# bytewax/bytewax

Measured on AMD Instinct MI355X. Metric: events/sec (whole node), tumbling-window wordcount, higher is better.
Workload: dtype int64; 1 GPU; model=tumbling-window wordcount (keyed count, 60s windows), events_per_batch_per_gpu=64000000, vocab=1000000, parallelism=key-hash all-to-allv dp1, engine=dataflow (run_main: source -> keyed_window_agg -> sink), radix=True, radix_v2=False, latency_method=poll-gap under load, closed_window_rows=317000000

## Files before the change

### bytewax_amd/_native/stream_kernels.hip

```cpp

#include <hip/hip_runtime.h>
#include <torch/extension.h>
#include <pybind11/stl.h>
#include <ATen/hip/HIPContext.h>

#include <chrono>
#include <type_traits>
#include <cstdlib>
#include <cstdint>
#include <cstring>
#include <vector>

#define WAVE 64
#define EMPTY_SLOT 0xFFFFFFFFFFFFFFFFULL

#define HIP_CHECK(expr)                                               \
  do {                                                                \
    hipError_t _e = (expr);                                           \
    TORCH_CHECK(_e == hipSuccess, "HIP error: ", hipGetErrorString(_e)); \
  } while (0)

static inline int n_blocks(int64_t n, int block) {
  int64_t b = (n + block - 1) / block;
  if (b > 2048) b = 2048;
// ... 169 lines not shown
    int64_t late_cap) {
  static_assert(!(LATE && DEDUP), "late tracking excludes the dedup path");
  if (ts_base_dev != nullptr) ts_base += *ts_base_dev;
  int lane = threadIdx.x & (WAVE - 1);
  int64_t stride = gridDim.x * (int64_t)blockDim.x;
  int64_t local_max = 0;
  int64_t first = blockIdx.x * (int64_t)blockDim.x + threadIdx.x;
  for (int64_t i = first; i - lane < n; i += stride) {
    bool valid = i < n;
    int64_t t = valid ? ((int64_t)ts[i] + ts_base) : 0;
    if constexpr (LATE) {
      bool is_late = valid && t < late_cutoff;
      int64_t lv = 0;
      if (MODE == AGG_SUM && is_late) lv = vals[i];
      late_append<MODE == AGG_SUM>(
          is_late, is_late ? keys[i] : 0, t, lv, late_keys, late_ts,
          late_vals, late_n, late_cap, error_flag);
      if (is_late) {
        valid = false;
        t = 0;
      }
    }
    if (t > local_max) local_max = t;
    uint64_t packed = 0;
    unsigned long long inc = 0;
    if (valid) {
      int64_t win = (t - align_ms) / off_ms;
      packed = ((uint64_t)(uint32_t)(int32_t)win << 32) | (uint32_t)keys[i];
      inc = (MODE == AGG_COUNT) ? 1ULL : (unsigned long long)vals[i];
      if (off_ms < len_ms) {
        int64_t num = t - align_ms - len_ms;
        int64_t win_lo = num / off_ms;
        if (num % off_ms != 0 && num < 0) win_lo -= 1;
        win_lo += 1;
        for (int64_t wn = win_lo; wn < win; ++wn) {
          uint64_t p2 =
              ((uint64_t)(uint32_t)(int32_t)wn << 32) | (uint32_t)keys[i];
          if (!hash_add(tkeys, tvals, mask, region_bits, p2, inc)) {
            atomicOr(error_flag, 1);
          }
        }
      }
    }

    bool ok = true;
    if (DEDUP) {
      unsigned long long remaining = __ballot(valid);
      bool leader = false;
      unsigned long long agg = 0;
      while (remaining) {
        int l = __ffsll((unsigned long long)remaining) - 1;
        uint64_t lk = (uint64_t)__shfl((long long)packed, l);
        unsigned long long match =
            __ballot(valid && packed == lk);
        if (MODE == AGG_COUNT) {
          if (lane == l) {
            leader = true;
            agg = __popcll(match);
          }
        } else {
          unsigned long long contrib =
              (valid && packed == lk) ? inc : 0ULL;
          for (int off = WAVE / 2; off > 0; off >>= 1) {
            contrib += (unsigned long long)__shfl_xor(
                (long long)contrib, off);
          }
          if (lane == l) {
            leader = true;
            agg = contrib;
          }
        }
        remaining &= ~match;
      }
      if (leader) ok = hash_add(tkeys, tvals, mask, region_bits, packed, agg);
    } else if (valid) {
      ok = hash_add(tkeys, tvals, mask, region_bits, packed, inc);
    }
    if (!ok) atomicOr(error_flag, 1);
  }
  for (int off = WAVE / 2; off > 0; off >>= 1) {
    int64_t other = __shfl_down((long long)local_max, off);
    if (other > local_max) local_max = other;
  }
  if ((threadIdx.x & (WAVE - 1)) == 0 && local_max > 0) {
    atomicMax(max_ts, (unsigned long long)local_max);
  }
}



#define V2_COARSE 256
#define V2_STAGE 32

__global__ __launch_bounds__(512) void k_scatter_coarse(
    const int32_t* __restrict__ keys,
    const int64_t* __restrict__ ts,
    int64_t n,
    int64_t align_ms,
    int64_t len_ms,
    int64_t ts_base,
    uint64_t mask,
    int region_bits,
    int64_t cap_c,
    int64_t res_cap,
    int* __restrict__ gcur,
    int* __restrict__ gres,
    uint64_t* __restrict__ ev,
    uint64_t* __restrict__ ev_res,
    unsigned long long* __restrict__ max_ts,
    int* __restrict__ error_flag) {
  __shared__ uint64_t stage[V2_COARSE][V2_STAGE];
  __shared__ int lcnt[V2_COARSE];
  int nb = (int)(((mask + 1) >> region_bits));
  int shift = 0;
  while ((nb >> shift) > V2_COARSE) ++shift;
  for (int b = threadIdx.x; b < V2_COARSE; b += blockDim.x) lcnt[b] = 0;
  __syncthreads();

  const int TILE = 8;
  int64_t chunk = (int64_t)blockDim.x * TILE;
  int64_t start = (int64_t)blockIdx.x * chunk;
  int64_t gstride = (int64_t)gridDim.x * chunk;
  int64_t local_max = 0;
  for (int64_t tile0 = start; tile0 < n; tile0 += gstride) {
    for (int t = 0; t < TILE; ++t) {
      int64_t i = tile0 + (int64_t)t * blockDim.x + threadIdx.x;
      if (i < n) {
        int64_t tm = ts[i] + ts_base;
        if (tm > local_max) local_max = tm;
        int64_t win = (tm - align_ms) / len_ms;
        uint64_t packed =
            ((uint64_t)(uint32_t)(int32_t)win << 32) | (uint32_t)keys[i];
        int cb = (int)(region_of(mix64(packed), mask, region_bits) >> shift);
        int r = atomicAdd(&lcnt[cb], 1);
        if (r < V2_STAGE) {
          stage[cb][r] = packed;
        } else {
          int rp = atomicAdd(&gres[cb], 1);
          if (rp < res_cap) {
            ev_res[(int64_t)cb * res_cap + rp] = packed;
          } else {
            atomicOr(error_flag, 1);
          }
        }
      }
    }
    __syncthreads();
    for (int b = threadIdx.x; b < V2_COARSE; b += blockDim.x) {
      int c = lcnt[b];
      if (c > V2_STAGE) c = V2_STAGE;
      int groups = c / 8;
      for (int g = 0; g < groups; ++g) {
        int base8 = atomicAdd(&gcur[b], 8);
        if (base8 + 8 <= cap_c) {
          uint64_t* dst = ev + (int64_t)b * cap_c + base8;
          #pragma unroll
          for (int q = 0; q < 8; ++q) dst[q] = stage[b][g * 8 + q];
        } else {
          for (int q = 0; q < 8; ++q) {
            int rp = atomicAdd(&gres[b], 1);
            if (rp < res_cap) {
              ev_res[(int64_t)b * res_cap + rp] = stage[b][g * 8 + q];
            } else {
              atomicOr(error_flag, 1);
            }
          }
        }
      }
      int rem = c - groups * 8;
      for (int q = 0; q < rem; ++q) {
        stage[b][q] = stage[b][groups * 8 + q];
      }
      lcnt[b] = rem;
    }
    __syncthreads();
  }
  for (int b = threadIdx.x; b < V2_COARSE; b += blockDim.x) {
    int c = lcnt[b];
    if (c > V2_STAGE) c = V2_STAGE;
    for (int q = 0; q < c; ++q) {
      int rp = atomicAdd(&gres[b], 1);
      if (rp < res_cap) {
        ev_res[(int64_t)b * res_cap + rp] = stage[b][q];
      } else {
        atomicOr(error_flag, 1);
      }
    }
  }
  for (int off = WAVE / 2; off > 0; off >>= 1) {
    int64_t other = __shfl_down((long long)local_max, off);
    if (other > local_max) local_max = other;
  }
  if ((threadIdx.x & (WAVE - 1)) == 0 && local_max > 0) {
    atomicMax(max_ts, (unsigned long long)local_max);
  }
}

#define V2_CACHE 4096

__global__ __launch_bounds__(256) void k_agg_cached(
    const uint64_t* __restrict__ ev,
    const uint64_t* __restrict__ ev_res,
    const int* __restrict__ gcur,
    const int* __restrict__ gres,
    int64_t cap_c,
    int64_t res_cap,
    int slices,
    uint64_t* __restrict__ tkeys,
    unsigned long long* __restrict__ tvals,
    uint64_t mask,
    int region_bits,
    int* __restrict__ error_flag) {
  __shared__ uint64_t ckeys[V2_CACHE];
  __shared__ unsigned long long cvals[V2_CACHE];
  for (int s = threadIdx.x; s < V2_CACHE; s += blockDim.x) {
    ckeys[s] = EMPTY_SLOT;
    cvals[s] = 0;
  }
  __syncthreads();
  int cb = blockIdx.x % V2_COARSE;
  int slice = blockIdx.x / V2_COARSE;

  auto agg_one = [&](uint64_t packed) {
    uint64_t h64 = mix64(packed);
    int lh = (int)((h64 >> 20) & (V2_CACHE - 1));
    for (int p = 0; p < 2; ++p) {
      uint64_t cur = ckeys[lh];
      if (cur == packed) {
        atomicAdd(&cvals[lh], 1ULL);
        return;
      }
      if (cur == EMPTY_SLOT) {
        uint64_t prev = atomicCAS(
            (unsigned long long*)&ckeys[lh], EMPTY_SLOT, packed);
        if (prev == EMPTY_SLOT || prev == packed) {
          atomicAdd(&cvals[lh], 1ULL);
          return;
        }
      }
      lh = (lh + 1) & (V2_CACHE - 1);
    }
    if (!hash_add(tkeys, tvals, mask, region_bits, packed, 1ULL)) {
      atomicOr(error_flag, 1);
    }
  };

  int c = gcur[cb];
  if (c > cap_c) c = (int)cap_c;
  for (int j = slice * (int)blockDim.x + threadIdx.x; j < c;
       j += slices * (int)blockDim.x) {
    agg_one(ev[(int64_t)cb * cap_c + j]);
  }
  int cr = gres[cb];
  if (cr > res_cap) cr = (int)res_cap;
  for (int j = slice * (int)blockDim.x + threadIdx.x; j < cr;
       j += slices * (int)blockDim.x) {
    agg_one(ev_res[(int64_t)cb * res_cap + j]);
  }
  __syncthreads();
  for (int s = threadIdx.x; s < V2_CACHE; s += blockDim.x) {
    if (ckeys[s] != EMPTY_SLOT) {
      if (!hash_add(tkeys, tvals, mask, region_bits, ckeys[s], cvals[s])) {
        atomicOr(error_flag, 1);
      }
    }
  }
}

__device__ __forceinline__ int64_t win_lo_of(
    int64_t t, int64_t align_ms, int64_t len_ms, int64_t off_ms) {
  int64_t num = t - align_ms - len_ms;
  int64_t fl = num >= 0 ? num / off_ms : -((-num + off_ms - 1) / off_ms);
  return fl + 1;
}

__device__ __forceinline__ int64_t win_of(
    int64_t t, int64_t align_ms, int64_t len_ms, uint64_t m2,
    uint64_t maxfast) {
  int64_t x = t - align_ms;
  if (m2 != 0 && (uint64_t)x < maxfast) {
    return (int64_t)__umul64hi((uint64_t)x, m2);
  }
  return x / len_ms;
}

static inline void magic_div_u64(
    int64_t d, uint64_t* m2, uint64_t* maxfast) {
  *m2 = 0;
  *maxfast = 0;
  if (d <= 1) return;
  if ((d & (d - 1)) == 0) {
    int s = 0;
    while ((int64_t(1) << s) < d) ++s;
    *m2 = (uint64_t)1 << (64 - s);
    *maxfast = ~(uint64_t)0;
    return;
  }
  const unsigned p = 60;
  unsigned __int128 one = 1;
  uint64_t M = (uint64_t)(((one << p) + (uint64_t)d - 1) / (uint64_t)d);
  uint64_t e = (uint64_t)((unsigned __int128)M * (uint64_t)d - (one << p));
  *m2 = M << 4;
  *maxfast = e ? (uint64_t)((one << p) / e) : ~(uint64_t)0;
}

template <int MODE, typename TS = int64_t, bool LATE = false>
__global__ void k_radix_scatter_fixed(
    const int32_t* __restrict__ keys,
    const TS* __restrict__ ts,
    const int64_t* __restrict__ vals,
    int64_t n,
    int64_t align_ms,
    int64_t len_ms,
    int64_t off_ms,
    int64_t ts_base,
    uint64_t mask,
    int region_bits,
    int64_t cap,
    int* __restrict__ gcursors,
    uint64_t* __restrict__ ev_packed,
    int64_t* __restrict__ ev_vals,
    int* __restrict__ ov_cursor,
    uint64_t* __restrict__ ov_packed,
    int64_t* __restrict__ ov_vals,
    int64_t ov_cap,
    unsigned long long* __restrict__ max_ts,
    int* __restrict__ error_flag,
    uint64_t win_m2,
    uint64_t win_maxfast,
    int64_t late_cutoff,
    int32_t* __restrict__ late_keys,
    int64_t* __restrict__ late_ts,
    int64_t* __restrict__ late_vals,
    int* __restrict__ late_n,
    int64_t late_cap) {
  static_assert(!(LATE && MODE == AGG_TS), "no late tracking for AGG_TS");
  extern __shared__ int lmem[];
  __shared__ int s_late[LATE ? 2 : 1];
  int nb = (int)(((mask + 1) >> region_bits));
  int* lhist = lmem;
  int* lbase = lmem + nb;
  for (int b = threadIdx.x; b < nb; b += blockDim.x) lhist[b] = 0;
  if constexpr (LATE) {
    if (threadIdx.x == 0) s_late[0] = 0;
  }
  __syncthreads();
  int64_t start = blockIdx.x * (int64_t)blockDim.x + threadIdx.x;
  int64_t stride = gridDim.x * (int64_t)blockDim.x;
  int64_t local_max = 0;
  for (int64_t i = start; i < n; i += stride) {
    int64_t t = (int64_t)ts[i] + ts_base;
    if constexpr (LATE) {
      bool is_late = t < late_cutoff;
      wave_reserve(is_late, &s_late[0]);
      if (is_late) continue;
    }
    if (t > local_max) local_max = t;
    uint64_t packed;
    int nwin = 1;
    if (MODE == AGG_TS) {
      packed = (uint64_t)(uint32_t)keys[i];
    } else {
      int64_t win = win_of(t, align_ms, off_ms, win_m2, win_maxfast);
      packed = ((uint64_t)(uint32_t)(int32_t)win << 32) | (uint32_t)keys[i];
      if (off_ms < len_ms) {
        nwin = (int)(win - win_lo_of(t, align_ms, len_ms, off_ms)) + 1;
      }
    }
    for (int w = 0; w < nwin; ++w) {
      atomicAdd(&lhist[(int)region_of(mix64(packed), mask, region_bits)], 1);
      packed -= (uint64_t)1 << 32;
    }
  }
  __syncthreads();
  for (int b = threadIdx.x; b < nb; b += blockDim.x) {
    lbase[b] = lhist[b] > 0 ? atomicAdd(&gcursors[b], lhist[b]) : 0;
    lhist[b] = 0;
  }
  if constexpr (LATE) {
    if (threadIdx.x == 0) {
      s_late[1] = s_late[0] > 0 ? atomicAdd(late_n, s_late[0]) : 0;
      s_late[0] = 0;
    }
  }
  __syncthreads();
  for (int64_t i = start; i < n; i += stride) {
    int64_t t = (int64_t)ts[i] + ts_base;
    if constexpr (LATE) {
      bool is_late = t < late_cutoff;
      int lpos = wave_reserve(is_late, &s_late[0]);
      if (is_late) {
        late_store<MODE == AGG_SUM>(
            (int64_t)s_late[1] + lpos, keys[i], t,
            MODE == AGG_SUM ? vals[i] : 0, late_keys, late_ts, late_vals,
            late_cap, error_flag);
        continue;
      }
    }
    uint64_t packed;
    int nwin = 1;
    if (MODE == AGG_TS) {
      packed = (uint64_t)(uint32_t)keys[i];
    } else {
      int64_t win = win_of(t, align_ms, off_ms, win_m2, win_maxfast);
      packed = ((uint64_t)(uint32_t)(int32_t)win << 32) | (uint32_t)keys[i];
      if (off_ms < len_ms) {
        nwin = (int)(win - win_lo_of(t, align_ms, len_ms, off_ms)) + 1;
      }
    }
    int64_t v = (MODE == AGG_SUM) ? vals[i] : (MODE == AGG_TS ? t : 0);
    for (int w = 0; w < nwin; ++w) {
      int b = (int)region_of(mix64(packed), mask, region_bits);
      int64_t in_bucket = lbase[b] + atomicAdd(&lhist[b], 1);
      if (in_bucket < cap) {
        int64_t pos = (int64_t)b * cap + in_bucket;
        ev_packed[pos] = packed;
        if (MODE != AGG_COUNT) ev_vals[pos] = v;
      } else {
        int opos = atomicAdd(ov_cursor, 1);
        if (opos < ov_cap) {
          ov_packed[opos] = packed;
          if (MODE != AGG_COUNT) ov_vals[opos] = v;
        } else {
          atomicOr(error_flag, 1);
        }
      }
      packed -= (uint64_t)1 << 32;
    }
  }
  for (int off = WAVE / 2; off > 0; off >>= 1) {
    int64_t other = __shfl_down((long long)local_max, off);
    if (other > local_max) local_max = other;
  }
  if ((threadIdx.x & (WAVE - 1)) == 0 && local_max > 0) {
    atomicMax(max_ts, (unsigned long long)local_max);
  }
}

template <int MODE, typename TS = int64_t>
__global__ void k_radix_scatter_direct(
    const int32_t* __restrict__ keys,
    const TS* __restrict__ ts,
    const int64_t* __restrict__ vals,
    int64_t n,
    int64_t align_ms,
    int64_t len_ms,
    int64_t off_ms,
    int64_t ts_base,
    uint64_t mask,
    int region_bits,
    int64_t cap,
    int* __restrict__ gcursors,
    uint64_t* __restrict__ ev_packed,
    int64_t* __restrict__ ev_vals,
    int* __restrict__ ov_cursor,
    uint64_t* __restrict__ ov_packed,
    int64_t* __restrict__ ov_vals,
    int64_t ov_cap,
    unsigned long long* __restrict__ max_ts,
    int* __restrict__ error_flag,
    uint64_t win_m2,
    uint64_t win_maxfast) {
  int64_t start = blockIdx.x * (int64_t)blockDim.x + threadIdx.x;
  int64_t stride = gridDim.x * (int64_t)blockDim.x;
  int64_t local_max = 0;
  for (int64_t i = start; i < n; i += stride) {
    int64_t t = (int64_t)ts[i] + ts_base;
    if (t > local_max) local_max = t;
    int64_t win = win_of(t, align_ms, len_ms, win_m2, win_maxfast);
    uint64_t packed =
        ((uint64_t)(uint32_t)(int32_t)win << 32) | (uint32_t)keys[i];
    int b = (int)region_of(mix64(packed), mask, region_bits);
    int64_t in_bucket = atomicAdd(&gcursors[b], 1);
    int64_t v = (MODE == AGG_SUM) ? vals[i] : 0;
    if (in_bucket < cap) {
      int64_t pos = (int64_t)b * cap + in_bucket;
      ev_packed[pos] = packed;
      if (MODE == AGG_SUM) ev_vals[pos] = v;
    } else {
      int opos = atomicAdd(ov_cursor, 1);
      if (opos < ov_cap) {
        ov_packed[opos] = packed;
        if (MODE == AGG_SUM) ov_vals[opos] = v;
      } else {
        atomicOr(error_flag, 1);
      }
    }
  }
  for (int off = WAVE / 2; off > 0; off >>= 1) {
    int64_t other = __shfl_down((long long)local_max, off);
    if (other > local_max) local_max = other;
  }
  if ((threadIdx.x & (WAVE - 1)) == 0 && local_max > 0) {
    atomicMax(max_ts, (unsigned long long)local_max);
  }
}

#define SC_GRAN 8

template <int MODE, typename TS = int64_t, int U = 16, int BLK = 256,
          bool LATE = false>
__global__ __launch_bounds__(BLK) void k_radix_scatter_staged(
    const int32_t* __restrict__ keys,
    const TS* __restrict__ ts,
    const int64_t* __restrict__ vals,
    int64_t n,
    int64_t align_ms,
    int64_t len_ms,
    int64_t off_ms,
    int64_t ts_base,
    uint64_t mask,
    int seg_bits,
    int64_t cap,
    int* __restrict__ gcursors,
    uint64_t* __restrict__ ev_packed,
    int64_t* __restrict__ ev_vals,
    int* __restrict__ ov_cursor,
    uint64_t* __restrict__ ov_packed,
    int64_t* __restrict__ ov_vals,
    int64_t ov_cap,
    unsigned long long* __restrict__ max_ts,
    int* __restrict__ error_flag,
    uint64_t win_m2,
    uint64_t win_maxfast,
    int64_t late_cutoff,
    int32_t* __restrict__ late_keys,
    int64_t* __restrict__ late_ts,
    int64_t* __restrict__ late_vals,
    int* __restrict__ late_n,
    int64_t late_cap) {
  static_assert(!(LATE && MODE == AGG_TS), "no late tracking for AGG_TS");
  extern __shared__ char smem[];
  __shared__ int s_late[LATE ? 2 : 1];
  const int nseg = (int)(((mask + 1) >> seg_bits));
  uint64_t* res = (uint64_t*)smem;
  int64_t* res_v =
      (int64_t*)(smem + (size_t)nseg * SC_GRAN * 8);
  int* res_cnt =
      (int*)(smem + (size_t)nseg * SC_GRAN * 8 *
                        (MODE != AGG_COUNT ? 2 : 1));
  int* lhist = res_cnt + nseg;
  int* lbase = lhist + nseg;
  int* lofs = lbase + nseg;
  for (int b = threadIdx.x; b < nseg; b += blockDim.x) {
    res_cnt[b] = 0;
    lhist[b] = 0;
  }
  if constexpr (LATE) {
    if (threadIdx.x == 0) s_late[0] = 0;
  }
  __syncthreads();

  auto emit = [&](int b, int64_t gpos, uint64_t packed, int64_t v) {
    if (gpos < cap) {
      int64_t pos = (int64_t)b * cap + gpos;
      ev_packed[pos] = packed;
      if (MODE != AGG_COUNT) ev_vals[pos] = v;
    } else if (packed != EMPTY_SLOT) {
      int opos = atomicAdd(ov_cursor, 1);
      if (opos < ov_cap) {
        ov_packed[opos] = packed;
        if (MODE != AGG_COUNT) ov_vals[opos] = v;
      } else {
        atomicOr(error_flag, 1);
      }
    }
  };

  const int64_t tile = (int64_t)blockDim.x * U;
  int64_t local_max = 0;
  for (int64_t t0 = (int64_t)blockIdx.x * tile; t0 < n;
       t0 += (int64_t)gridDim.x * tile) {
    uint64_t pk[U];
    int64_t pv[U];
    int sg[U];
    int nw[U];
    for (int u = 0; u < U; ++u) {
      int64_t i = t0 + (int64_t)u * blockDim.x + threadIdx.x;
      sg[u] = -1;
      if constexpr (LATE) {
        bool in = i < n;
        int64_t tl = in ? ((int64_t)ts[i] + ts_base) : 0;
        bool is_late = in && tl < late_cutoff;
        int lpos = wave_reserve(is_late, &s_late[0]);
        if (is_late) {
          sg[u] = -2;
          nw[u] = lpos;
          continue;
        }
      }
      if (i >= n) continue;
      int64_t t = (int64_t)ts[i] + ts_base;
      if (t > local_max) local_max = t;
      uint64_t packed;
      int nwin = 1;
      if (MODE == AGG_TS) {
        packed = (uint64_t)(uint32_t)keys[i];
      } else {
        int64_t win = win_of(t, align_ms, off_ms, win_m2, win_maxfast);
        packed =
            ((uint64_t)(uint32_t)(int32_t)win << 32) | (uint32_t)keys[i];
        if (off_ms < len_ms) {
          nwin =
              (int)(win - win_lo_of(t, align_ms, len_ms, off_ms)) + 1;
        }
      }
      pk[u] = packed;
      nw[u] = nwin;
      if (MODE == AGG_SUM) pv[u] = vals[i];
      else if (MODE == AGG_TS) pv[u] = t;
      int b = (int)region_of(mix64(packed), mask, seg_bits);
      sg[u] = b;
      atomicAdd(&lhist[b], 1);
      uint64_t p2 = packed;
      for (int w = 1; w < nwin; ++w) {
        p2 -= (uint64_t)1 << 32;
        atomicAdd(
            &lhist[(int)region_of(mix64(p2), mask, seg_bits)], 1);
      }
    }
    __syncthreads();
    for (int b = threadIdx.x; b < nseg; b += blockDim.x) {
      int tot = res_cnt[b] + lhist[b];
      int grant = tot & ~(SC_GRAN - 1);
      lbase[b] = grant > 0 ? atomicAdd(&gcursors[b], grant) : 0;
      lofs[b] = res_cnt[b];
      lhist[b] = grant;
    }
    if constexpr (LATE) {
      if (threadIdx.x == 0)
        s_late[1] = s_late[0] > 0 ? atomicAdd(late_n, s_late[0]) : 0;
    }
    __syncthreads();
    for (int b = threadIdx.x; b < nseg; b += blockDim.x) {
      int grant = lhist[b];
      if (grant > 0) {
        int rc = res_cnt[b];
        int gb = lbase[b];
        for (int j = 0; j < rc; ++j) {
          emit(b, (int64_t)gb + j, res[(size_t)b * SC_GRAN + j],
               MODE != AGG_COUNT ? res_v[(size_t)b * SC_GRAN + j] : 0);
        }
        res_cnt[b] = 0;
      }
    }
    __syncthreads();
    for (int u = 0; u < U; ++u) {
      if constexpr (LATE) {
        if (sg[u] == -2) {
          int64_t i = t0 + (int64_t)u * blockDim.x + threadIdx.x;
          late_store<MODE == AGG_SUM>(
              (int64_t)s_late[1] + nw[u], keys[i], (int64_t)ts[i] + ts_base,
              MODE == AGG_SUM ? vals[i] : 0, late_keys, late_ts, late_vals,
              late_cap, error_flag);
        }
      }
      if (sg[u] < 0) continue;
      uint64_t p2 = pk[u];
      for (int w = 0; w < nw[u]; ++w) {
        int b = w == 0 ? sg[u]
                       : (int)region_of(mix64(p2), mask, seg_bits);
        int vpos = atomicAdd(&lofs[b], 1);
        int grant = lhist[b];
        if (vpos < grant) {
          emit(b, (int64_t)lbase[b] + vpos, p2,
               MODE != AGG_COUNT ? pv[u] : 0);
        } else {
          res[(size_t)b * SC_GRAN + (vpos - grant)] = p2;
          if (MODE != AGG_COUNT)
            res_v[(size_t)b * SC_GRAN + (vpos - grant)] = pv[u];
        }
        p2 -= (uint64_t)1 << 32;
      }
    }
    __syncthreads();
    for (int b = threadIdx.x; b < nseg; b += blockDim.x) {
      res_cnt[b] = lofs[b] - lhist[b];
      lhist[b] = 0;
    }
    if constexpr (LATE) {
      if (threadIdx.x == 0) s_late[0] = 0;
    }
    __syncthreads();
  }
  for (int b = threadIdx.x; b < nseg; b += blockDim.x) {
    int rc = res_cnt[b];
    if (rc == 0) continue;
    int gb = atomicAdd(&gcursors[b], SC_GRAN);
    for (int j = 0; j < SC_GRAN; ++j) {
      uint64_t p = j < rc ? res[(size_t)b * SC_GRAN + j] : EMPTY_SLOT;
      emit(b, (int64_t)gb + j, p,
           (MODE != AGG_COUNT && j < rc) ? res_v[(size_t)b * SC_GRAN + j]
                                         : 0);
    }
  }
  for (int off = WAVE / 2; off > 0; off >>= 1) {
    int64_t other = __shfl_down((long long)local_max, off);
    if (other > local_max) local_max = other;
  }
  if ((threadIdx.x & (WAVE - 1)) == 0 && local_max > 0) {
    atomicMax(max_ts, (unsigned long long)local_max);
  }
}


#define GD_SPILL 0xFFFFFFFFu

static inline size_t staged2_lds_bytes(int64_t nseg, int64_t tile) {
  size_t stage_n = (size_t)(tile + 7 * nseg);
  return stage_n * 8
         + (size_t)nseg * SC_GRAN * 8
         + 3 * (size_t)nseg * sizeof(int)
         + (stage_n / SC_GRAN) * sizeof(uint32_t);
}

template <typename TS = int64_t, int U = 16, int BLK = 512>
__global__ __launch_bounds__(BLK) void k_radix_scatter_staged2(
    const int32_t* __restrict__ keys,
    const TS* __restrict__ ts,
    const int64_t* __restrict__ vals,
    int64_t n,
    int64_t align_ms,
    int64_t len_ms,
    int64_t off_ms,
    int64_t ts_base,
    uint64_t mask,
    int seg_bits,
    int64_t cap,
    int* __restrict__ gcursors,
    uint64_t* __restrict__ ev_packed,
    int64_t* __restrict__ ev_vals,
    int* __restrict__ ov_cursor,
    uint64_t* __restrict__ ov_packed,
    int64_t* __restrict__ ov_vals,
    int64_t ov_cap,
    unsigned long long* __restrict__ max_ts,
    int* __restrict__ error_flag,
    uint64_t win_m2,
    uint64_t win_maxfast) {
  constexpr int T = BLK * U;
  constexpr int NW = BLK / WAVE;
  static_assert(T + 7 * BLK < (1 << 14), "staging offset must fit 14 bits");
  static_assert(T <= (1 << 13), "tile rank shares a word with the segment");
  extern __shared__ __attribute__((aligned(16))) char smem_wc[];
  __shared__ int s_wtot[NW];
  const int nseg = (int)(((mask + 1) >> seg_bits));
  const int stage_n = T + 7 * nseg;
  uint64_t* stage = (uint64_t*)smem_wc;
  uint64_t* res = stage + stage_n;
  int* res_cnt = (int*)(res + (size_t)nseg * SC_GRAN);
  int* lhist = res_cnt + nseg;
  int* lpack = lhist + nseg;
  uint32_t* gdst = (uint32_t*)(lpack + nseg);
  const int tid = threadIdx.x;
  const int lane = tid & (WAVE - 1);
  const int wave = tid / WAVE;
  if (tid < nseg) {
    res_cnt[tid] = 0;
    lhist[tid] = 0;
  }
  __syncthreads();

  auto spill = [&](uint64_t packed) {
    int opos = atomicAdd(ov_cursor, 1);
    if (opos < ov_cap) ov_packed[opos] = packed;
    else atomicOr(error_flag, 1);
  };

  int32_t rk[U];
  TS rt[U];
  auto load_tile = [&](int64_t t0) {
#pragma unroll
    for (int u = 0; u < U; ++u) {
      int64_t i = t0 + u * BLK + tid;
      if (i > n - 1) i = n - 1;
      rk[u] = keys[i];
      rt[u] = ts[i];
    }
  };
  const int64_t stride = (int64_t)gridDim.x * T;
  int64_t local_max = 0;
  int64_t t0 = (int64_t)blockIdx.x * T;
  if (t0 < n) load_tile(t0);
  for (; t0 < n; t0 += stride) {
    uint64_t pk[U];
    int sr[U];
#pragma unroll
    for (int u = 0; u < U; ++u) {
      int64_t i = t0 + u * BLK + tid;
      int64_t t = (int64_t)rt[u] + ts_base;
      int64_t win = win_of(t, align_ms, len_ms, win_m2, win_maxfast);
      uint64_t packed =
          ((uint64_t)(uint32_t)(int32_t)win << 32) | (uint32_t)rk[u];
      pk[u] = packed;
      int b = (int)region_of(mix64(packed), mask, seg_bits);
      sr[u] = -1;
      if (i < n) {
        if (t > local_max) local_max = t;
        sr[u] = (atomicAdd(&lhist[b], 1) << 13) | b;
      }
    }
    if (t0 + stride < n) load_tile(t0 + stride);
    __syncthreads();
    int rc = 0, grant = 0, gb = 0;
    if (tid < nseg) {
      rc = res_cnt[tid];
      int tot = rc + lhist[tid];
      grant = tot & ~(SC_GRAN - 1);
      if (grant > 0) gb = atomicAdd(&gcursors[tid], grant);
      res_cnt[tid] = tot - grant;
      lhist[tid] = 0;
    }
    int incl = grant;
    for (int o = 1; o < WAVE; o <<= 1) {
      int v = __shfl_up(incl, o);
      if (lane >= o) incl += v;
    }
    if (lane == WAVE - 1) s_wtot[wave] = incl;
    __syncthreads();
    int total = 0, woff = 0;
    for (int w = 0; w < NW; ++w) {
      int v = s_wtot[w];
      if (w < wave) woff += v;
      total += v;
    }
    if (tid < nseg) {
      int off = woff + incl - grant;
      lpack[tid] = off | (rc << 14) | (grant << 17);
      if (grant > 0) {
#pragma unroll
        for (int j = 0; j < SC_GRAN - 1; ++j)
          stage[off + j] = res[(size_t)tid * SC_GRAN + j];
        for (int j = 0; j < grant; j += SC_GRAN) {
          int64_t gp = (int64_t)gb + j;
          gdst[(off + j) / SC_GRAN] =
              gp < cap ? (uint32_t)(((int64_t)tid * cap + gp) / SC_GRAN)
                       : GD_SPILL;
        }
      }
    }
    __syncthreads();
    for (int u = 0; u < U; ++u) {
      if (sr[u] < 0) continue;
      int b = sr[u] & ((1 << 13) - 1);
      int w = lpack[b];
      int vpos = ((w >> 14) & 7) + (sr[u] >> 13);
      int g = w >> 17;
      if (vpos < g) stage[(w & ((1 << 14) - 1)) + vpos] = pk[u];
      else res[(size_t)b * SC_GRAN + (vpos - g)] = pk[u];
    }
    __syncthreads();
    for (int p = tid; p < total / 2; p += BLK) {
      ulonglong2 v = *(const ulonglong2*)(stage + 2 * p);
      uint32_t d = gdst[p / 4];
      if (d != GD_SPILL) {
        *(ulonglong2*)(ev_packed + (int64_t)d * SC_GRAN + 2 * (p & 3)) = v;
      } else {
        if (v.x != EMPTY_SLOT) spill(v.x);
        if (v.y != EMPTY_SLOT) spill(v.y);
      }
    }
  }
  __syncthreads();
  if (tid < nseg) {
    int rc = res_cnt[tid];
    if (rc > 0) {
      int gb = atomicAdd(&gcursors[tid], SC_GRAN);
      for (int j = 0; j < SC_GRAN; ++j) {
        uint64_t p = j < rc ? res[(size_t)tid * SC_GRAN + j] : EMPTY_SLOT;
        int64_t gp = (int64_t)gb + j;
        if (gp < cap) ev_packed[(int64_t)tid * cap + gp] = p;
        else if (p != EMPTY_SLOT) spill(p);
      }
    }
  }
  for (int off = WAVE / 2; off > 0; off >>= 1) {
    int64_t other = __shfl_down((long long)local_max, off);
    if (other > local_max) local_max = other;
  }
  if ((threadIdx.x & (WAVE - 1)) == 0 && local_max > 0) {
    atomicMax(max_ts, (unsigned long long)local_max);
  }
}

template <int MODE>
__global__ void k_overflow_agg(
    const uint64_t* __restrict__ ov_packed,
    const int64_t* __restrict__ ov_vals,
    const int* __restrict__ ov_cursor,
    int64_t ov_cap,
    uint64_t* __restrict__ tkeys,
    unsigned long long* __restrict__ tvals,
    uint64_t mask,
    int region_bits,
    int* __restrict__ error_flag) {
  int64_t n = *ov_cursor;
  if (n > ov_cap) n = ov_cap;
  int64_t i = blockIdx.x * (int64_t)blockDim.x + threadIdx.x;
  int64_t stride = gridDim.x * (int64_t)blockDim.x;
  for (; i < n; i += stride) {
    unsigned long long inc =
        (MODE == AGG_SUM) ? (unsigned long long)ov_vals[i] : 1ULL;
    if (!hash_add(tkeys, tvals, mask, region_bits, ov_packed[i], inc)) {
      atomicOr(error_flag, 1);
    }
  }
}

typedef unsigned long long agg_u64x2 __attribute__((ext_vector_type(2)));

template <int MODE>
__global__ __launch_bounds__(1024) void k_radix_agg(
    const uint64_t* __restrict__ ev_packed,
    const int64_t* __restrict__ ev_vals,
    const int* __restrict__ counts,
    int64_t cap,
    uint64_t* __restrict__ tkeys,
    unsigned long long* __restrict__ tvals,
    uint64_t mask,
    int region_bits,
    int lds_bits,
    int* __restrict__ error_flag) {
  extern __shared__ char smem[];
  int region = 1 << lds_bits;
  uint64_t* lkeys = (uint64_t*)smem;
  unsigned long long* lvals =
      (unsigned long long*)(smem + (size_t)region * sizeof(uint64_t));
  for (int s = threadIdx.x; s < region; s += blockDim.x) {
    lkeys[s] = EMPTY_SLOT;
    lvals[s] = 0;
  }
  __syncthreads();
  int b = blockIdx.x;
  int cnt = counts[b];
  if (cnt > (int)cap) cnt = (int)cap;
  const uint64_t* seg = ev_packed + (int64_t)b * cap;
  const int64_t* segv =
      (MODE == AGG_SUM) ? ev_vals + (int64_t)b * cap : nullptr;

  auto add = [&](uint64_t packed, unsigned long long inc) {
    if (packed == EMPTY_SLOT) return;
    uint64_t h64 = mix64(packed);
    int lh = (int)((h64 >> 32) & (region - 1));
    bool done = false;
    for (int p = 0; p < region; ++p) {
      uint64_t cur = lkeys[lh];
      if (cur == packed) {
        atomicAdd(&lvals[lh], inc);
        done = true;
        break;
      }
      if (cur == EMPTY_SLOT) {
        uint64_t prev = atomicCAS(
            (unsigned long long*)&lkeys[lh], EMPTY_SLOT, packed);
        if (prev == EMPTY_SLOT || prev == packed) {
          atomicAdd(&lvals[lh], inc);
          done = true;
          break;
        }
      }
      lh = (lh + 1) & (region - 1);
    }
    if (!done) {
      if (!hash_add(tkeys, tvals, mask, region_bits, packed, inc)) {
        atomicOr(error_flag, 1);
      }
    }
  };

  const int head = (cnt > 0 && ((uintptr_t)seg & 15) != 0) ? 1 : 0;
  const int nvec = (cnt - head) >> 1;
  const int tail = head + 2 * nvec;
  if (threadIdx.x == 0 && head) {
    add(seg[0], MODE == AGG_SUM ? (unsigned long long)segv[0] : 1ULL);
  }
  if (threadIdx.x == blockDim.x - 1 && tail < cnt) {
    add(seg[tail],
        MODE == AGG_SUM ? (unsigned long long)segv[tail] : 1ULL);
  }

  constexpr int R = (MODE == AGG_SUM) ? 2 : 4;
  const agg_u64x2* vseg = (const agg_u64x2*)(seg + head);
  const int64_t* vval = (MODE == AGG_SUM) ? segv + head : nullptr;
  const int T = (int)blockDim.x;
  const int chunk = R * T;
  agg_u64x2 cur_p[R], nxt_p[R];
  unsigned long long cur_v[R][2], nxt_v[R][2];
  auto fetch = [&](agg_u64x2 (&bp)[R], unsigned long long (&bv)[R][2],
                   int base) {
#pragma unroll
    for (int r = 0; r < R; ++r) {
      int v = base + r * T + (int)threadIdx.x;
      if (v < nvec) {
        bp[r] = vseg[v];
        if (MODE == AGG_SUM) {
          bv[r][0] = (unsigned long long)vval[2 * v];
          bv[r][1] = (unsigned long long)vval[2 * v + 1];
        }
      } else {
        bp[r] = agg_u64x2{EMPTY_SLOT, EMPTY_SLOT};
        if (MODE == AGG_SUM) bv[r][0] = bv[r][1] = 0;
      }
    }
  };
  if (nvec > 0) fetch(cur_p, cur_v, 0);
  for (int base = 0; base < nvec; base += chunk) {
    if (base + chunk < nvec) fetch(nxt_p, nxt_v, base + chunk);
#pragma unroll
    for (int r = 0; r < R; ++r) {
      add(cur_p[r].x, MODE == AGG_SUM ? cur_v[r][0] : 1ULL);
      add(cur_p[r].y, MODE == AGG_SUM ? cur_v[r][1] : 1ULL);
    }
#pragma unroll
    for (int r = 0; r < R; ++r) {
      cur_p[r] = nxt_p[r];
      if (MODE == AGG_SUM) {
        cur_v[r][0] = nxt_v[r][0];
        cur_v[r][1] = nxt_v[r][1];
      }
    }
  }
  __syncthreads();
  for (int s = threadIdx.x; s < region; s += blockDim.x) {
    if (lkeys[s] != EMPTY_SLOT) {
      if (!hash_add(tkeys, tvals, mask, region_bits, lkeys[s], lvals[s])) {
        atomicOr(error_flag, 1);
      }
    }
  }
}

#define AGG_DELTA_MAX 14u
#define AGG_DELTA_MID 7u

template <int BLK, int R>
__global__ __launch_bounds__(BLK, BLK == 1024 ? 8 : 4) void k_radix_agg_count(
    const uint64_t* __restrict__ ev_packed,
    const int* __restrict__ counts,
    int64_t cap,
    uint64_t* __restrict__ tkeys,
    unsigned long long* __restrict__ tvals,
    uint64_t mask,
    int region_bits,
    int lds_bits,
    int* __restrict__ error_flag) {
  extern __shared__ char smem[];
  unsigned long long* cells = (unsigned long long*)smem;
  const int region = 1 << lds_bits;
  const uint32_t lmask = (uint32_t)region - 1;
  const int b = blockIdx.x;
  int cnt = counts[b];
  if (cnt > (int)cap) cnt = (int)cap;
  if (cnt <= 0) return;
  for (int s = threadIdx.x; s < region / 2; s += BLK) {
    ((agg_u64x2*)cells)[s] = agg_u64x2{EMPTY_SLOT, EMPTY_SLOT};
  }
  const uint64_t* seg = ev_packed + (int64_t)b * cap;
  const uint32_t wbase = (uint32_t)(seg[0] >> 32) - AGG_DELTA_MID;
  __syncthreads();

  auto escape = [&](uint64_t packed) {
    if (!hash_add(tkeys, tvals, mask, region_bits, packed, 1ULL)) {
      atomicOr(error_flag, 1);
    }
  };
  auto slot_of = [&](uint64_t packed) {
    return (uint32_t)(mix64(packed) >> 32) & lmask;
  };
  auto tag_of = [&](uint64_t packed) {
    return ((unsigned long long)(uint32_t)packed << 4) |
           (unsigned long long)((uint32_t)(packed >> 32) - wbase);
  };
  auto drain = [&](uint32_t pend, auto entry, auto start, auto skipped) {
    uint64_t packed = 0;
    unsigned long long tag = 0;
    uint32_t lh = 0;
    int left = 0;
    while (left != 0 || pend != 0) {
      if (left == 0) {
        int e = __ffs(pend) - 1;
        pend &= pend - 1;
        packed = entry(e);
        if ((uint32_t)(packed >> 32) - wbase > AGG_DELTA_MAX) {
          escape(packed);
          continue;
        }
        tag = tag_of(packed);
        lh = start(e);
        left = region - (skipped(e) ? 1 : 0);
      }
      unsigned long long cur = cells[lh];
      if (cur == EMPTY_SLOT) {
        cur = atomicCAS(&cells[lh], EMPTY_SLOT, tag << 28);
        if (cur == EMPTY_SLOT) cur = tag << 28;
      }
      if ((cur >> 28) == tag) {
        atomicAdd((unsigned int*)&cells[lh], 1u);
        left = 0;
      } else {
        lh = (lh + 1) & lmask;
        if (--left == 0) escape(packed);
      }
    }
  };
  auto add_one = [&](uint64_t packed) {
    if (packed == EMPTY_SLOT) return;
    drain(
        1u, [&](int) { return packed; },
        [&](int) { return slot_of(packed); }, [&](int) { return false; });
  };

  const int head = ((uintptr_t)seg & 15) != 0 ? 1 : 0;
  const int nvec = (cnt - head) >> 1;
  const int tail = head + 2 * nvec;
  if (threadIdx.x == 0 && head) add_one(seg[0]);
  if (threadIdx.x == BLK - 1 && tail < cnt) add_one(seg[tail]);

  const agg_u64x2* vseg = (const agg_u64x2*)(seg + head);
  constexpr int chunk = R * BLK;
  constexpr int E = 2 * R;
  agg_u64x2 cur_p[R], nxt_p[R];
  auto fetch = [&](agg_u64x2 (&bp)[R], int base) {
#pragma unroll
    for (int r = 0; r < R; ++r) {
      int v = base + r * BLK + (int)threadIdx.x;
      if (v < nvec) bp[r] = vseg[v];
      else bp[r] = agg_u64x2{EMPTY_SLOT, EMPTY_SLOT};
    }
  };
  fetch(cur_p, 0);
  for (int base = 0; base < nvec; base += chunk) {
    if (base + chunk < nvec) fetch(nxt_p, base + chunk);
    uint32_t slot[E];
    unsigned long long first[E];
#pragma unroll
    for (int e = 0; e < E; ++e) {
      uint64_t packed = (e & 1) ? cur_p[e >> 1].y : cur_p[e >> 1].x;
      slot[e] = slot_of(packed);
      first[e] = cells[slot[e]];
    }
    uint32_t pend = 0, moved = 0;
#pragma unroll
    for (int e = 0; e < E; ++e) {
      uint64_t packed = (e & 1) ? cur_p[e >> 1].y : cur_p[e >> 1].x;
      if (packed == EMPTY_SLOT) continue;
      bool in_range = (uint32_t)(packed >> 32) - wbase <= AGG_DELTA_MAX;
      if (in_range && (first[e] >> 28) == tag_of(packed)) {
        atomicAdd((unsigned int*)&cells[slot[e]], 1u);
      } else {
        pend |= 1u << e;
        if (first[e] != EMPTY_SLOT) {
          slot[e] = (slot[e] + 1) & lmask;
          moved |= 1u << e;
        }
      }
    }
    if (pend != 0) {
      drain(
          pend,
          [&](int e) {
            uint64_t v = 0;
#pragma unroll
            for (int j = 0; j < E; ++j) {
              if (j == e) v = (j & 1) ? cur_p[j >> 1].y : cur_p[j >> 1].x;
            }
            return v;
          },
          [&](int e) {
            uint32_t v = 0;
#pragma unroll
            for (int j = 0; j < E; ++j) {
              if (j == e) v = slot[j];
            }
            return v;
          },
          [&](int e) { return ((moved >> e) & 1u) != 0; });
    }
#pragma unroll
    for (int r = 0; r < R; ++r) cur_p[r] = nxt_p[r];
  }
  __syncthreads();

  for (int s = threadIdx.x; s < region; s += BLK) {
    unsigned long long c = cells[s];
    if (c != EMPTY_SLOT) {
      uint64_t packed =
          ((uint64_t)(wbase + ((uint32_t)c >> 28)) << 32) | (c >> 32);
      if (!hash_add(tkeys, tvals, mask, region_bits, packed,
                    c & 0x0FFFFFFFULL)) {
        atomicOr(error_flag, 1);
      }
    }
  }
}

__global__ void k_overflow_agg_stats(
    const uint64_t* __restrict__ ov_packed,
    const int64_t* __restrict__ ov_vals,
    const int* __restrict__ ov_cursor,
    int64_t ov_cap,
    uint64_t* __restrict__ tkeys,
    long long* __restrict__ tcnt,
    long long* __restrict__ tsum,
    long long* __restrict__ tmin,
    long long* __restrict__ tmax,
    uint64_t mask,
    int* __restrict__ error_flag) {
  int64_t n = *ov_cursor;
  if (n > ov_cap) n = ov_cap;
  int64_t i = blockIdx.x * (int64_t)blockDim.x + threadIdx.x;
  int64_t stride = gridDim.x * (int64_t)blockDim.x;
  for (; i < n; i += stride) {
    uint64_t slot = find_slot(tkeys, mask, ov_packed[i]);
    if (slot == ~0ULL) {
      atomicOr(error_flag, 1);
      continue;
    }
    long long v = ov_vals[i];
    atomicAdd((unsigned long long*)&tcnt[slot], 1ULL);
    atomicAdd((unsigned long long*)&tsum[slot], (unsigned long long)v);
    atomicMin(&tmin[slot], v);
    atomicMax(&tmax[slot], v);
  }
}

__global__ __launch_bounds__(1024) void k_radix_agg_stats(
    const uint64_t* __restrict__ ev_packed,
    const int64_t* __restrict__ ev_vals,
    const int* __restrict__ offsets,
    const int* __restrict__ counts,
    uint64_t* __restrict__ tkeys,
    long long* __restrict__ tcnt,
    long long* __restrict__ tsum,
    long long* __restrict__ tmin,
    long long* __restrict__ tmax,
    int64_t clamp_cap,
    uint64_t mask,
    int region_bits,
    int lds_bits,
    int* __restrict__ error_flag) {
  extern __shared__ char smem[];
  int region = 1 << lds_bits;
  uint64_t* lkeys = (uint64_t*)smem;
  long long* lcnt = (long long*)(smem + (size_t)region * 8);
  long long* lsum = (long long*)(smem + (size_t)region * 16);
  long long* lmin = (long long*)(smem + (size_t)region * 24);
  long long* lmax = (long long*)(smem + (size_t)region * 32);
  const long long LLMAX = 0x7FFFFFFFFFFFFFFFLL;
  for (int s = threadIdx.x; s < region; s += blockDim.x) {
    lkeys[s] = EMPTY_SLOT;
    lcnt[s] = 0;
    lsum[s] = 0;
    lmin[s] = LLMAX;
    lmax[s] = -LLMAX - 1;
  }
  __syncthreads();
  int b = blockIdx.x;
  int cnt = counts[b];
  if (clamp_cap > 0 && cnt > (int)clamp_cap) cnt = (int)clamp_cap;
  int start = offsets[b];
  for (int j = threadIdx.x; j < cnt; j += blockDim.x) {
    uint64_t packed = ev_packed[start + j];
    if (packed == EMPTY_SLOT) continue;
    long long v = ev_vals[start + j];
    uint64_t h64 = mix64(packed);
    int lh = (int)((h64 >> 32) & (region - 1));
    int slot = -1;
    for (int p = 0; p < region; ++p) {
      uint64_t cur = lkeys[lh];
      if (cur == packed) {
        slot = lh;
        break;
      }
      if (cur == EMPTY_SLOT) {
        uint64_t prev = atomicCAS(
            (unsigned long long*)&lkeys[lh], EMPTY_SLOT, packed);
        if (prev == EMPTY_SLOT || prev == packed) {
          slot = lh;
          break;
        }
      }
      lh = (lh + 1) & (region - 1);
    }
    if (slot >= 0) {
      atomicAdd((unsigned long long*)&lcnt[slot], 1ULL);
      atomicAdd((unsigned long long*)&lsum[slot], (unsigned long long)v);
      atomicMin(&lmin[slot], v);
      atomicMax(&lmax[slot], v);
    } else {
      uint64_t gslot = find_slot(tkeys, mask, packed);
      if (gslot == ~0ULL) {
        atomicOr(error_flag, 1);
      } else {
        atomicAdd((unsigned long long*)&tcnt[gslot], 1ULL);
        atomicAdd((unsigned long long*)&tsum[gslot], (unsigned long long)v);
        atomicMin(&tmin[gslot], v);
        atomicMax(&tmax[gslot], v);
      }
    }
  }
  __syncthreads();
  for (int s = threadIdx.x; s < region; s += blockDim.x) {
    if (lkeys[s] != EMPTY_SLOT) {
      uint64_t gslot = find_slot(tkeys, mask, lkeys[s]);
      if (gslot == ~0ULL) {
        atomicOr(error_flag, 1);
        continue;
      }
      atomicAdd((unsigned long long*)&tcnt[gslot],
                (unsigned long long)lcnt[s]);
      atomicAdd((unsigned long long*)&tsum[gslot],
                (unsigned long long)lsum[s]);
      atomicMin(&tmin[gslot], lmin[s]);
      atomicMax(&tmax[gslot], lmax[s]);
    }
  }
}

__global__ void k_close_extract(
    const uint64_t* __restrict__ tkeys,
    const unsigned long long* __restrict__ tvals,
    int64_t nslots,
    int64_t win_lo,
    int64_t win_hi,
    int32_t* __restrict__ out_keys,
    int32_t* __restrict__ out_wins,
    int64_t* __restrict__ out_vals,
    int* __restrict__ out_n,
    int64_t cap) {
  int64_t i = blockIdx.x * (int64_t)blockDim.x + threadIdx.x;
  int64_t stride = gridDim.x * (int64_t)blockDim.x;
  for (; i < nslots; i += stride) {
    uint64_t k = tkeys[i];
    bool take = false;
    int32_t win = 0;
    if (k != EMPTY_SLOT) {
      win = (int32_t)(uint32_t)(k >> 32);
      take = (int64_t)win >= win_lo && (int64_t)win < win_hi;
    }
    unsigned long long ball = __ballot(take);
    int lane = threadIdx.x & (WAVE - 1);
    if (ball != 0) {
      int wave_total = __popcll(ball);
      int rank = __popcll(ball & ((1ULL << lane) - 1ULL));
      int base = 0;
      int lead = __ffsll((unsigned long long)ball) - 1;
      if (lane == lead) base = atomicAdd(out_n, wave_total);
      base = __shfl(base, lead);
      if (take) {
        int64_t idx = base + rank;
        if (idx < cap) {
          out_keys[idx] = (int32_t)(uint32_t)(k & 0xFFFFFFFFULL);
          out_wins[idx] = win;
          out_vals[idx] = (int64_t)tvals[i];
        }
      }
    }
  }
}

#define CM_BLK 256
#define CM_PER 8
#define CM_CHUNK (CM_BLK * CM_PER)
#define CM_MAX_GRID 1024

__global__ __launch_bounds__(CM_BLK) void k_close_migrate(
    const uint64_t* __restrict__ tkeys,
    const unsigned long long* __restrict__ tvals,
    int64_t nslots,
    int64_t win_hi,
    uint64_t* __restrict__ nkeys,
    unsigned long long* __restrict__ nvals,
    uint64_t mask,
    int region_bits,
    int32_t* __restrict__ out_keys,
    int32_t* __restrict__ out_wins,
    int64_t* __restrict__ out_vals,
    int* __restrict__ out_n,
    int64_t cap,
    int* __restrict__ error_flag) {
  constexpr int NW = CM_BLK / WAVE;
  __shared__ int s_wave[2][NW];
  __shared__ int s_base[2];
  const int lane = threadIdx.x & (WAVE - 1);
  const int wave = threadIdx.x / WAVE;
  const bool vec = ((((uintptr_t)tkeys) | ((uintptr_t)tvals)) & 15) == 0;
  const int64_t nchunks = (nslots + CM_CHUNK - 1) / CM_CHUNK;
  int par = 0;
  for (int64_t c = blockIdx.x; c < nchunks; c += gridDim.x, par ^= 1) {
    const int64_t c0 = c * CM_CHUNK;
    uint64_t k[CM_PER];
    unsigned long long v[CM_PER];
    for (int j = 0; j < CM_PER / 2; ++j) {
      int64_t s = c0 + (int64_t)j * (CM_BLK * 2) + threadIdx.x * 2;
      if (vec && s + 1 < nslots) {
        ulonglong2 kk = *(const ulonglong2*)(tkeys + s);
        k[2 * j] = kk.x;
        k[2 * j + 1] = kk.y;
        v[2 * j] = 0;
        v[2 * j + 1] = 0;
        if (kk.x != EMPTY_SLOT || kk.y != EMPTY_SLOT) {
          ulonglong2 vv = *(const ulonglong2*)(tvals + s);
          v[2 * j] = vv.x;
          v[2 * j + 1] = vv.y;
        }
      } else {
        for (int q = 0; q < 2; ++q) {
          k[2 * j + q] = s + q < nslots ? tkeys[s + q] : EMPTY_SLOT;
          v[2 * j + q] = k[2 * j + q] != EMPTY_SLOT ? tvals[s + q] : 0;
        }
      }
    }
    unsigned takem = 0;
    for (int q = 0; q < CM_PER; ++q) {
      if (k[q] == EMPTY_SLOT) continue;
      int32_t win = (int32_t)(uint32_t)(k[q] >> 32);
      if ((int64_t)win < win_hi) {
        takem |= 1u << q;
      } else {
        uint64_t slot = find_slot_r(nkeys, mask, region_bits, k[q]);
        if (slot == ~0ULL) atomicOr(error_flag, 1);
        else nvals[slot] = v[q];
      }
    }
    const int cnt = __popc(takem);
    int incl = cnt;
    for (int off = 1; off < WAVE; off <<= 1) {
      int o = __shfl_up(incl, off);
      if (lane >= off) incl += o;
    }
    if (lane == WAVE - 1) s_wave[par][wave] = incl;
    __syncthreads();
    if (threadIdx.x == 0) {
      int total = 0;
      for (int w = 0; w < NW; ++w) total += s_wave[par][w];
      s_base[par] = total > 0 ? atomicAdd(out_n, total) : 0;
    }
    __syncthreads();
    if (takem != 0) {
      int64_t idx = (int64_t)s_base[par] + (incl - cnt);
      for (int w = 0; w < wave; ++w) idx += s_wave[par][w];
      for (int q = 0; q < CM_PER; ++q) {
        if (!((takem >> q) & 1u)) continue;
        if (idx < cap) {
          out_keys[idx] = (int32_t)(uint32_t)(k[q] & 0xFFFFFFFFULL);
          out_wins[idx] = (int32_t)(uint32_t)(k[q] >> 32);
          out_vals[idx] = (int64_t)v[q];
        }
        ++idx;
      }
    }
  }
}

__device__ __forceinline__ uint64_t find_slot_r(
    uint64_t* __restrict__ tkeys, uint64_t mask, int region_bits,
    uint64_t packed) {
  uint64_t h64 = mix64(packed);
  uint64_t h, probe_mask, base;
  if (region_bits == 0) {
    base = 0;
    probe_mask = mask;
    h = h64 & mask;
  } else {
    base = region_of(h64, mask, region_bits) << region_bits;
    probe_mask = (1ULL << region_bits) - 1;
    h = (h64 >> 32) & probe_mask;
  }
  for (uint64_t probes = 0; probes <= probe_mask; ++probes) {
    uint64_t slot = base | h;
    uint64_t cur = tkeys[slot];
    if (cur == packed) return slot;
    if (cur == EMPTY_SLOT) {
      uint64_t prev = atomicCAS(
          (unsigned long long*)&tkeys[slot], EMPTY_SLOT, packed);
      if (prev == EMPTY_SLOT || prev == packed) return slot;
    }
    h = (h + 1) & probe_mask;
  }
  return ~0ULL;
}

__device__ __forceinline__ uint64_t find_slot(
    uint64_t* __restrict__ tkeys, uint64_t mask, uint64_t packed) {
  return find_slot_r(tkeys, mask, 0, packed);
}

template <bool LATE = false>
__global__ void k_stats_insert(
    const int32_t* __restrict__ keys,
// ... 933 lines not shown
  int64_t stride = gridDim.x * (int64_t)blockDim.x;
  for (; i < n; i += stride) {
    int len = (int)(offs[i + 1] - offs[i]);
    uint64_t lo, hi;
    str_hash128(bytes + offs[i], len, &lo, &hi);
    uint64_t h = lo & mask;
    int32_t id = -1;
    for (uint64_t probes = 0; probes <= mask; ++probes) {
      uint64_t cur = dlo[h];
      if (cur == lo && dhi[h] == hi) {
        id = dids[h];
        break;
      }
      if (cur == EMPTY_SLOT) break;
      h = (h + 1) & mask;
    }
    out_ids[i] = id;
    if (id < 0) atomicExch(error_flag, 2);
  }
}

__global__ void k_dict_insert_pinned(
    const uint8_t* __restrict__ bytes,
    const int64_t* __restrict__ offs,
    const int32_t* __restrict__ ids,
    int64_t n,
    uint64_t* __restrict__ dlo,
    uint64_t* __restrict__ dhi,
    int32_t* __restrict__ dids,
    uint64_t mask,
    int* __restrict__ error_flag) {
  int64_t i = blockIdx.x * (int64_t)blockDim.x + threadIdx.x;
  int64_t stride = gridDim.x * (int64_t)blockDim.x;
  for (; i < n; i += stride) {
    int len = (int)(offs[i + 1] - offs[i]);
    uint64_t lo, hi;
    str_hash128(bytes + offs[i], len, &lo, &hi);
    uint64_t h = lo & mask;
    for (uint64_t probes = 0; probes <= mask; ++probes) {
      uint64_t prev = atomicCAS((unsigned long long*)&dlo[h],
                                EMPTY_SLOT, lo);
      if (prev == EMPTY_SLOT) {
        dhi[h] = hi;
        dids[h] = ids[i];
        break;
      }
      h = (h + 1) & mask;
      if (probes == mask) atomicOr(error_flag, 1);
    }
  }
}


__device__ __forceinline__ int str_owner(
    const uint8_t* __restrict__ bytes, const int64_t* __restrict__ offs,
    int64_t i, int world) {
  uint64_t lo, hi;
  str_hash128(bytes + offs[i], (int)(offs[i + 1] - offs[i]), &lo, &hi);
  return (int)(hi % (uint64_t)world);
}

__global__ void k_str_bucket_hist(
    const uint8_t* __restrict__ bytes,
    const int64_t* __restrict__ offs,
    int64_t n,
    int world,
    int* __restrict__ counts,
    long long* __restrict__ byte_counts
) {
  int64_t i = blockIdx.x * (int64_t)blockDim.x + threadIdx.x;
  int64_t stride = gridDim.x * (int64_t)blockDim.x;
  for (; i < n; i += stride) {
    int dst = str_owner(bytes, offs, i, world);
    atomicAdd(&counts[dst], 1);
    atomicAdd((unsigned long long*)&byte_counts[dst],
              (unsigned long long)(offs[i + 1] - offs[i]));
  }
}

__global__ void k_str_meta_scatter(
    const uint8_t* __restrict__ bytes,
    const int64_t* __restrict__ offs,
    const int64_t* __restrict__ ts,
    const int64_t* __restrict__ vals,
    int64_t n,
    int world,
    int* __restrict__ cursors,
    int32_t* __restrict__ send_lens,
    int64_t* __restrict__ send_ts,
    int64_t* __restrict__ send_vals,
    int32_t* __restrict__ src_idx) {
  int64_t i = blockIdx.x * (int64_t)blockDim.x + threadIdx.x;
  int64_t stride = gridDim.x * (int64_t)blockDim.x;
  for (; i < n; i += stride) {
    int dst = str_owner(bytes, offs, i, world);
    int pos = atomicAdd(&cursors[dst], 1);
    send_lens[pos] = (int32_t)(offs[i + 1] - offs[i]);
    send_ts[pos] = ts[i];
    if (vals != nullptr) send_vals[pos] = vals[i];
    src_idx[pos] = (int32_t)i;
  }
}

__global__ void k_str_byte_gather(
    const uint8_t* __restrict__ bytes,
    const int64_t* __restrict__ offs,
    const int32_t* __restrict__ src_idx,
    const int64_t* __restrict__ send_offs,
    int64_t n,
    uint8_t* __restrict__ send_bytes) {
  int64_t j = blockIdx.x * (int64_t)blockDim.x + threadIdx.x;
  int64_t stride = gridDim.x * (int64_t)blockDim.x;
  for (; j < n; j += stride) {
    int64_t i = src_idx[j];
    int64_t src = offs[i];
    int len = (int)(offs[i + 1] - src);
    int64_t dst = send_offs[j];
    for (int b = 0; b < len; ++b) send_bytes[dst + b] = bytes[src + b];
  }
}


static void check_dev(const torch::Tensor& t, torch::ScalarType st,
                      const char* name) {
  TORCH_CHECK(t.is_cuda(), name, " must be a device tensor");
  TORCH_CHECK(t.scalar_type() == st, name, " has wrong dtype");
  TORCH_CHECK(t.is_contiguous(), name, " must be contiguous");
}

struct LateSink {
  int64_t cutoff;
  int32_t* keys;
  int64_t* ts;
  int64_t* vals;
  int* n;
  int64_t cap;
};

static LateSink make_late_sink(
    int64_t late_cutoff,
    torch::Tensor& late_keys,
    torch::Tensor& late_ts,
    c10::optional<torch::Tensor>& late_vals,
    torch::Tensor& late_n,
    bool need_vals) {
  check_dev(late_keys, torch::kInt32, "late_keys");
  check_dev(late_ts, torch::kInt64, "late_ts");
  check_dev(late_n, torch::kInt32, "late_n");
  int64_t cap = late_keys.numel();
  TORCH_CHECK(late_ts.numel() >= cap, "late_ts smaller than late_keys");
  TORCH_CHECK(late_n.numel() >= 1, "late_n must hold the cursor");
  int64_t* vp = nullptr;
  if (need_vals) {
    TORCH_CHECK(late_vals.has_value(), "late tracking needs late_vals");
    check_dev(*late_vals, torch::kInt64, "late_vals");
    TORCH_CHECK(late_vals->numel() >= cap,
                "late_vals smaller than late_keys");
    vp = late_vals->data_ptr<int64_t>();
  }
  return LateSink{late_cutoff, late_keys.data_ptr<int32_t>(),
                  late_ts.data_ptr<int64_t>(), vp,
                  late_n.data_ptr<int32_t>(), cap};
}

static void window_agg_insert_impl(
    torch::Tensor keys,
    torch::Tensor ts,
    c10::optional<torch::Tensor> vals,
    torch::Tensor tkeys,
    torch::Tensor tvals,
    torch::Tensor max_ts,
    torch::Tensor error_flag,
    int64_t align_ms,
    int64_t len_ms,
    int64_t mode,
    bool dedup,
    int64_t ts_base,
    int64_t region_bits,
    int64_t off_ms,
    const LateSink* late) {
  TORCH_CHECK(late == nullptr || !dedup,
              "late tracking is incompatible with the dedup path");
  if (off_ms <= 0) off_ms = len_ms;
  TORCH_CHECK(off_ms <= len_ms, "window offset must be <= length");
  TORCH_CHECK(off_ms == len_ms || !dedup,
              "sliding windows are incompatible with the dedup path");
  check_dev(keys, torch::kInt32, "keys");
  bool ts32 = ts.scalar_type() == torch::kInt32;
  if (!ts32) check_dev(ts, torch::kInt64, "ts");
  check_dev(tkeys, torch::kInt64, "tkeys");
  check_dev(tvals, torch::kInt64, "tvals");
  check_dev(max_ts, torch::kInt64, "max_ts");
  check_dev(error_flag, torch::kInt32, "error_flag");
  int64_t n = keys.numel();
  TORCH_CHECK(ts.numel() == n, "ts/keys length mismatch");
  int64_t nslots = tkeys.numel();
  TORCH_CHECK((nslots & (nslots - 1)) == 0, "table size must be 2^k");
  TORCH_CHECK(len_ms > 0, "window length must be positive");
  const int64_t* vptr = nullptr;
  if (mode == AGG_SUM) {
    TORCH_CHECK(vals.has_value(), "sum mode requires vals");
    check_dev(*vals, torch::kInt64, "vals");
    TORCH_CHECK(vals->numel() == n, "vals/keys length mismatch");
    vptr = vals->data_ptr<int64_t>();
  }
  if (n == 0) return;
  auto stream = at::hip::getCurrentHIPStream();
  dim3 block(256);
  dim3 grid(n_blocks(n, 256));
  auto launch = [&](auto kern, auto tsptr) {
    hipLaunchKernelGGL(
        kern, grid, block, 0, stream,
        keys.data_ptr<int32_t>(), tsptr, vptr, n,
        (uint64_t*)tkeys.data_ptr<int64_t>(),
        (unsigned long long*)tvals.data_ptr<int64_t>(),
        (uint64_t)(nslots - 1), align_ms, len_ms, off_ms, ts_base,
        (int)region_bits,
        (unsigned long long*)max_ts.data_ptr<int64_t>(),
        error_flag.data_ptr<int32_t>(), (const int64_t*)nullptr,
        late ? late->cutoff : (int64_t)0, late ? late->keys : nullptr,
        late ? late->ts : nullptr, late ? late->vals : nullptr,
        late ? late->n : nullptr, late ? late->cap : (int64_t)0);
  };
  auto dispatch = [&](auto tsptr) {
    using TSV = std::remove_const_t<std::remove_pointer_t<decltype(tsptr)>>;
    if (late != nullptr && mode == AGG_COUNT)
      launch((k_window_agg_insert<AGG_COUNT, false, TSV, true>), tsptr);
    else if (late != nullptr)
      launch((k_window_agg_insert<AGG_SUM, false, TSV, true>), tsptr);
    else if (mode == AGG_COUNT && !dedup)
      launch(k_window_agg_insert<AGG_COUNT, false, TSV>, tsptr);
    else if (mode == AGG_COUNT && dedup)
      launch(k_window_agg_insert<AGG_COUNT, true, TSV>, tsptr);
    else if (mode == AGG_SUM && !dedup)
      launch(k_window_agg_insert<AGG_SUM, false, TSV>, tsptr);
    else
      launch(k_window_agg_insert<AGG_SUM, true, TSV>, tsptr);
  };
  if (ts32) dispatch(ts.data_ptr<int32_t>());
  else dispatch(ts.data_ptr<int64_t>());
}

void window_agg_insert(
    torch::Tensor keys,
    torch::Tensor ts,
    c10::optional<torch::Tensor> vals,
    torch::Tensor tkeys,
    torch::Tensor tvals,
    torch::Tensor max_ts,
    torch::Tensor error_flag,
    int64_t align_ms,
    int64_t len_ms,
    int64_t mode,
    bool dedup,
    int64_t ts_base,
    int64_t region_bits,
    int64_t off_ms) {
  window_agg_insert_impl(keys, ts, vals, tkeys, tvals, max_ts, error_flag,
                         align_ms, len_ms, mode, dedup, ts_base, region_bits,
                         off_ms, nullptr);
}

void window_agg_insert_late(
    torch::Tensor keys,
    torch::Tensor ts,
    c10::optional<torch::Tensor> vals,
    torch::Tensor tkeys,
    torch::Tensor tvals,
    torch::Tensor max_ts,
    torch::Tensor error_flag,
    int64_t align_ms,
    int64_t len_ms,
    int64_t mode,
    int64_t ts_base,
    int64_t region_bits,
    int64_t off_ms,
    int64_t late_cutoff,
    torch::Tensor late_keys,
    torch::Tensor late_ts,
    c10::optional<torch::Tensor> late_vals,
    torch::Tensor late_n) {
  LateSink sink = make_late_sink(late_cutoff, late_keys, late_ts, late_vals,
                                 late_n, mode == AGG_SUM);
  window_agg_insert_impl(keys, ts, vals, tkeys, tvals, max_ts, error_flag,
                         align_ms, len_ms, mode, false, ts_base, region_bits,
                         off_ms, &sink);
}

static unsigned device_cu_count() {
  static int cus = 0;
  if (cus == 0) {
    int dev = 0, v = 0;
    if (hipGetDevice(&dev) == hipSuccess &&
        hipDeviceGetAttribute(&v, hipDeviceAttributeMultiprocessorCount,
                              dev) == hipSuccess &&
        v > 0)
      cus = v;
    else
      cus = 256;
  }
  return (unsigned)cus;
}

template <typename TSV>
static void launch_count_staged(
    hipStream_t stream, const int32_t* keys, const TSV* ts, int64_t n,
    int64_t xf, int64_t align_ms, int64_t len_ms, int64_t off_ms,
    int64_t ts_base, uint64_t mask, int seg_bits, int64_t nseg, int64_t cap,
    int* gcur, uint64_t* evp, int* ovc, uint64_t* ovp, int64_t ov_cap,
    unsigned long long* max_ts, int* err, uint64_t win_m2,
    uint64_t win_maxfast, bool overlapped) {
  int env_u = 0, env_threads = 0, env_blocks = 0;
  if (const char* e = std::getenv("BYTEWAX_SCATTER_U")) env_u = atoi(e);
  if (const char* e = std::getenv("BYTEWAX_SCATTER_THREADS"))
    env_threads = atoi(e);
  if (const char* e = std::getenv("BYTEWAX_SCATTER_BLOCKS")) {
    int v = atoi(e);
    if (v > 0) env_blocks = v;
  }
  auto go = [&](auto kern, int threads, int u, unsigned cap_gs, size_t lds,
                auto... extra) {
    int64_t tile = (int64_t)threads * u;
    int64_t gs = (n * xf + tile - 1) / tile;
    if (env_blocks > 0) cap_gs = (unsigned)env_blocks;
    if (gs > (int64_t)cap_gs) gs = cap_gs;
    if (gs < 1) gs = 1;
    hipLaunchKernelGGL(
        kern, dim3((unsigned)gs), dim3((unsigned)threads), lds, stream, keys,
        ts, (const int64_t*)nullptr, n, align_ms, len_ms, off_ms, ts_base,
        mask, seg_bits, cap, gcur, evp, (int64_t*)nullptr, ovc, ovp,
        (int64_t*)nullptr, ov_cap, max_ts, err, win_m2, win_maxfast,
        extra...);
    HIP_CHECK(hipGetLastError());
  };
  if (xf == 1 && scatter_staged2_env() && (((uintptr_t)evp) & 15) == 0) {
    const unsigned cus = device_cu_count() * (overlapped ? 2u : 1u);
    int threads = env_threads == 1024 ? 1024 : 512;
    int u = threads == 512 && env_u != 8 ? 16 : 8;
    size_t lds = staged2_lds_bytes(nseg, (int64_t)threads * u);
    if (nseg <= threads && lds <= 160 * 1024) {
      if (threads == 1024)
        go((k_radix_scatter_staged2<TSV, 8, 1024>), 1024, 8, cus, lds);
      else if (u == 16)
        go((k_radix_scatter_staged2<TSV, 16, 512>), 512, 16, cus, lds);
      else
        go((k_radix_scatter_staged2<TSV, 8, 512>), 512, 8, cus, lds);
      return;
    }
  }
  size_t lds = (size_t)nseg * SC_GRAN * 8 + 4 * (size_t)nseg * sizeof(int);
  int threads = 512;
  if (env_threads == 256 || env_threads == 1024) threads = env_threads;
  if (threads == 512)
    go((k_radix_scatter_staged<AGG_COUNT, TSV, 16, 512>), 512, 16, 1024u,
       lds, NO_LATE_ARGS);
  else if (threads == 1024)
    go((k_radix_scatter_staged<AGG_COUNT, TSV, 16, 1024>), 1024, 16, 1024u,
       lds, NO_LATE_ARGS);
  else if (env_u == 8)
    go((k_radix_scatter_staged<AGG_COUNT, TSV, 8>), 256, 8, 1024u, lds,
       NO_LATE_ARGS);
  else if (env_u == 32)
    go((k_radix_scatter_staged<AGG_COUNT, TSV, 32>), 256, 32, 1024u, lds,
       NO_LATE_ARGS);
  else
    go((k_radix_scatter_staged<AGG_COUNT, TSV, 16>), 256, 16, 1024u, lds,
       NO_LATE_ARGS);
}

static bool agg_wide_env() {
  const char* s = std::getenv("BYTEWAX_AGG");
  return s != nullptr && s[0] == 'w';
}

static void launch_count_agg(
    hipStream_t stream, const uint64_t* evp, const int* gcur, int64_t cap,
    uint64_t* tkeys, unsigned long long* tvals, uint64_t mask,
    int region_bits, int seg_bits, int64_t nseg, int* err) {
  auto go = [&](auto kern, int threads, size_t lds, auto... lead) {
    hipLaunchKernelGGL(
        kern, dim3((unsigned)nseg), dim3((unsigned)threads), lds, stream,
        evp, lead..., gcur, cap, tkeys, tvals, mask, region_bits, seg_bits,
        err);
    HIP_CHECK(hipGetLastError());
  };
  if (!agg_wide_env() && cap < ((int64_t)1 << 28) && seg_bits >= 8 &&
      seg_bits <= 13) {
    size_t lds = (size_t)8 << seg_bits;
    if (seg_bits >= 12) go((k_radix_agg_count<1024, 2>), 1024, lds);
    else go((k_radix_agg_count<256, 2>), 256, lds);
    return;
  }
  go(k_radix_agg<AGG_COUNT>, seg_bits >= 12 ? 1024 : 256,
     (size_t)16 << seg_bits, (const int64_t*)nullptr);
}

static void radix_window_insert_impl(
    torch::Tensor keys,
    torch::Tensor ts,
    c10::optional<torch::Tensor> vals,
    torch::Tensor tkeys,
    torch::Tensor tvals,
    torch::Tensor max_ts,
    torch::Tensor error_flag,
    torch::Tensor gcursors,
    torch::Tensor ev_packed,
    torch::Tensor ev_vals,
    torch::Tensor ov_cursor,
    torch::Tensor ov_packed,
    torch::Tensor ov_vals,
    int64_t align_ms,
    int64_t len_ms,
    int64_t mode,
    int64_t ts_base,
    int64_t region_bits,
    int64_t off_ms,
    std::vector<int64_t> seg_counts,
    std::vector<int64_t> seg_bases,
    const LateSink* late) {
  if (off_ms <= 0) off_ms = len_ms;
  TORCH_CHECK(off_ms <= len_ms, "window offset must be <= length");
  check_dev(keys, torch::kInt32, "keys");
  bool seg32 = !seg_counts.empty();
  bool ts32 = ts.scalar_type() == torch::kInt32;
  if (seg32) {
    TORCH_CHECK(seg_counts.size() == seg_bases.size(),
                "seg_counts/seg_bases length mismatch");
    check_dev(ts, torch::kInt32, "ts32");
  } else if (!ts32) {
    check_dev(ts, torch::kInt64, "ts");
  }
  int64_t n = keys.numel();
  int64_t nslots = tkeys.numel();
  TORCH_CHECK((nslots & (nslots - 1)) == 0, "table size must be 2^k");
  TORCH_CHECK(region_bits > 0, "radix path requires region_bits > 0");
  TORCH_CHECK(region_bits <= 12, "region_bits > 12 exceeds the LDS "
              "budget of the aggregation kernel (16 B/slot)");
  int64_t nb = nslots >> region_bits;
  TORCH_CHECK(nb >= 1 && nb <= 8192, "region count out of range");
  TORCH_CHECK(gcursors.numel() >= nb, "gcursors too small");
  const int64_t* vptr = nullptr;
  if (mode == AGG_SUM) {
    TORCH_CHECK(vals.has_value(), "sum mode requires vals");
    vptr = vals->data_ptr<int64_t>();
  }
  if (n == 0) return;
  auto stream = at::hip::getCurrentHIPStream();
  uint64_t mask = (uint64_t)(nslots - 1);
  dim3 block(256);
  dim3 grid(n_blocks(n, 256));

  ScatterKind kind = scatter_kind_env();
  int64_t xf = off_ms < len_ms ? (len_ms + off_ms - 1) / off_ms : 1;
  TORCH_CHECK(xf <= 64, "sliding expansion > 64x; use a larger offset");
  if (kind == SCAT_DIRECT && xf > 1) kind = SCAT_FIXED;
  if (late != nullptr && kind == SCAT_DIRECT) kind = SCAT_FIXED;
  int coarse = scatter_coarse_bits(kind);
  int seg_bits = (int)region_bits + coarse;
  int64_t nseg = nslots >> seg_bits;
  size_t staged_lds = (size_t)nseg * SC_GRAN * 8 *
                          (mode == AGG_SUM ? 2 : 1) +
                      4 * (size_t)nseg * sizeof(int);
  const size_t late_lds = late != nullptr ? 2 * sizeof(int) : 0;
  while (kind == SCAT_STAGED &&
         (nseg < 1 || staged_lds + late_lds > 160 * 1024 ||
          seg_bits > 13)) {
    if (coarse > 0 && seg_bits > 13) {
      coarse -= 1;
    } else {
      kind = SCAT_FIXED;
      coarse = 0;
    }
    seg_bits = (int)region_bits + coarse;
    nseg = nslots >> seg_bits;
    staged_lds = (size_t)nseg * SC_GRAN * 8 * (mode == AGG_SUM ? 2 : 1) +
                 4 * (size_t)nseg * sizeof(int);
  }
  if (seg_bits > 13) {
    coarse = 0;
    seg_bits = (int)region_bits;
    nseg = nb;
  }
  int64_t cap = ev_packed.numel() / nseg;
  if (kind == SCAT_STAGED) {
    cap &= ~(int64_t)(SC_GRAN - 1);
    if (cap < SC_GRAN) {
      kind = SCAT_FIXED;
      coarse = 0;
      seg_bits = (int)region_bits;
      nseg = nb;
      cap = ev_packed.numel() / nseg;
    }
  }
  TORCH_CHECK(cap * nseg >= 2 * n * xf || cap >= n * xf,
              "scatter buffers too small (need ~2x batch x expansion)");
  if (mode == AGG_SUM) {
    TORCH_CHECK(ev_vals.numel() >= nseg * cap, "ev_vals too small");
  }
  gcursors.narrow(0, 0, nseg).zero_();
  ov_cursor.zero_();
  size_t hist_lds = (size_t)nseg * sizeof(int);

  int env_blocks = 0;
  if (const char* sb = std::getenv("BYTEWAX_SCATTER_BLOCKS")) {
    int v = atoi(sb);
    if (v > 0) env_blocks = v;
  }

  struct Seg {
    int64_t off, n, base;
  };
  std::vector<Seg> segs;
  if (seg32) {
    int64_t off = 0;
    for (size_t i = 0; i < seg_counts.size(); ++i) {
      if (seg_counts[i] > 0) segs.push_back({off, seg_counts[i], seg_bases[i]});
      off += seg_counts[i];
    }
    TORCH_CHECK(off == n, "segment counts must sum to batch length");
  } else {
    segs.push_back({0, n, ts_base});
  }

  uint64_t win_m2, win_maxfast;
  magic_div_u64(off_ms, &win_m2, &win_maxfast);
  unsigned scat_threads = 256;
  auto scat = [&](auto kern, auto tsptr, const Seg& sg, unsigned gx,
                  size_t lds, auto... extra) {
    hipLaunchKernelGGL(
        kern, dim3(gx), dim3(scat_threads), lds, stream,
        keys.data_ptr<int32_t>() + sg.off, tsptr + sg.off,
        vptr != nullptr ? vptr + sg.off : nullptr, sg.n, align_ms, len_ms,
        off_ms, sg.base, mask, seg_bits, cap, gcursors.data_ptr<int32_t>(),
        (uint64_t*)ev_packed.data_ptr<int64_t>(),
        mode == AGG_SUM ? ev_vals.data_ptr<int64_t>() : nullptr,
        ov_cursor.data_ptr<int32_t>(),
        (uint64_t*)ov_packed.data_ptr<int64_t>(),
        mode == AGG_SUM ? ov_vals.data_ptr<int64_t>() : nullptr,
        ov_packed.numel(),
        (unsigned long long*)max_ts.data_ptr<int64_t>(),
        error_flag.data_ptr<int32_t>(), win_m2, win_maxfast, extra...);
    HIP_CHECK(hipGetLastError());
  };
  auto scat_late = [&](auto tsptr, const Seg& sg) {
    using TSV = std::remove_const_t<std::remove_pointer_t<decltype(tsptr)>>;
    if (kind == SCAT_STAGED) {
      int sthreads = mode == AGG_COUNT ? 512 : 256;
      scat_threads = (unsigned)sthreads;
      unsigned gs =
          (unsigned)((sg.n * xf + sthreads * 16 - 1) / (sthreads * 16));
      if (gs > 1024u) gs = 1024u;
      if (gs < 1) gs = 1;
      if (mode == AGG_COUNT)
        scat((k_radix_scatter_staged<AGG_COUNT, TSV, 16, 512, true>), tsptr,
             sg, gs, staged_lds, late->cutoff, late->keys, late->ts,
             late->vals, late->n, late->cap);
      else
        scat((k_radix_scatter_staged<AGG_SUM, TSV, 16, 256, true>), tsptr,
             sg, gs, staged_lds, late->cutoff, late->keys, late->ts,
             late->vals, late->n, late->cap);
    } else {
      scat_threads = 256;
      unsigned gx = (unsigned)n_blocks(sg.n, 256);
      if (mode == AGG_COUNT)
        scat((k_radix_scatter_fixed<AGG_COUNT, TSV, true>), tsptr, sg, gx,
             2 * hist_lds, late->cutoff, late->keys, late->ts, late->vals,
             late->n, late->cap);
      else
        scat((k_radix_scatter_fixed<AGG_SUM, TSV, true>), tsptr, sg, gx,
             2 * hist_lds, late->cutoff, late->keys, late->ts, late->vals,
             late->n, late->cap);
    }
  };
  auto scat_any = [&](auto tsptr, const Seg& sg) {
    using TSV = std::remove_const_t<std::remove_pointer_t<decltype(tsptr)>>;
    if (late != nullptr) {
      scat_late(tsptr, sg);
      return;
    }
    unsigned gx = (unsigned)n_blocks(sg.n, 256);
    if (env_blocks > 0 && (unsigned)env_blocks < gx) gx = (unsigned)env_blocks;
    if (kind == SCAT_STAGED) {
      if (mode == AGG_COUNT) {
        launch_count_staged<TSV>(
            stream, keys.data_ptr<int32_t>() + sg.off, tsptr + sg.off, sg.n,
            xf, align_ms, len_ms, off_ms, sg.base, mask, seg_bits, nseg, cap,
            gcursors.data_ptr<int32_t>(),
            (uint64_t*)ev_packed.data_ptr<int64_t>(),
            ov_cursor.data_ptr<int32_t>(),
            (uint64_t*)ov_packed.data_ptr<int64_t>(), ov_packed.numel(),
            (unsigned long long*)max_ts.data_ptr<int64_t>(),
            error_flag.data_ptr<int32_t>(), win_m2, win_maxfast,
            false);
      } else {
        unsigned cap_gs = env_blocks > 0 ? (unsigned)env_blocks : 1024u;
        unsigned gs = (unsigned)((sg.n * xf + 256 * 16 - 1) / (256 * 16));
        if (gs > cap_gs) gs = cap_gs;
        if (gs < 1) gs = 1;
        scat_threads = 256;
        scat(k_radix_scatter_staged<AGG_SUM, TSV>, tsptr, sg, gs,
             staged_lds, NO_LATE_ARGS);
      }
    } else if (kind == SCAT_DIRECT) {
      scat_threads = 256;
      if (mode == AGG_COUNT)
        scat(k_radix_scatter_direct<AGG_COUNT, TSV>, tsptr, sg, gx, 0);
      else
        scat(k_radix_scatter_direct<AGG_SUM, TSV>, tsptr, sg, gx, 0);
    } else {
      scat_threads = 256;
      if (mode == AGG_COUNT)
        scat(k_radix_scatter_fixed<AGG_COUNT, TSV>, tsptr, sg, gx,
             2 * hist_lds, NO_LATE_ARGS);
      else
        scat(k_radix_scatter_fixed<AGG_SUM, TSV>, tsptr, sg, gx,
             2 * hist_lds, NO_LATE_ARGS);
    }
  };
  for (const Seg& sg : segs) {
    if (seg32 || ts32) scat_any(ts.data_ptr<int32_t>(), sg);
    else scat_any(ts.data_ptr<int64_t>(), sg);
  }

  size_t agg_lds = (size_t)16 << seg_bits;
  dim3 agg_block(seg_bits >= 12 ? 1024 : 256);
  auto agg = [&](auto kern) {
    hipLaunchKernelGGL(
        kern, dim3((unsigned)nseg), agg_block, agg_lds, stream,
        (const uint64_t*)ev_packed.data_ptr<int64_t>(),
        mode == AGG_SUM ? ev_vals.data_ptr<int64_t>() : nullptr,
        gcursors.data_ptr<int32_t>(), cap,
        (uint64_t*)tkeys.data_ptr<int64_t>(),
        (unsigned long long*)tvals.data_ptr<int64_t>(), mask,
        (int)region_bits, seg_bits, error_flag.data_ptr<int32_t>());
  };
  if (mode == AGG_COUNT) {
    launch_count_agg(
        stream, (const uint64_t*)ev_packed.data_ptr<int64_t>(),
        gcursors.data_ptr<int32_t>(), cap,
        (uint64_t*)tkeys.data_ptr<int64_t>(),
        (unsigned long long*)tvals.data_ptr<int64_t>(), mask,
        (int)region_bits, seg_bits, nseg, error_flag.data_ptr<int32_t>());
  } else {
    agg(k_radix_agg<AGG_SUM>);
  }

  auto ov = [&](auto kern) {
    hipLaunchKernelGGL(
        kern, dim3(64), dim3(256), 0, stream,
        (const uint64_t*)ov_packed.data_ptr<int64_t>(),
        mode == AGG_SUM ? ov_vals.data_ptr<int64_t>() : nullptr,
        ov_cursor.data_ptr<int32_t>(), ov_packed.numel(),
        (uint64_t*)tkeys.data_ptr<int64_t>(),
        (unsigned long long*)tvals.data_ptr<int64_t>(), mask,
        (int)region_bits, error_flag.data_ptr<int32_t>());
  };
  if (mode == AGG_COUNT) ov(k_overflow_agg<AGG_COUNT>);
  else ov(k_overflow_agg<AGG_SUM>);
}

void radix_window_insert(
    torch::Tensor keys,
    torch::Tensor ts,
    c10::optional<torch::Tensor> vals,
    torch::Tensor tkeys,
    torch::Tensor tvals,
    torch::Tensor max_ts,
    torch::Tensor error_flag,
    torch::Tensor gcursors,
    torch::Tensor ev_packed,
    torch::Tensor ev_vals,
    torch::Tensor ov_cursor,
    torch::Tensor ov_packed,
    torch::Tensor ov_vals,
    int64_t align_ms,
    int64_t len_ms,
    int64_t mode,
    int64_t ts_base,
    int64_t region_bits,
    int64_t off_ms = 0,
    std::vector<int64_t> seg_counts = {},
    std::vector<int64_t> seg_bases = {}) {
  radix_window_insert_impl(
      keys, ts, vals, tkeys, tvals, max_ts, error_flag, gcursors, ev_packed,
      ev_vals, ov_cursor, ov_packed, ov_vals, align_ms, len_ms, mode, ts_base,
      region_bits, off_ms, std::move(seg_counts), std::move(seg_bases),
      nullptr);
}

void radix_window_insert_late(
    torch::Tensor keys,
    torch::Tensor ts,
    c10::optional<torch::Tensor> vals,
    torch::Tensor tkeys,
    torch::Tensor tvals,
    torch::Tensor max_ts,
    torch::Tensor error_flag,
    torch::Tensor gcursors,
    torch::Tensor ev_packed,
    torch::Tensor ev_vals,
    torch::Tensor ov_cursor,
    torch::Tensor ov_packed,
    torch::Tensor ov_vals,
    int64_t align_ms,
    int64_t len_ms,
    int64_t mode,
    int64_t ts_base,
    int64_t region_bits,
    int64_t off_ms,
    int64_t late_cutoff,
    torch::Tensor late_keys,
    torch::Tensor late_ts,
    c10::optional<torch::Tensor> late_vals,
    torch::Tensor late_n) {
  LateSink sink = make_late_sink(late_cutoff, late_keys, late_ts, late_vals,
                                 late_n, mode == AGG_SUM);
  radix_window_insert_impl(
      keys, ts, vals, tkeys, tvals, max_ts, error_flag, gcursors, ev_packed,
      ev_vals, ov_cursor, ov_packed, ov_vals, align_ms, len_ms, mode, ts_base,
      region_bits, off_ms, {}, {}, &sink);
}

void radix_scatter_only(
    torch::Tensor keys,
    torch::Tensor ts,
    c10::optional<torch::Tensor> vals,
    torch::Tensor max_ts,
    torch::Tensor error_flag,
    torch::Tensor gcursors,
    torch::Tensor ev_packed,
    torch::Tensor ev_vals,
    torch::Tensor ov_cursor,
    torch::Tensor ov_packed,
    torch::Tensor ov_vals,
    int64_t nslots,
    int64_t align_ms,
    int64_t len_ms,
    int64_t mode,
    int64_t ts_base,
    int64_t region_bits,
    int64_t off_ms,
    std::vector<int64_t> seg_counts,
    std::vector<int64_t> seg_bases) {
  if (off_ms <= 0) off_ms = len_ms;
  TORCH_CHECK(off_ms <= len_ms, "window offset must be <= length");
  check_dev(keys, torch::kInt32, "keys");
  bool seg32 = !seg_counts.empty();
  bool ts32 = ts.scalar_type() == torch::kInt32;
  if (seg32) {
    TORCH_CHECK(seg_counts.size() == seg_bases.size(),
                "seg_counts/seg_bases length mismatch");
    check_dev(ts, torch::kInt32, "ts32");
  } else if (!ts32) {
    check_dev(ts, torch::kInt64, "ts");
  }
  int64_t n = keys.numel();
  TORCH_CHECK((nslots & (nslots - 1)) == 0, "table size must be 2^k");
  int64_t nb = nslots >> region_bits;
  const int64_t* vptr = nullptr;
  if (mode == AGG_SUM) {
    TORCH_CHECK(vals.has_value(), "sum mode requires vals");
    vptr = vals->data_ptr<int64_t>();
  }
  auto stream = at::hip::getCurrentHIPStream();
  uint64_t mask = (uint64_t)(nslots - 1);
  dim3 block(256);
  uint64_t win_m2, win_maxfast;
  magic_div_u64(off_ms <= 0 ? len_ms : off_ms, &win_m2, &win_maxfast);

  ScatterKind kind = scatter_kind_env();
  int64_t xf = off_ms < len_ms ? (len_ms + off_ms - 1) / off_ms : 1;
  TORCH_CHECK(xf <= 64, "sliding expansion > 64x; use a larger offset");
  if (kind == SCAT_DIRECT && xf > 1) kind = SCAT_FIXED;
  int coarse = scatter_coarse_bits(kind);
  int seg_bits = (int)region_bits + coarse;
  int64_t nseg = nslots >> seg_bits;
  size_t staged_lds = (size_t)nseg * SC_GRAN * 8 *
                          (mode == AGG_SUM ? 2 : 1) +
                      4 * (size_t)nseg * sizeof(int);
  while (kind == SCAT_STAGED &&
         (nseg < 1 || staged_lds > 160 * 1024 || seg_bits > 13)) {
    if (coarse > 0 && seg_bits > 13) {
      coarse -= 1;
    } else {
      kind = SCAT_FIXED;
      coarse = 0;
    }
    seg_bits = (int)region_bits + coarse;
    nseg = nslots >> seg_bits;
    staged_lds = (size_t)nseg * SC_GRAN * 8 * (mode == AGG_SUM ? 2 : 1) +
                 4 * (size_t)nseg * sizeof(int);
  }
  if (seg_bits > 13) {
    coarse = 0;
    seg_bits = (int)region_bits;
    nseg = nb;
  }
  int64_t cap = ev_packed.numel() / nseg;
  if (kind == SCAT_STAGED) {
    cap &= ~(int64_t)(SC_GRAN - 1);
    if (cap < SC_GRAN) {
      kind = SCAT_FIXED;
      coarse = 0;
      seg_bits = (int)region_bits;
      nseg = nb;
      cap = ev_packed.numel() / nseg;
    }
  }
  TORCH_CHECK(cap * nseg >= 2 * n * xf || cap >= n * xf,
              "scatter buffers too small");
  size_t hist_lds = (size_t)nseg * sizeof(int);
  HIP_CHECK(hipMemsetAsync(
      gcursors.data_ptr<int32_t>(), 0, (size_t)nseg * sizeof(int), stream));
  HIP_CHECK(hipMemsetAsync(
      ov_cursor.data_ptr<int32_t>(), 0, sizeof(int), stream));
  if (n == 0) return;

  struct Seg {
    int64_t off, n, base;
  };
  std::vector<Seg> segs;
  if (seg32) {
    int64_t off = 0;
    for (size_t i = 0; i < seg_counts.size(); ++i) {
      if (seg_counts[i] > 0) segs.push_back({off, seg_counts[i], seg_bases[i]});
      off += seg_counts[i];
    }
  } else {
    segs.push_back({0, n, ts_base});
  }
  unsigned scat_threads = 256;
  auto scat = [&](auto kern, auto tsptr, const Seg& sg, unsigned gx,
                  size_t lds, auto... extra) {
    hipLaunchKernelGGL(
        kern, dim3(gx), dim3(scat_threads), lds,
        stream, keys.data_ptr<int32_t>() + sg.off, tsptr + sg.off,
        vptr != nullptr ? vptr + sg.off : nullptr, sg.n, align_ms, len_ms,
        off_ms, sg.base, mask, seg_bits, cap, gcursors.data_ptr<int32_t>(),
        (uint64_t*)ev_packed.data_ptr<int64_t>(),
        mode == AGG_SUM ? ev_vals.data_ptr<int64_t>() : nullptr,
        ov_cursor.data_ptr<int32_t>(),
        (uint64_t*)ov_packed.data_ptr<int64_t>(),
        mode == AGG_SUM ? ov_vals.data_ptr<int64_t>() : nullptr,
        ov_packed.numel(),
        (unsigned long long*)max_ts.data_ptr<int64_t>(),
        error_flag.data_ptr<int32_t>(), win_m2, win_maxfast, extra...);
  };
  auto scat_any = [&](auto tsptr, const Seg& sg) {
    using TSV = std::remove_const_t<std::remove_pointer_t<decltype(tsptr)>>;
    if (kind == SCAT_STAGED) {
      if (mode == AGG_COUNT) {
        launch_count_staged<TSV>(
            stream, keys.data_ptr<int32_t>() + sg.off, tsptr + sg.off, sg.n,
            xf, align_ms, len_ms, off_ms, sg.base, mask, seg_bits, nseg, cap,
            gcursors.data_ptr<int32_t>(),
            (uint64_t*)ev_packed.data_ptr<int64_t>(),
            ov_cursor.data_ptr<int32_t>(),
            (uint64_t*)ov_packed.data_ptr<int64_t>(), ov_packed.numel(),
            (unsigned long long*)max_ts.data_ptr<int64_t>(),
            error_flag.data_ptr<int32_t>(), win_m2, win_maxfast,
            true);
      } else {
        unsigned gs = (unsigned)((sg.n + 4095) / 4096);
        if (gs > 1024) gs = 1024;
        if (gs < 1) gs = 1;
        scat(k_radix_scatter_staged<AGG_SUM, TSV>, tsptr, sg, gs,
             staged_lds, NO_LATE_ARGS);
      }
    } else if (kind == SCAT_DIRECT) {
      unsigned gx = (unsigned)n_blocks(sg.n, 256);
      if (mode == AGG_COUNT)
        scat(k_radix_scatter_direct<AGG_COUNT, TSV>, tsptr, sg, gx, 0);
      else
        scat(k_radix_scatter_direct<AGG_SUM, TSV>, tsptr, sg, gx, 0);
    } else {
      unsigned gx = (unsigned)n_blocks(sg.n, 256);
      if (mode == AGG_COUNT)
        scat(k_radix_scatter_fixed<AGG_COUNT, TSV>, tsptr, sg, gx,
             2 * hist_lds, NO_LATE_ARGS);
      else
        scat(k_radix_scatter_fixed<AGG_SUM, TSV>, tsptr, sg, gx,
             2 * hist_lds, NO_LATE_ARGS);
    }
  };
  for (const Seg& sg : segs) {
    if (seg32 || ts32) scat_any(ts.data_ptr<int32_t>(), sg);
    else scat_any(ts.data_ptr<int64_t>(), sg);
  }
}

void radix_agg_only(
    torch::Tensor tkeys,
    torch::Tensor tvals,
    torch::Tensor error_flag,
    torch::Tensor gcursors,
    torch::Tensor ev_packed,
    torch::Tensor ev_vals,
    torch::Tensor ov_cursor,
    torch::Tensor ov_packed,
    torch::Tensor ov_vals,
    int64_t mode,
    int64_t region_bits) {
  int64_t nslots = tkeys.numel();
  int64_t nb = nslots >> region_bits;
  auto stream = at::hip::getCurrentHIPStream();
  uint64_t mask = (uint64_t)(nslots - 1);
  ScatterKind kind = scatter_kind_env();
  int coarse = scatter_coarse_bits(kind);
  int seg_bits = (int)region_bits + coarse;
  int64_t nseg = nslots >> seg_bits;
  size_t staged_lds = (size_t)nseg * SC_GRAN * 8 *
                          (mode == AGG_SUM ? 2 : 1) +
                      4 * (size_t)nseg * sizeof(int);
  while (kind == SCAT_STAGED &&
         (nseg < 1 || staged_lds > 160 * 1024 || seg_bits > 13)) {
    if (coarse > 0 && seg_bits > 13) {
      coarse -= 1;
    } else {
      kind = SCAT_FIXED;
      coarse = 0;
    }
    seg_bits = (int)region_bits + coarse;
    nseg = nslots >> seg_bits;
    staged_lds = (size_t)nseg * SC_GRAN * 8 * (mode == AGG_SUM ? 2 : 1) +
                 4 * (size_t)nseg * sizeof(int);
  }
  if (seg_bits > 13) {
    seg_bits = (int)region_bits;
    nseg = nb;
  }
  int64_t cap = ev_packed.numel() / nseg;
  if (kind == SCAT_STAGED) {
    cap &= ~(int64_t)(SC_GRAN - 1);
    if (cap < SC_GRAN) {
      kind = SCAT_FIXED;
      seg_bits = (int)region_bits;
      nseg = nb;
      cap = ev_packed.numel() / nseg;
    }
  }
  size_t agg_lds = (size_t)16 << seg_bits;
  dim3 agg_block(seg_bits >= 12 ? 1024 : 256);
  auto agg = [&](auto kern) {
    hipLaunchKernelGGL(
        kern, dim3((unsigned)nseg), agg_block, agg_lds, stream,
        (const uint64_t*)ev_packed.data_ptr<int64_t>(),
        mode == AGG_SUM ? ev_vals.data_ptr<int64_t>() : nullptr,
        gcursors.data_ptr<int32_t>(), cap,
        (uint64_t*)tkeys.data_ptr<int64_t>(),
        (unsigned long long*)tvals.data_ptr<int64_t>(), mask,
        (int)region_bits, seg_bits, error_flag.data_ptr<int32_t>());
  };
  if (mode == AGG_COUNT) {
    launch_count_agg(
        stream, (const uint64_t*)ev_packed.data_ptr<int64_t>(),
        gcursors.data_ptr<int32_t>(), cap,
        (uint64_t*)tkeys.data_ptr<int64_t>(),
        (unsigned long long*)tvals.data_ptr<int64_t>(), mask,
        (int)region_bits, seg_bits, nseg, error_flag.data_ptr<int32_t>());
  } else {
    agg(k_radix_agg<AGG_SUM>);
  }
  auto ov = [&](auto kern) {
    hipLaunchKernelGGL(
        kern, dim3(64), dim3(256), 0, stream,
        (const uint64_t*)ov_packed.data_ptr<int64_t>(),
        mode == AGG_SUM ? ov_vals.data_ptr<int64_t>() : nullptr,
        ov_cursor.data_ptr<int32_t>(), ov_packed.numel(),
        (uint64_t*)tkeys.data_ptr<int64_t>(),
        (unsigned long long*)tvals.data_ptr<int64_t>(), mask,
        (int)region_bits, error_flag.data_ptr<int32_t>());
  };
  if (mode == AGG_COUNT) ov(k_overflow_agg<AGG_COUNT>);
  else ov(k_overflow_agg<AGG_SUM>);
}

void radix_v2_window_insert(
    torch::Tensor keys,
    torch::Tensor ts,
    torch::Tensor tkeys,
    torch::Tensor tvals,
    torch::Tensor max_ts,
    torch::Tensor error_flag,
    torch::Tensor gcur,
    torch::Tensor gres,
    torch::Tensor ev,
    torch::Tensor ev_res,
    int64_t align_ms,
    int64_t len_ms,
    int64_t ts_base,
    int64_t region_bits) {
  check_dev(keys, torch::kInt32, "keys");
  check_dev(ts, torch::kInt64, "ts");
  int64_t n = keys.numel();
  int64_t nslots = tkeys.numel();
  TORCH_CHECK((nslots & (nslots - 1)) == 0, "table size must be 2^k");
  int64_t cap_c = ev.numel() / V2_COARSE;
  TORCH_CHECK(cap_c % 8 == 0, "coarse capacity must be 8-aligned");
  int64_t res_cap = ev_res.numel() / V2_COARSE;
  if (n == 0) return;
  auto stream = at::hip::getCurrentHIPStream();
  uint64_t mask = (uint64_t)(nslots - 1);
  gcur.zero_();
  gres.zero_();
  hipLaunchKernelGGL(
      k_scatter_coarse, dim3(256), dim3(512), 0, stream,
      keys.data_ptr<int32_t>(), ts.data_ptr<int64_t>(), n, align_ms,
      len_ms, ts_base, mask, (int)region_bits, cap_c, res_cap,
      gcur.data_ptr<int32_t>(), gres.data_ptr<int32_t>(),
      (uint64_t*)ev.data_ptr<int64_t>(),
      (uint64_t*)ev_res.data_ptr<int64_t>(),
      (unsigned long long*)max_ts.data_ptr<int64_t>(),
      error_flag.data_ptr<int32_t>());
  int slices = 8;
  hipLaunchKernelGGL(
      k_agg_cached, dim3(V2_COARSE * slices), dim3(256), 0, stream,
      (const uint64_t*)ev.data_ptr<int64_t>(),
      (const uint64_t*)ev_res.data_ptr<int64_t>(),
      gcur.data_ptr<int32_t>(), gres.data_ptr<int32_t>(), cap_c, res_cap,
      slices, (uint64_t*)tkeys.data_ptr<int64_t>(),
      (unsigned long long*)tvals.data_ptr<int64_t>(), mask,
      (int)region_bits, error_flag.data_ptr<int32_t>());
}

static void launch_close_migrate(
    hipStream_t stream, const torch::Tensor& tkeys,
    const torch::Tensor& tvals, int64_t win_hi, const torch::Tensor& nkeys,
    const torch::Tensor& nvals, int64_t region_bits,
    const torch::Tensor& out_keys, const torch::Tensor& out_wins,
    const torch::Tensor& out_vals, const torch::Tensor& out_n,
    const torch::Tensor& error_flag) {
  int64_t nslots = tkeys.numel();
  int64_t nchunks = (nslots + CM_CHUNK - 1) / CM_CHUNK;
  if (nchunks < 1) nchunks = 1;
  unsigned grid = (unsigned)(nchunks < CM_MAX_GRID ? nchunks : CM_MAX_GRID);
  hipLaunchKernelGGL(
      k_close_migrate, dim3(grid), dim3(CM_BLK), 0, stream,
      (const uint64_t*)tkeys.data_ptr<int64_t>(),
      (const unsigned long long*)tvals.data_ptr<int64_t>(), nslots, win_hi,
      (uint64_t*)nkeys.data_ptr<int64_t>(),
      (unsigned long long*)nvals.data_ptr<int64_t>(),
      (uint64_t)(nslots - 1), (int)region_bits,
      out_keys.data_ptr<int32_t>(), out_wins.data_ptr<int32_t>(),
      out_vals.data_ptr<int64_t>(), out_n.data_ptr<int32_t>(),
      out_keys.numel(), error_flag.data_ptr<int32_t>());
}

int64_t close_extract(
    torch::Tensor tkeys,
    torch::Tensor tvals,
    int64_t win_lo,
    int64_t win_hi,
    torch::Tensor out_keys,
    torch::Tensor out_wins,
    torch::Tensor out_vals,
    torch::Tensor out_n) {
  check_dev(tkeys, torch::kInt64, "tkeys");
  check_dev(tvals, torch::kInt64, "tvals");
  check_dev(out_keys, torch::kInt32, "out_keys");
  check_dev(out_wins, torch::kInt32, "out_wins");
  check_dev(out_vals, torch::kInt64, "out_vals");
  check_dev(out_n, torch::kInt32, "out_n");
  int64_t nslots = tkeys.numel();
  auto stream = at::hip::getCurrentHIPStream();
  dim3 block(256);
  dim3 grid(n_blocks(nslots, 256));
  hipLaunchKernelGGL(
      k_close_extract, grid, block, 0, stream,
      (const uint64_t*)tkeys.data_ptr<int64_t>(),
      (const unsigned long long*)tvals.data_ptr<int64_t>(), nslots, win_lo,
      win_hi, out_keys.data_ptr<int32_t>(),
      out_wins.data_ptr<int32_t>(), out_vals.data_ptr<int64_t>(),
      out_n.data_ptr<int32_t>(), out_keys.numel());
  return 0;
}

void close_migrate(
    torch::Tensor tkeys,
    torch::Tensor tvals,
    torch::Tensor nkeys,
    torch::Tensor nvals,
    int64_t win_hi,
    int64_t region_bits,
    torch::Tensor out_keys,
    torch::Tensor out_wins,
    torch::Tensor out_vals,
    torch::Tensor out_n,
    torch::Tensor error_flag) {
  check_dev(tkeys, torch::kInt64, "tkeys");
  check_dev(nkeys, torch::kInt64, "nkeys");
  check_dev(tvals, torch::kInt64, "tvals");
  check_dev(nvals, torch::kInt64, "nvals");
  int64_t nslots = tkeys.numel();
  TORCH_CHECK(nkeys.numel() == nslots, "table size mismatch");
  launch_close_migrate(
      at::hip::getCurrentHIPStream(), tkeys, tvals, win_hi, nkeys, nvals,
      region_bits, out_keys, out_wins, out_vals, out_n, error_flag);
}

static void stats_insert_impl(
    torch::Tensor keys,
    torch::Tensor ts,
    torch::Tensor vals,
    torch::Tensor tkeys,
    torch::Tensor tcnt,
    torch::Tensor tsum,
    torch::Tensor tmin,
    torch::Tensor tmax,
    torch::Tensor max_ts,
    torch::Tensor error_flag,
    int64_t align_ms,
    int64_t len_ms,
    int64_t ts_base,
    const LateSink* late) {
  check_dev(keys, torch::kInt32, "keys");
  check_dev(ts, torch::kInt64, "ts");
  check_dev(vals, torch::kInt64, "vals");
  check_dev(tkeys, torch::kInt64, "tkeys");
  int64_t n = keys.numel();
  int64_t nslots = tkeys.numel();
  TORCH_CHECK((nslots & (nslots - 1)) == 0, "table size must be 2^k");
  if (n == 0) return;
  auto stream = at::hip::getCurrentHIPStream();
  dim3 block(256);
  dim3 grid(n_blocks(n, 256));
  auto launch = [&](auto kern, auto... extra) {
    hipLaunchKernelGGL(
        kern, grid, block, 0, stream, keys.data_ptr<int32_t>(),
        ts.data_ptr<int64_t>(), vals.data_ptr<int64_t>(),
        n, (uint64_t*)tkeys.data_ptr<int64_t>(),
        (long long*)tcnt.data_ptr<int64_t>(),
        (long long*)tsum.data_ptr<int64_t>(),
        (long long*)tmin.data_ptr<int64_t>(),
        (long long*)tmax.data_ptr<int64_t>(), (uint64_t)(nslots - 1),
        align_ms, len_ms, ts_base,
        (unsigned long long*)max_ts.data_ptr<int64_t>(),
        error_flag.data_ptr<int32_t>(), extra...);
  };
  if (late != nullptr)
    launch(k_stats_insert<true>, late->cutoff, late->keys, late->ts,
           late->vals, late->n, late->cap);
  else
    launch(k_stats_insert<false>, NO_LATE_ARGS);
}

void stats_insert(
    torch::Tensor keys,
    torch::Tensor ts,
    torch::Tensor vals,
    torch::Tensor tkeys,
    torch::Tensor tcnt,
    torch::Tensor tsum,
    torch::Tensor tmin,
    torch::Tensor tmax,
    torch::Tensor max_ts,
    torch::Tensor error_flag,
    int64_t align_ms,
    int64_t len_ms,
    int64_t ts_base) {
  stats_insert_impl(keys, ts, vals, tkeys, tcnt, tsum, tmin, tmax, max_ts,
                    error_flag, align_ms, len_ms, ts_base, nullptr);
}

void stats_insert_late(
    torch::Tensor keys,
    torch::Tensor ts,
    torch::Tensor vals,
    torch::Tensor tkeys,
    torch::Tensor tcnt,
    torch::Tensor tsum,
    torch::Tensor tmin,
    torch::Tensor tmax,
    torch::Tensor max_ts,
    torch::Tensor error_flag,
    int64_t align_ms,
    int64_t len_ms,
    int64_t ts_base,
    int64_t late_cutoff,
    torch::Tensor late_keys,
    torch::Tensor late_ts,
    torch::Tensor late_vals,
    torch::Tensor late_n) {
  c10::optional<torch::Tensor> lv(late_vals);
  LateSink sink =
      make_late_sink(late_cutoff, late_keys, late_ts, lv, late_n, true);
  stats_insert_impl(keys, ts, vals, tkeys, tcnt, tsum, tmin, tmax, max_ts,
                    error_flag, align_ms, len_ms, ts_base, &sink);
}

static void radix_stats_insert_impl(
    torch::Tensor keys,
    torch::Tensor ts,
    torch::Tensor vals,
    torch::Tensor tkeys,
    torch::Tensor tcnt,
    torch::Tensor tsum,
    torch::Tensor tmin,
    torch::Tensor tmax,
    torch::Tensor max_ts,
    torch::Tensor error_flag,
    torch::Tensor gcursors,
    torch::Tensor ev_packed,
    torch::Tensor ev_vals,
    torch::Tensor ov_cursor,
    torch::Tensor ov_packed,
    torch::Tensor ov_vals,
    int64_t align_ms,
    int64_t len_ms,
    int64_t ts_base,
    int64_t region_bits,
    const LateSink* late) {
  check_dev(keys, torch::kInt32, "keys");
  bool ts32 = ts.scalar_type() == torch::kInt32;
  if (!ts32) check_dev(ts, torch::kInt64, "ts");
  check_dev(vals, torch::kInt64, "vals");
  int64_t n = keys.numel();
  int64_t nslots = tkeys.numel();
  TORCH_CHECK((nslots & (nslots - 1)) == 0, "table size must be 2^k");
  TORCH_CHECK(region_bits > 0 && region_bits <= 10,
              "stats radix needs 0 < region_bits <= 10 (40 B/slot LDS)");
  int64_t nb = nslots >> region_bits;
  TORCH_CHECK(nb >= 1 && nb <= 8192, "region count out of range");
  if (n == 0) return;
  auto stream = at::hip::getCurrentHIPStream();
  uint64_t mask = (uint64_t)(nslots - 1);
  dim3 block(256);
  dim3 grid(n_blocks(n, 256));

  ScatterKind kind = scatter_kind_env();
  if (late != nullptr && kind == SCAT_DIRECT) kind = SCAT_FIXED;
  int coarse = scatter_coarse_bits(kind);
  int seg_bits = (int)region_bits + coarse;
  int64_t nseg = nslots >> seg_bits;
  size_t staged_lds = (size_t)nseg * SC_GRAN * 8 * 2 +
                      4 * (size_t)nseg * sizeof(int);
  const size_t late_lds = late != nullptr ? 2 * sizeof(int) : 0;
  while (kind == SCAT_STAGED &&
         (nseg < 1 || staged_lds + late_lds > 160 * 1024 ||
          seg_bits > 11)) {
    if (coarse > 0 && seg_bits > 11) {
      coarse -= 1;
    } else {
      kind = SCAT_FIXED;
      coarse = 0;
    }
    seg_bits = (int)region_bits + coarse;
    nseg = nslots >> seg_bits;
    staged_lds = (size_t)nseg * SC_GRAN * 8 * 2 +
                 4 * (size_t)nseg * sizeof(int);
  }
  if (seg_bits > 11) {
    coarse = 0;
    seg_bits = (int)region_bits;
    nseg = nb;
  }
  int64_t cap = ev_packed.numel() / nseg;
  if (kind == SCAT_STAGED) {
    cap &= ~(int64_t)(SC_GRAN - 1);
    if (cap < SC_GRAN) {
      kind = SCAT_FIXED;
      coarse = 0;
      seg_bits = (int)region_bits;
      nseg = nb;
      cap = ev_packed.numel() / nseg;
    }
  }
  TORCH_CHECK(cap * nseg >= 2 * n || cap >= n,
              "scatter buffers too small (need ~2x batch)");
// ... 906 lines not shown
    torch::Tensor dst_acc,
    torch::Tensor out_keys,
    torch::Tensor out_start,
    torch::Tensor out_end,
    torch::Tensor out_vals,
    torch::Tensor out_n,
    torch::Tensor error_flag,
    int64_t horizon_ms,
    int64_t max_open) {
  check_dev(scnt, torch::kInt32, "scnt");
  check_dev(dst_cnt, torch::kInt32, "dst_cnt");
  int64_t nslots = skeys.numel();
  TORCH_CHECK((nslots & (nslots - 1)) == 0, "table size must be 2^k");
  TORCH_CHECK(max_open >= 1 && max_open <= 32, "bad max_open");
  TORCH_CHECK(dst_keys.numel() == nslots && scnt.numel() == nslots &&
                  dst_cnt.numel() == nslots,
              "session tables differ in size");
  for (const auto& t : {sstart, slast, sacc, dst_start, dst_last, dst_acc}) {
    TORCH_CHECK(t.numel() == nslots * max_open,
                "session table shape does not match max_open");
  }
  int64_t out_cap = out_keys.numel();
  TORCH_CHECK(out_start.numel() >= out_cap && out_end.numel() >= out_cap &&
                  out_vals.numel() >= out_cap,
              "out columns shorter than out_keys");
  auto stream = at::hip::getCurrentHIPStream();
  hipLaunchKernelGGL(
      k_session_multi_close_migrate, dim3(n_blocks(nslots, 256)),
      dim3(256), 0, stream, (const uint64_t*)skeys.data_ptr<int64_t>(),
      scnt.data_ptr<int32_t>(),
      (const long long*)sstart.data_ptr<int64_t>(),
      (const long long*)slast.data_ptr<int64_t>(),
      (const long long*)sacc.data_ptr<int64_t>(), nslots, (int)max_open,
      horizon_ms, (uint64_t*)dst_keys.data_ptr<int64_t>(),
      dst_cnt.data_ptr<int32_t>(),
      (long long*)dst_start.data_ptr<int64_t>(),
      (long long*)dst_last.data_ptr<int64_t>(),
      (long long*)dst_acc.data_ptr<int64_t>(), (uint64_t)(nslots - 1),
      out_keys.data_ptr<int32_t>(), out_start.data_ptr<int64_t>(),
      out_end.data_ptr<int64_t>(), out_vals.data_ptr<int64_t>(),
      out_n.data_ptr<int32_t>(), out_cap,
      error_flag.data_ptr<int32_t>());
}

void join_extract(
    torch::Tensor tkeys,
    torch::Tensor tval0,
    torch::Tensor tval1,
    torch::Tensor tflags,
    torch::Tensor out_keys,
    torch::Tensor out_v0,
    torch::Tensor out_v1,
    torch::Tensor out_flags,
    torch::Tensor out_n) {
  int64_t nslots = tkeys.numel();
  auto stream = at::hip::getCurrentHIPStream();
  dim3 block(256);
  dim3 grid(n_blocks(nslots, 256));
  hipLaunchKernelGGL(
      k_join_extract, grid, block, 0, stream,
      (uint64_t*)tkeys.data_ptr<int64_t>(),
      (long long*)tval0.data_ptr<int64_t>(),
      (long long*)tval1.data_ptr<int64_t>(), tflags.data_ptr<int32_t>(),
      nslots, out_keys.data_ptr<int32_t>(), out_v0.data_ptr<int64_t>(),
      out_v1.data_ptr<int64_t>(), out_flags.data_ptr<int32_t>(),
      out_n.data_ptr<int32_t>(), out_keys.numel());
}

int64_t filter_compact(
    torch::Tensor keys,
    torch::Tensor ts,
    c10::optional<torch::Tensor> vals,
    torch::Tensor mask,
    torch::Tensor out_keys,
    torch::Tensor out_ts,
    torch::Tensor out_vals,
    torch::Tensor out_n) {
  check_dev(keys, torch::kInt32, "keys");
  check_dev(ts, torch::kInt64, "ts");
  TORCH_CHECK(mask.scalar_type() == torch::kUInt8 ||
                  mask.scalar_type() == torch::kBool,
              "mask must be bool/uint8");
  int64_t n = keys.numel();
  if (n == 0) return 0;
  const int64_t* vptr = nullptr;
  if (vals.has_value()) vptr = vals->data_ptr<int64_t>();
  auto stream = at::hip::getCurrentHIPStream();
  dim3 block(256);
  dim3 grid(n_blocks(n, 256));
  hipLaunchKernelGGL(
      k_filter_compact, grid, block, 0, stream, keys.data_ptr<int32_t>(),
      ts.data_ptr<int64_t>(), vptr, (const uint8_t*)mask.data_ptr(), n,
      out_keys.data_ptr<int32_t>(), out_ts.data_ptr<int64_t>(),
      out_vals.data_ptr<int64_t>(), out_n.data_ptr<int32_t>());
  return 0;
}

void bucket_hist(torch::Tensor keys, int64_t world, torch::Tensor counts) {
  check_dev(keys, torch::kInt32, "keys");
  check_dev(counts, torch::kInt32, "counts");
  int64_t n = keys.numel();
  if (n == 0) return;
  auto stream = at::hip::getCurrentHIPStream();
  dim3 block(256);
  dim3 grid(n_blocks(n, 256));
  hipLaunchKernelGGL(
      k_bucket_hist, grid, block, (int)(world * sizeof(int)), stream,
      keys.data_ptr<int32_t>(), n, (int)world, counts.data_ptr<int32_t>());
}

void bucket_scatter(
    torch::Tensor keys,
    torch::Tensor ts,
    c10::optional<torch::Tensor> vals,
    int64_t world,
    torch::Tensor cursors,
    torch::Tensor out_keys,
    torch::Tensor out_ts,
    torch::Tensor out_vals) {
  check_dev(keys, torch::kInt32, "keys");
  bool ts32 = ts.scalar_type() == torch::kInt32;
  if (!ts32) check_dev(ts, torch::kInt64, "ts");
  TORCH_CHECK(out_ts.scalar_type() == ts.scalar_type(),
              "out_ts dtype must match ts");
  check_dev(cursors, torch::kInt32, "cursors");
  int64_t n = keys.numel();
  if (n == 0) return;
  const int64_t* vptr = nullptr;
  if (vals.has_value()) {
    check_dev(*vals, torch::kInt64, "vals");
    vptr = vals->data_ptr<int64_t>();
  }
  auto stream = at::hip::getCurrentHIPStream();
  dim3 block(256);
  dim3 grid(n_blocks(n, 256));
  if (ts32) {
    hipLaunchKernelGGL(
        k_bucket_scatter<int32_t>, grid, block, 0, stream,
        keys.data_ptr<int32_t>(), ts.data_ptr<int32_t>(), vptr, n,
        (int)world, cursors.data_ptr<int32_t>(),
        out_keys.data_ptr<int32_t>(), out_ts.data_ptr<int32_t>(),
        out_vals.data_ptr<int64_t>());
  } else {
    hipLaunchKernelGGL(
        k_bucket_scatter<int64_t>, grid, block, 0, stream,
        keys.data_ptr<int32_t>(), ts.data_ptr<int64_t>(), vptr, n,
        (int)world, cursors.data_ptr<int32_t>(),
        out_keys.data_ptr<int32_t>(), out_ts.data_ptr<int64_t>(),
        out_vals.data_ptr<int64_t>());
  }
}


int64_t native_run_window_steps(
    std::vector<torch::Tensor> key_pool,
    std::vector<torch::Tensor> ts_pool,
    int64_t start_step,
    int64_t n_steps,
    int64_t sim_ms_per_batch,
    torch::Tensor tkeys,
    torch::Tensor tvals,
    torch::Tensor max_ts,
    torch::Tensor error_flag,
    torch::Tensor out_keys,
    torch::Tensor out_wins,
    torch::Tensor out_vals,
    torch::Tensor out_n,
    int64_t align_ms,
    int64_t len_ms,
    int64_t wait_ms,
    int64_t mode,
    bool dedup,
    int64_t closed_horizon_in,
    torch::Tensor step_ns_out,
    torch::Tensor state_out,
    int64_t region_bits,
    bool use_radix,
    c10::optional<torch::Tensor> gcursors,
    c10::optional<torch::Tensor> ev_packed,
    c10::optional<torch::Tensor> ev_vals,
    c10::optional<torch::Tensor> ov_cursor,
    c10::optional<torch::Tensor> ov_packed,
    c10::optional<torch::Tensor> ov_vals,
    torch::Tensor alt_tkeys,
    torch::Tensor alt_tvals,
    bool use_radix_v2,
    c10::optional<torch::Tensor> v2_gcur,
    c10::optional<torch::Tensor> v2_gres,
    c10::optional<torch::Tensor> v2_ev,
    c10::optional<torch::Tensor> v2_ev_res,
    bool pipelined = false,
    c10::optional<torch::Tensor> gcursors2 = c10::nullopt,
    c10::optional<torch::Tensor> ev_packed2 = c10::nullopt,
    c10::optional<torch::Tensor> ov_cursor2 = c10::nullopt,
    c10::optional<torch::Tensor> ov_packed2 = c10::nullopt) {
  TORCH_CHECK(!key_pool.empty(), "empty key pool");
  int64_t nslots = tkeys.numel();
  TORCH_CHECK((nslots & (nslots - 1)) == 0, "table size must be 2^k");
  int64_t n = key_pool[0].numel();
  auto stream = at::hip::getCurrentHIPStream();
  dim3 block(256);
  dim3 grid(n_blocks(n, 256));
  int64_t* step_ns =
      step_ns_out.numel() >= n_steps ? step_ns_out.data_ptr<int64_t>()
                                     : nullptr;

  int64_t closed_horizon = closed_horizon_in;
  int64_t total_rows = 0;
  int pool = (int)key_pool.size();
  torch::Tensor cur_k = tkeys, cur_v = tvals;
  torch::Tensor alt_k = alt_tkeys, alt_v = alt_tvals;
  int swap_parity = 0;

  int* h_n = nullptr;
  HIP_CHECK(hipHostMalloc((void**)&h_n, sizeof(int), hipHostMallocDefault));

  bool pipe = pipelined && use_radix && !use_radix_v2 &&
              gcursors2.has_value();
  hipStream_t sc_stream = nullptr;
  hipEvent_t ev_sc[2] = {nullptr, nullptr};
  hipEvent_t ev_ag[2] = {nullptr, nullptr};
  int64_t nb = 0, cap = 0, nseg = 0;
  int seg_bits = (int)region_bits;
  ScatterKind kind = SCAT_FIXED;
  size_t staged_lds = 0;
  uint64_t mask = (uint64_t)(nslots - 1);
  uint64_t win_m2 = 0, win_maxfast = 0;
  if (pipe) {
    nb = nslots >> region_bits;
    TORCH_CHECK(ev_packed2->numel() == ev_packed->numel(),
                "pipelined scatter buffers must match");
    magic_div_u64(len_ms, &win_m2, &win_maxfast);
    kind = scatter_kind_env();
    int coarse = scatter_coarse_bits(kind);
    seg_bits = (int)region_bits + coarse;
    nseg = nslots >> seg_bits;
    staged_lds =
        (size_t)nseg * SC_GRAN * 8 + 4 * (size_t)nseg * sizeof(int);
    while (kind == SCAT_STAGED &&
           (nseg < 1 || staged_lds > 160 * 1024 || seg_bits > 13)) {
      if (coarse > 0 && seg_bits > 13) {
        coarse -= 1;
      } else {
        kind = SCAT_FIXED;
        coarse = 0;
      }
      seg_bits = (int)region_bits + coarse;
      nseg = nslots >> seg_bits;
      staged_lds =
          (size_t)nseg * SC_GRAN * 8 + 4 * (size_t)nseg * sizeof(int);
    }
    if (seg_bits > 13) {
      seg_bits = (int)region_bits;
      nseg = nb;
    }
    cap = ev_packed->numel() / nseg;
    if (kind == SCAT_STAGED) {
      cap &= ~(int64_t)(SC_GRAN - 1);
      if (cap < SC_GRAN) {
        kind = SCAT_FIXED;
        seg_bits = (int)region_bits;
        nseg = nb;
        cap = ev_packed->numel() / nseg;
      }
    }
    HIP_CHECK(hipStreamCreateWithFlags(&sc_stream, hipStreamNonBlocking));
    for (int i = 0; i < 2; ++i) {
      HIP_CHECK(hipEventCreateWithFlags(&ev_sc[i], hipEventDisableTiming));
      HIP_CHECK(hipEventCreateWithFlags(&ev_ag[i], hipEventDisableTiming));
    }
  }

  {
    pybind11::gil_scoped_release release;
    for (int64_t s = 0; s < n_steps; ++s) {
      if (step_ns != nullptr) {
        step_ns[s] = std::chrono::duration_cast<std::chrono::nanoseconds>(
                         std::chrono::steady_clock::now().time_since_epoch())
                         .count();
      }
      int64_t step = start_step + s;
      auto& keys = key_pool[step % pool];
      auto& ts = ts_pool[step % pool];
      int64_t base = align_ms + step * sim_ms_per_batch;
      if (use_radix_v2) {
        radix_v2_window_insert(
            keys, ts, cur_k, cur_v, max_ts, error_flag, *v2_gcur,
            *v2_gres, *v2_ev, *v2_ev_res, align_ms, len_ms, base,
            region_bits);
      } else if (pipe) {
        int par = (int)(step & 1);
        torch::Tensor& gcur = par ? *gcursors2 : *gcursors;
        torch::Tensor& evp = par ? *ev_packed2 : *ev_packed;
        torch::Tensor& ovc = par ? *ov_cursor2 : *ov_cursor;
        torch::Tensor& ovp = par ? *ov_packed2 : *ov_packed;
        if (s >= 2) {
          HIP_CHECK(hipStreamWaitEvent(sc_stream, ev_ag[par], 0));
        }
        HIP_CHECK(hipMemsetAsync(
            gcur.data_ptr<int32_t>(), 0, (size_t)nseg * sizeof(int),
            sc_stream));
        HIP_CHECK(hipMemsetAsync(
            ovc.data_ptr<int32_t>(), 0, sizeof(int), sc_stream));
        auto scat_step = [&](auto tsptr) {
          using TSV =
              std::remove_const_t<std::remove_pointer_t<decltype(tsptr)>>;
          if (kind == SCAT_STAGED) {
            launch_count_staged<TSV>(
                sc_stream, keys.data_ptr<int32_t>(), tsptr, n, 1, align_ms,
                len_ms, len_ms, base, mask, seg_bits, nseg, cap,
                gcur.data_ptr<int32_t>(), (uint64_t*)evp.data_ptr<int64_t>(),
                ovc.data_ptr<int32_t>(), (uint64_t*)ovp.data_ptr<int64_t>(),
                ovp.numel(), (unsigned long long*)max_ts.data_ptr<int64_t>(),
                error_flag.data_ptr<int32_t>(), win_m2, win_maxfast,
            true);
          } else if (kind == SCAT_DIRECT) {
            hipLaunchKernelGGL(
                (k_radix_scatter_direct<AGG_COUNT, TSV>), grid, block, 0,
                sc_stream, keys.data_ptr<int32_t>(), tsptr,
                (const int64_t*)nullptr, n, align_ms, len_ms, len_ms, base,
                mask,
                seg_bits, cap, gcur.data_ptr<int32_t>(),
                (uint64_t*)evp.data_ptr<int64_t>(), (int64_t*)nullptr,
                ovc.data_ptr<int32_t>(), (uint64_t*)ovp.data_ptr<int64_t>(),
                (int64_t*)nullptr, ovp.numel(),
                (unsigned long long*)max_ts.data_ptr<int64_t>(),
                error_flag.data_ptr<int32_t>(), win_m2, win_maxfast);
          } else {
            size_t hist_lds = (size_t)nseg * sizeof(int);
            hipLaunchKernelGGL(
                (k_radix_scatter_fixed<AGG_COUNT, TSV>), grid, block,
                2 * hist_lds,
                sc_stream, keys.data_ptr<int32_t>(), tsptr,
                (const int64_t*)nullptr, n, align_ms, len_ms, len_ms, base, mask,
                seg_bits, cap, gcur.data_ptr<int32_t>(),
                (uint64_t*)evp.data_ptr<int64_t>(), (int64_t*)nullptr,
                ovc.data_ptr<int32_t>(), (uint64_t*)ovp.data_ptr<int64_t>(),
                (int64_t*)nullptr, ovp.numel(),
                (unsigned long long*)max_ts.data_ptr<int64_t>(),
                error_flag.data_ptr<int32_t>(), win_m2, win_maxfast,
                NO_LATE_ARGS);
          }
        };
        if (ts.scalar_type() == torch::kInt32)
          scat_step(ts.data_ptr<int32_t>());
        else scat_step(ts.data_ptr<int64_t>());
        HIP_CHECK(hipEventRecord(ev_sc[par], sc_stream));
        HIP_CHECK(hipStreamWaitEvent(stream, ev_sc[par], 0));
        launch_count_agg(
            stream, (const uint64_t*)evp.data_ptr<int64_t>(),
            gcur.data_ptr<int32_t>(), cap,
            (uint64_t*)cur_k.data_ptr<int64_t>(),
            (unsigned long long*)cur_v.data_ptr<int64_t>(), mask,
            (int)region_bits, seg_bits, nseg,
            error_flag.data_ptr<int32_t>());
        hipLaunchKernelGGL(
            k_overflow_agg<AGG_COUNT>, dim3(64), block, 0, stream,
            (const uint64_t*)ovp.data_ptr<int64_t>(),
            (const int64_t*)nullptr, ovc.data_ptr<int32_t>(), ovp.numel(),
            (uint64_t*)cur_k.data_ptr<int64_t>(),
            (unsigned long long*)cur_v.data_ptr<int64_t>(), mask,
            (int)region_bits, error_flag.data_ptr<int32_t>());
        HIP_CHECK(hipEventRecord(ev_ag[par], stream));
      } else if (use_radix) {
        radix_window_insert(
            keys, ts, c10::nullopt, cur_k, cur_v, max_ts, error_flag,
            *gcursors, *ev_packed, *ev_vals, *ov_cursor, *ov_packed,
            *ov_vals, align_ms, len_ms, AGG_COUNT, base, region_bits);
      } else {
        auto launch = [&](auto kern, auto tsptr) {
          hipLaunchKernelGGL(
              kern, grid, block, 0, stream, keys.data_ptr<int32_t>(),
              tsptr, (const int64_t*)nullptr, n,
              (uint64_t*)cur_k.data_ptr<int64_t>(),
              (unsigned long long*)cur_v.data_ptr<int64_t>(),
              (uint64_t)(nslots - 1), align_ms, len_ms, len_ms, base,
              (int)region_bits,
              (unsigned long long*)max_ts.data_ptr<int64_t>(),
              error_flag.data_ptr<int32_t>(), (const int64_t*)nullptr,
              NO_LATE_ARGS);
        };
        auto disp = [&](auto tsptr) {
          using TSV =
              std::remove_const_t<std::remove_pointer_t<decltype(tsptr)>>;
          if (dedup)
            launch(k_window_agg_insert<AGG_COUNT, true, TSV>, tsptr);
          else launch(k_window_agg_insert<AGG_COUNT, false, TSV>, tsptr);
        };
        if (ts.scalar_type() == torch::kInt32)
          disp(ts.data_ptr<int32_t>());
        else disp(ts.data_ptr<int64_t>());
      }

      int64_t wm = base + sim_ms_per_batch - 1;
      int64_t horizon = (wm - wait_ms - align_ms) / len_ms;
      if (horizon > closed_horizon) {
        HIP_CHECK(hipMemsetAsync(out_n.data_ptr<int32_t>(), 0, sizeof(int), stream));
        launch_close_migrate(
            stream, cur_k, cur_v, horizon, alt_k, alt_v, region_bits,
            out_keys, out_wins, out_vals, out_n, error_flag);
        HIP_CHECK(hipMemcpyAsync(h_n, out_n.data_ptr<int32_t>(), sizeof(int),
                       hipMemcpyDeviceToHost, stream));
        std::swap(cur_k, alt_k);
        std::swap(cur_v, alt_v);
        swap_parity ^= 1;
        HIP_CHECK(hipMemsetAsync(alt_k.data_ptr<int64_t>(), 0xFF,
                                 (size_t)nslots * 8, stream));
        HIP_CHECK(hipMemsetAsync(alt_v.data_ptr<int64_t>(), 0,
                                 (size_t)nslots * 8, stream));
        HIP_CHECK(hipStreamSynchronize(stream));
        total_rows += *h_n;
        closed_horizon = horizon;
      }
    }
    if (sc_stream != nullptr) {
      HIP_CHECK(hipStreamSynchronize(sc_stream));
    }
    HIP_CHECK(hipStreamSynchronize(stream));
  }
  if (sc_stream != nullptr) {
    for (int i = 0; i < 2; ++i) {
      HIP_CHECK(hipEventDestroy(ev_sc[i]));
      HIP_CHECK(hipEventDestroy(ev_ag[i]));
    }
    HIP_CHECK(hipStreamDestroy(sc_stream));
  }
  HIP_CHECK(hipHostFree(h_n));
  auto* st = state_out.data_ptr<int64_t>();
  st[0] = closed_horizon;
  st[1] = total_rows;
  st[2] = swap_parity;
  return total_rows;
}

int64_t native_run_window_steps_graph(
    std::vector<torch::Tensor> key_pool,
    std::vector<torch::Tensor> ts_pool,
    int64_t start_step,
    int64_t n_steps,
    int64_t sim_ms_per_batch,
    torch::Tensor tkeys,
    torch::Tensor tvals,
    torch::Tensor max_ts,
    torch::Tensor error_flag,
    torch::Tensor out_keys,
    torch::Tensor out_wins,
    torch::Tensor out_vals,
    torch::Tensor out_n,
    int64_t align_ms,
    int64_t len_ms,
    int64_t wait_ms,
    int64_t closed_horizon_in,
    torch::Tensor state_out,
    int64_t region_bits,
    torch::Tensor alt_tkeys,
    torch::Tensor alt_tvals,
    torch::Tensor ts_base_dev) {
  TORCH_CHECK(!key_pool.empty(), "empty key pool");
  int64_t nslots = tkeys.numel();
  TORCH_CHECK((nslots & (nslots - 1)) == 0, "table size must be 2^k");
  int64_t n = key_pool[0].numel();
  auto stream = at::hip::getCurrentHIPStream();
  dim3 block(256);
  dim3 grid(n_blocks(n, 256));
  int pool = (int)key_pool.size();
  uint64_t mask = (uint64_t)(nslots - 1);

  ts_base_dev.fill_(align_ms + start_step * sim_ms_per_batch);

  auto launch_insert_on = [&](int j, hipStream_t st) {
    hipLaunchKernelGGL(
        (k_window_agg_insert<AGG_COUNT, false>), grid, block, 0, st,
        key_pool[j].data_ptr<int32_t>(), ts_pool[j].data_ptr<int64_t>(),
        (const int64_t*)nullptr, n, (uint64_t*)tkeys.data_ptr<int64_t>(),
        (unsigned long long*)tvals.data_ptr<int64_t>(), mask, align_ms,
        len_ms, len_ms, 0, (int)region_bits,
        (unsigned long long*)max_ts.data_ptr<int64_t>(),
        error_flag.data_ptr<int32_t>(),
        (const int64_t*)ts_base_dev.data_ptr<int64_t>(), NO_LATE_ARGS);
    hipLaunchKernelGGL(
        k_bump, dim3(1), dim3(1), 0, st,
        ts_base_dev.data_ptr<int64_t>(), sim_ms_per_batch);
  };
  auto launch_insert = [&](int j) { launch_insert_on(j, stream); };

  int64_t closed_horizon = closed_horizon_in;
  int64_t total_rows = 0;
  int* h_n = nullptr;
  HIP_CHECK(hipHostMalloc((void**)&h_n, sizeof(int), hipHostMallocDefault));

  hipGraph_t graph = nullptr;
  hipGraphExec_t gexec = nullptr;
  {
    pybind11::gil_scoped_release release;
    hipStream_t cs = nullptr;
    HIP_CHECK(hipStreamCreateWithFlags(&cs, hipStreamNonBlocking));
    HIP_CHECK(hipStreamBeginCapture(cs, hipStreamCaptureModeThreadLocal));
    for (int j = 0; j < pool; ++j) launch_insert_on(j, cs);
    HIP_CHECK(hipStreamEndCapture(cs, &graph));
    HIP_CHECK(hipStreamDestroy(cs));
    HIP_CHECK(hipGraphInstantiate(&gexec, graph, nullptr, nullptr, 0));

    auto horizon_after = [&](int64_t step) {
      int64_t wm = align_ms + (step + 1) * sim_ms_per_batch - 1;
      return (wm - wait_ms - align_ms) / len_ms;
    };
    auto do_close = [&](int64_t horizon) {
      HIP_CHECK(hipMemsetAsync(out_n.data_ptr<int32_t>(), 0, sizeof(int),
                               stream));
      launch_close_migrate(
          stream, tkeys, tvals, horizon, alt_tkeys, alt_tvals, region_bits,
          out_keys, out_wins, out_vals, out_n, error_flag);
      HIP_CHECK(hipMemcpyAsync(h_n, out_n.data_ptr<int32_t>(), sizeof(int),
                               hipMemcpyDeviceToHost, stream));
      HIP_CHECK(hipMemsetAsync(tkeys.data_ptr<int64_t>(), 0xFF,
                               (size_t)nslots * 8, stream));
      HIP_CHECK(hipMemsetAsync(tvals.data_ptr<int64_t>(), 0,
                               (size_t)nslots * 8, stream));
      launch_close_migrate(
          stream, alt_tkeys, alt_tvals, (int64_t)(-(1LL << 40)), tkeys,
          tvals, region_bits, out_keys, out_wins, out_vals, out_n,
          error_flag);
      HIP_CHECK(hipMemsetAsync(alt_tkeys.data_ptr<int64_t>(), 0xFF,
                               (size_t)nslots * 8, stream));
      HIP_CHECK(hipMemsetAsync(alt_tvals.data_ptr<int64_t>(), 0,
                               (size_t)nslots * 8, stream));
      HIP_CHECK(hipStreamSynchronize(stream));
      total_rows += *h_n;
      closed_horizon = horizon;
    };

    int64_t s = 0;
    while (s < n_steps) {
      bool group_ok = (n_steps - s) >= pool &&
                      horizon_after(start_step + s + pool - 1) ==
                          closed_horizon;
      if (group_ok) {
        HIP_CHECK(hipGraphLaunch(gexec, stream));
        s += pool;
      } else {
        launch_insert((int)((start_step + s) % pool));
        int64_t h = horizon_after(start_step + s);
        s += 1;
        if (h > closed_horizon) do_close(h);
      }
    }
    HIP_CHECK(hipStreamSynchronize(stream));
  }
  HIP_CHECK(hipGraphExecDestroy(gexec));
  HIP_CHECK(hipGraphDestroy(graph));
  HIP_CHECK(hipHostFree(h_n));
  auto* st = state_out.data_ptr<int64_t>();
  st[0] = closed_horizon;
  st[1] = total_rows;
  st[2] = 0;
  return total_rows;
}

void session_radix_insert(
    torch::Tensor keys,
    torch::Tensor ts,
    int64_t ts_base,
    int64_t gap_ms,
    torch::Tensor skeys,
    torch::Tensor sstart,
    torch::Tensor slast,
    torch::Tensor sacc,
    torch::Tensor gcursors,
    torch::Tensor ev_packed,
    torch::Tensor ev_vals,
    torch::Tensor ov_cursor,
    torch::Tensor ov_packed,
    torch::Tensor ov_vals,
    torch::Tensor out_keys,
    torch::Tensor out_start,
    torch::Tensor out_end,
    torch::Tensor out_vals,
    torch::Tensor out_n,
    torch::Tensor max_ts,
    torch::Tensor error_flag,
    int64_t seg_bits) {
  check_dev(keys, torch::kInt32, "keys");
  bool ts32 = ts.scalar_type() == torch::kInt32;
  if (!ts32) check_dev(ts, torch::kInt64, "ts");
  int64_t n = keys.numel();
  int64_t nslots = skeys.numel();
  TORCH_CHECK((nslots & (nslots - 1)) == 0, "table size must be 2^k");
  TORCH_CHECK(seg_bits > 0 && seg_bits < 40, "bad seg_bits");
  int64_t nseg = nslots >> seg_bits;
  TORCH_CHECK(nseg >= 1 && nseg <= 8192, "segment count out of range");
  TORCH_CHECK(gcursors.numel() >= nseg, "gcursors too small");
  int64_t cap = ev_packed.numel() / nseg;
  bool staged = true;
  cap &= ~(int64_t)(SC_GRAN - 1);
  if (cap < SC_GRAN) {
    staged = false;
    cap = ev_packed.numel() / nseg;
  }
  TORCH_CHECK(cap * nseg >= 2 * n || cap >= n,
              "session scatter buffers too small");
  TORCH_CHECK(ev_vals.numel() >= nseg * cap, "ev_vals too small");
  if (n == 0) return;
  auto stream = at::hip::getCurrentHIPStream();
  uint64_t mask = (uint64_t)(nslots - 1);
  gcursors.narrow(0, 0, nseg).zero_();
  ov_cursor.zero_();
  uint64_t win_m2, win_maxfast;
  magic_div_u64((int64_t)1 << 40, &win_m2, &win_maxfast);
  size_t staged_lds = (size_t)nseg * SC_GRAN * 8 * 2 +
                      4 * (size_t)nseg * sizeof(int);
  auto scat512 = [&](auto kern, auto tsptr, unsigned gx, size_t lds) {
    hipLaunchKernelGGL(
        kern, dim3(gx), dim3(512), lds, stream,
        keys.data_ptr<int32_t>(), tsptr, (const int64_t*)nullptr, n, 0,
        (int64_t)1 << 40, (int64_t)1 << 40, ts_base, mask, (int)seg_bits,
        cap,
        gcursors.data_ptr<int32_t>(),
        (uint64_t*)ev_packed.data_ptr<int64_t>(),
        ev_vals.data_ptr<int64_t>(), ov_cursor.data_ptr<int32_t>(),
        (uint64_t*)ov_packed.data_ptr<int64_t>(),
        ov_vals.data_ptr<int64_t>(), ov_packed.numel(),
        (unsigned long long*)max_ts.data_ptr<int64_t>(),
        error_flag.data_ptr<int32_t>(), win_m2, win_maxfast, NO_LATE_ARGS);
  };
  auto scat = [&](auto kern, auto tsptr, unsigned gx, size_t lds) {
    hipLaunchKernelGGL(
        kern, dim3(gx), dim3(256), lds, stream,
        keys.data_ptr<int32_t>(), tsptr, (const int64_t*)nullptr, n, 0,
        (int64_t)1 << 40, (int64_t)1 << 40, ts_base, mask, (int)seg_bits, cap,
        gcursors.data_ptr<int32_t>(),
        (uint64_t*)ev_packed.data_ptr<int64_t>(),
        ev_vals.data_ptr<int64_t>(), ov_cursor.data_ptr<int32_t>(),
        (uint64_t*)ov_packed.data_ptr<int64_t>(),
        ov_vals.data_ptr<int64_t>(), ov_packed.numel(),
        (unsigned long long*)max_ts.data_ptr<int64_t>(),
        error_flag.data_ptr<int32_t>(), win_m2, win_maxfast, NO_LATE_ARGS);
  };
  auto scat_any = [&](auto tsptr) {
    using TSV = std::remove_const_t<std::remove_pointer_t<decltype(tsptr)>>;
    if (staged && staged_lds <= 160 * 1024) {
      unsigned gs = (unsigned)((n + 8191) / 8192);
      if (gs > 1024) gs = 1024;
      if (gs < 1) gs = 1;
      scat512(k_radix_scatter_staged<AGG_TS, TSV, 16, 512>, tsptr, gs,
              staged_lds);
    } else {
      size_t hist_lds = (size_t)nseg * sizeof(int);
      scat(k_radix_scatter_fixed<AGG_TS, TSV>, tsptr,
           (unsigned)n_blocks(n, 256), 2 * hist_lds);
    }
  };
  if (ts32) scat_any(ts.data_ptr<int32_t>());
  else scat_any(ts.data_ptr<int64_t>());

  auto offsets = at::arange(
      nseg, at::TensorOptions().dtype(at::kInt).device(keys.device()));
  offsets = offsets * (int)cap;
  int lds_bits = 12;
  while ((int64_t)1 << lds_bits > nslots >> 1 && lds_bits > 6) lds_bits--;
  size_t agg_lds = (size_t)32 << lds_bits;
  hipLaunchKernelGGL(
      k_radix_session_agg, dim3((unsigned)nseg),
      dim3(lds_bits >= 12 ? 1024 : 256), agg_lds, stream,
      (const uint64_t*)ev_packed.data_ptr<int64_t>(),
      ev_vals.data_ptr<int64_t>(), offsets.data_ptr<int32_t>(),
      gcursors.data_ptr<int32_t>(), cap, lds_bits,
      (uint64_t*)skeys.data_ptr<int64_t>(),
      (long long*)sstart.data_ptr<int64_t>(),
      (long long*)slast.data_ptr<int64_t>(),
      (long long*)sacc.data_ptr<int64_t>(), mask, gap_ms,
      ov_cursor.data_ptr<int32_t>(),
      (uint64_t*)ov_packed.data_ptr<int64_t>(),
      ov_vals.data_ptr<int64_t>(), ov_packed.numel(),
      out_keys.data_ptr<int32_t>(), out_start.data_ptr<int64_t>(),
      out_end.data_ptr<int64_t>(), out_vals.data_ptr<int64_t>(),
      out_n.data_ptr<int32_t>(), out_keys.numel(),
      error_flag.data_ptr<int32_t>());
  hipLaunchKernelGGL(
      k_session_ov_walk, dim3(1), dim3(64), 0, stream,
      (const uint64_t*)ov_packed.data_ptr<int64_t>(),
      ov_vals.data_ptr<int64_t>(), ov_cursor.data_ptr<int32_t>(),
      ov_packed.numel(), (uint64_t*)skeys.data_ptr<int64_t>(),
      (long long*)sstart.data_ptr<int64_t>(),
      (long long*)slast.data_ptr<int64_t>(),
      (long long*)sacc.data_ptr<int64_t>(), mask, gap_ms,
      out_keys.data_ptr<int32_t>(), out_start.data_ptr<int64_t>(),
      out_end.data_ptr<int64_t>(), out_vals.data_ptr<int64_t>(),
      out_n.data_ptr<int32_t>(), out_keys.numel(),
      error_flag.data_ptr<int32_t>());
}


int64_t dict_encode(
    torch::Tensor bytes,
    torch::Tensor offs,
    torch::Tensor dlo,
    torch::Tensor dhi,
    torch::Tensor dids,
    torch::Tensor counter,
    torch::Tensor new_ids,
    torch::Tensor new_idx,
    torch::Tensor new_n,
    torch::Tensor out_ids,
    torch::Tensor error_flag) {
  check_dev(bytes, torch::kUInt8, "bytes");
  check_dev(offs, torch::kInt64, "offs");
  check_dev(dlo, torch::kInt64, "dlo");
  check_dev(out_ids, torch::kInt32, "out_ids");
  int64_t n = offs.numel() - 1;
  int64_t nslots = dlo.numel();
  TORCH_CHECK((nslots & (nslots - 1)) == 0, "dict size must be 2^k");
  if (n == 0) return 0;
  auto stream = at::hip::getCurrentHIPStream();
  dim3 block(256);
  dim3 grid(n_blocks(n, 256));
  uint64_t mask = (uint64_t)(nslots - 1);
  new_n.zero_();
  hipLaunchKernelGGL(
      k_dict_insert, grid, block, 0, stream,
      bytes.data_ptr<uint8_t>(), offs.data_ptr<int64_t>(), n,
      (uint64_t*)dlo.data_ptr<int64_t>(),
      (uint64_t*)dhi.data_ptr<int64_t>(), dids.data_ptr<int32_t>(), mask,
      counter.data_ptr<int32_t>(), new_ids.data_ptr<int32_t>(),
      new_idx.data_ptr<int32_t>(), new_n.data_ptr<int32_t>(),
      new_ids.numel(), error_flag.data_ptr<int32_t>());
  hipLaunchKernelGGL(
      k_dict_lookup, grid, block, 0, stream,
      bytes.data_ptr<uint8_t>(), offs.data_ptr<int64_t>(), n,
      (const uint64_t*)dlo.data_ptr<int64_t>(),
      (const uint64_t*)dhi.data_ptr<int64_t>(), dids.data_ptr<int32_t>(),
      mask, out_ids.data_ptr<int32_t>(), error_flag.data_ptr<int32_t>());
  return n;
}

void dict_restore(
    torch::Tensor bytes,
    torch::Tensor offs,
    torch::Tensor ids,
    torch::Tensor dlo,
    torch::Tensor dhi,
    torch::Tensor dids,
    torch::Tensor error_flag) {
  check_dev(bytes, torch::kUInt8, "bytes");
  check_dev(offs, torch::kInt64, "offs");
  check_dev(ids, torch::kInt32, "ids");
  int64_t n = offs.numel() - 1;
  int64_t nslots = dlo.numel();
  TORCH_CHECK((nslots & (nslots - 1)) == 0, "dict size must be 2^k");
  if (n == 0) return;
  auto stream = at::hip::getCurrentHIPStream();
  hipLaunchKernelGGL(
      k_dict_insert_pinned, dim3(n_blocks(n, 256)), dim3(256), 0, stream,
      bytes.data_ptr<uint8_t>(), offs.data_ptr<int64_t>(),
      ids.data_ptr<int32_t>(), n, (uint64_t*)dlo.data_ptr<int64_t>(),
      (uint64_t*)dhi.data_ptr<int64_t>(), dids.data_ptr<int32_t>(),
      (uint64_t)(nslots - 1), error_flag.data_ptr<int32_t>());
}

void str_exchange_pack(
    torch::Tensor bytes,
    torch::Tensor offs,
    torch::Tensor ts,
    c10::optional<torch::Tensor> vals,
    int64_t world,
    torch::Tensor counts,
    torch::Tensor byte_counts,
    torch::Tensor send_lens,
    torch::Tensor send_ts,
    torch::Tensor send_vals,
    torch::Tensor send_bytes
) {
  check_dev(bytes, torch::kUInt8, "bytes");
  check_dev(offs, torch::kInt64, "offs");
  check_dev(ts, torch::kInt64, "ts");
  check_dev(send_lens, torch::kInt32, "send_lens");
  int64_t n = offs.numel() - 1;
  TORCH_CHECK(world >= 1, "world must be >= 1");
  TORCH_CHECK(send_lens.numel() >= n, "send_lens too small");
  TORCH_CHECK(send_bytes.numel() >= bytes.numel(), "send_bytes too small");
  counts.zero_();
  byte_counts.zero_();
  if (n == 0) return;
  auto stream = at::hip::getCurrentHIPStream();
  dim3 block(256);
  dim3 grid(n_blocks(n, 256));
  hipLaunchKernelGGL(
      k_str_bucket_hist, grid, block, 0, stream,
      bytes.data_ptr<uint8_t>(), offs.data_ptr<int64_t>(), n, (int)world,
      counts.data_ptr<int32_t>(),
      (long long*)byte_counts.data_ptr<int64_t>());
  auto cursors =
      (torch::cumsum(counts, 0, torch::kInt32) - counts).contiguous();
  const int64_t* vptr =
      vals.has_value() ? vals->data_ptr<int64_t>() : nullptr;
  auto src_idx = torch::empty(
      {n}, torch::TensorOptions()
               .dtype(torch::kInt32)
               .device(bytes.device()));
  hipLaunchKernelGGL(
      k_str_meta_scatter, grid, block, 0, stream,
      bytes.data_ptr<uint8_t>(), offs.data_ptr<int64_t>(),
      ts.data_ptr<int64_t>(), vptr, n, (int)world,
      cursors.data_ptr<int32_t>(), send_lens.data_ptr<int32_t>(),
      send_ts.data_ptr<int64_t>(),
      vptr != nullptr ? send_vals.data_ptr<int64_t>() : nullptr,
      src_idx.data_ptr<int32_t>());
  auto lens64 = send_lens.narrow(0, 0, n).to(torch::kInt64);
  auto send_offs = (torch::cumsum(lens64, 0) - lens64).contiguous();
  hipLaunchKernelGGL(
      k_str_byte_gather, grid, block, 0, stream,
      bytes.data_ptr<uint8_t>(), offs.data_ptr<int64_t>(),
      src_idx.data_ptr<int32_t>(), send_offs.data_ptr<int64_t>(), n,
      send_bytes.data_ptr<uint8_t>());
}

PYBIND11_MODULE(TORCH_EXTENSION_NAME, m) {
  m.def("str_exchange_pack", &str_exchange_pack,
        "pack a str batch into per-rank wire segments (content-hash "
        "owner) for the all-to-allv string exchange");
  m.def("session_radix_insert", &session_radix_insert,
        "fused radix session insert: AGG_TS scatter + per-segment LDS "
        "session aggregation + sequential overflow walk");
  m.def("dict_encode", &dict_encode,
        "device string-dictionary encode: 2-phase insert+lookup");
  m.def("dict_restore", &dict_restore,
        "device string-dictionary restore with pinned ids");
  m.def("window_agg_insert", &window_agg_insert,
        "Fused window-id + hash-insert + watermark over an event batch");
  m.def("radix_v2_window_insert", &radix_v2_window_insert,
        "Experimental two-level radix with full-line LDS-staged "
        "scatter (COUNT mode)");
  m.def("radix_scatter_only", &radix_scatter_only,
        "Scatter stage of the radix insert on the current stream");
  m.def("radix_agg_only", &radix_agg_only,
        "Aggregation stage of the radix insert on the current stream");
  m.def("window_agg_insert_late", &window_agg_insert_late,
        "Single-pass window insert that diverts events below the late "
        "cutoff to a late buffer");
  m.def("radix_window_insert_late", &radix_window_insert_late,
        "Radix window insert that diverts events below the late cutoff "
        "to a late buffer");
  m.def("stats_insert_late", &stats_insert_late,
        "Stats insert that diverts events below the late cutoff to a "
        "late buffer");
  m.def("radix_stats_insert_late", &radix_stats_insert_late,
        "Radix stats insert that diverts events below the late cutoff "
        "to a late buffer");
  m.def("radix_window_insert", &radix_window_insert,
        "Radix-partitioned LDS-staged keyed window aggregation");
  m.def("close_migrate", &close_migrate,
        "Window close with reclamation: emit closed cells and migrate "
        "live cells into a fresh table");
  m.def("close_extract", &close_extract,
        "Extract (and clear) closed windows from the keyed state table");
  m.def("stats_insert", &stats_insert,
        "Keyed running count/sum/min/max over an event batch (1BRC)");
  m.def("radix_stats_insert", &radix_stats_insert,
        "Radix-partitioned LDS-staged keyed stats aggregation");
  m.def("stats_fixup", &stats_fixup,
        "Add count/sum deltas to existing stats slots (recovery)");
  m.def("stats_extract", &stats_extract,
        "Extract (and clear) keyed stats below a window horizon");
  m.def("radix_join_insert", &radix_join_insert,
        "Region-partitioned stream join insert (L2-local table ops)");
  m.def("join_insert", &join_insert,
        "Stream-stream hash join insert; emits completed pairs");
  m.def("session_insert", &session_insert,
        "Gap-based session aggregation over a (key, ts)-sorted batch");
  m.def("session_close_migrate", &session_close_migrate,
        "Emit sessions idle past the horizon; migrate live cells");
  m.def("session_restore", &session_restore,
        "Rebuild session cells from a host spill");
  m.def("session_run_collapse", &session_run_collapse,
        "Collapse a (key, ts)-sorted batch into gap-separated runs");
  m.def("session_run_merge", &session_run_merge,
        "Merge sorted runs into the multi-session table (also restore)");
  m.def("session_multi_close_migrate", &session_multi_close_migrate,
        "Emit each cell's closable prefix; migrate the open sessions");
  m.def("session_merge_batch", &session_merge_batch,
        "Merge per-key per-batch (count, min_ts, max_ts) rows into "
        "the session table (gap >= batch span fast path)");
  m.def("join_extract", &join_extract,
        "Extract live join state (recovery snapshot)");
  m.def("filter_compact", &filter_compact,
        "Stream compaction of a RecordBatch by a boolean mask");
  m.def("bucket_hist", &bucket_hist, "Per-destination counts for exchange");
  m.def("bucket_scatter", &bucket_scatter,
        "Scatter events into per-destination segments for all-to-allv");
  m.def("native_run_window_steps_graph", &native_run_window_steps_graph,
        "hipGraph-captured native step loop (latency mode: one graph "
        "launch per pool cycle)");
  m.def("native_run_window_steps", &native_run_window_steps,
        "Run N steps of the columnar window pipeline with no Python "
        "between steps (native step loop)");
}
```

### bytewax_amd/gpu/__init__.py

```python

from dataclasses import dataclass
from datetime import datetime, timezone
from typing import Any, Dict, Optional, Tuple

from ._ext import build as build_ext
from ._ext import ext

EPOCH_UTC = datetime(1970, 1, 1, tzinfo=timezone.utc)

AGG_COUNT = 0
AGG_SUM = 1

_INT64_MAX = (1 << 63) - 1


def _ms(dt: datetime) -> int:
    return int((dt - EPOCH_UTC).total_seconds() * 1000)


@dataclass
class RecordBatch:

    keys: Any
    ts: Any
# ... 339 lines not shown
        self._late = (
            _LateTracker(device, wait_ms, mode == AGG_SUM, late_cap)
            if track_late
            else None
        )

        self.device = device
        self.align_ms = align_ms
        self.len_ms = len_ms
        self.off_ms = off_ms if off_ms > 0 else len_ms
        if self.off_ms > len_ms:
            msg = "window offset must be <= length"
            raise ValueError(msg)
        if self.off_ms < len_ms and dedup:
            msg = "sliding windows are incompatible with the dedup path"
            raise ValueError(msg)
        self.expand = (
            -(-len_ms // self.off_ms) if self.off_ms < len_ms else 1
        )
        self.mode = mode
        self.dedup = dedup
        self.max_ts_host = 0
        self.closed_horizon = -(1 << 62)
        self._close_pending = False
        self._close_ev = None
        self._outn_pin = None
        self._carry_cpu = None
        if radix_v2 and (mode != AGG_COUNT or dedup):
            msg = "radix_v2 supports the COUNT mode only"
            raise ValueError(msg)
        self.radix_v2 = radix_v2 and device.type != "cpu"
        if self.radix_v2:
            radix = True
        self.radix = radix
        self.region_bits = region_bits if radix else 0
        self.cpu = device.type == "cpu"
        if radix and not self.cpu:
            self.n_regions = (1 << slots_pow) >> region_bits
            if self.n_regions < 1:
                msg = "slots_pow must exceed region_bits"
                raise ValueError(msg)
            self.rx_gcursors = torch.zeros(
                self.n_regions, dtype=torch.int32, device=device
            )
            self.rx_ov_cursor = torch.zeros(
                1, dtype=torch.int32, device=device
            )
            self._alloc_rx(max(max_batch, 1))
        if self.cpu:
            self._table: Dict[Tuple[int, int], int] = {}
            return
        self.k = ext()
        self.nslots = 1 << slots_pow
        self.tkeys = torch.full(
            (self.nslots,), -1, dtype=torch.int64, device=device
        )
        self.tvals = torch.zeros(self.nslots, dtype=torch.int64, device=device)
        self.tkeys_alt = torch.full(
            (self.nslots,), -1, dtype=torch.int64, device=device
        )
        self.tvals_alt = torch.zeros(
            self.nslots, dtype=torch.int64, device=device
        )
        self.max_ts_dev = torch.zeros(1, dtype=torch.int64, device=device)
        self.error_flag = torch.zeros(1, dtype=torch.int32, device=device)
        self.out_cap = out_cap
        self.out_keys = torch.empty(out_cap, dtype=torch.int32, device=device)
        self.out_wins = torch.empty(out_cap, dtype=torch.int32, device=device)
        self.out_vals = torch.empty(out_cap, dtype=torch.int64, device=device)
        self.out_n = torch.zeros(1, dtype=torch.int32, device=device)
        self._pin_keys = None

    def _insert_cpu(self, batch: RecordBatch) -> None:
        import numpy as np

        if self.track_late:
            batch = _split_late_cpu(
                batch, self.max_ts_host - self.wait_ms, self._late
            )
        keys = batch.keys.numpy()
        ts64 = batch.ts.numpy().astype("int64", copy=False)
        wins = (
            (ts64 + batch.ts_base - self.align_ms) // self.off_ms
        ).astype("int64")
        if self.mode == AGG_COUNT:
            vals = np.ones(len(keys), dtype="int64")
        else:
            vals = batch.vals.numpy()
        packed = (wins << 32) | keys.astype("uint32")
        uniq, inv = np.unique(packed, return_inverse=True)
        sums = np.bincount(inv, weights=vals).astype("int64")
        for p, s in zip(uniq.tolist(), sums.tolist()):
            kw = (int(np.uint32(p & 0xFFFFFFFF)), int(p >> 32))
            self._table[kw] = self._table.get(kw, 0) + s
        if self.off_ms < self.len_ms:
            t_arr = batch.ts.numpy().astype("int64", copy=False) + batch.ts_base
            lo = (t_arr - self.align_ms - self.len_ms) // self.off_ms + 1
            for k, w_hi, w_lo, v in zip(
                keys.tolist(), wins.tolist(), lo.tolist(), vals.tolist()
            ):
                for wn in range(int(w_lo), int(w_hi)):
                    kw = (int(k), int(wn))
                    self._table[kw] = self._table.get(kw, 0) + int(v)
        mx = int(batch.ts.max().item()) + batch.ts_base if len(batch) else 0
        if mx > self.max_ts_host:
            self.max_ts_host = mx

    def _alloc_rx(self, max_batch: int) -> None:
        import torch

        per_region = max(
            32,
            -(-max_batch * self.expand * 5 // 2) // self.n_regions + 1,
        )
        total = per_region * self.n_regions
        self.rx_max_batch = max_batch
        self.rx_packed = torch.empty(
            total, dtype=torch.int64, device=self.device
        )
        if getattr(self, "radix_v2", False):
            cap_c = (-(-max_batch * 5 // 2) // 256 + 8) // 8 * 8
            res_cap = max(1 << 14, cap_c // 4)
            self.v2_gcur = torch.zeros(256, dtype=torch.int32, device=self.device)
            self.v2_gres = torch.zeros(256, dtype=torch.int32, device=self.device)
            self.v2_ev = torch.empty(
                256 * cap_c, dtype=torch.int64, device=self.device
            )
            self.v2_ev_res = torch.empty(
                256 * res_cap, dtype=torch.int64, device=self.device
            )
        self.rx_vals = torch.empty(
            total if self.mode == AGG_SUM else 0,
            dtype=torch.int64,
            device=self.device,
        )
        ov = max(1 << 20, max_batch)
        self.rx_ov_packed = torch.empty(
            ov, dtype=torch.int64, device=self.device
        )
        self.rx_ov_vals = torch.empty(
            ov if self.mode == AGG_SUM else 0,
            dtype=torch.int64,
            device=self.device,
        )
        if hasattr(self, "rx_packed2"):
            self.rx_gcursors2 = torch.zeros_like(self.rx_gcursors)
            self.rx_packed2 = torch.empty_like(self.rx_packed)
            self.rx_vals2 = torch.empty_like(self.rx_vals)
            self.rx_ov_cursor2 = torch.zeros_like(self.rx_ov_cursor)
            self.rx_ov_packed2 = torch.empty_like(self.rx_ov_packed)
            self.rx_ov_vals2 = torch.empty_like(self.rx_ov_vals)

    def insert(self, batch: RecordBatch) -> None:
        if self.cpu:
            self._insert_cpu(batch)
            if (
                batch.max_ts is not None
                and batch.max_ts > self.max_ts_host
            ):
                self.max_ts_host = batch.max_ts
            return
        if self.radix and len(batch) > self.rx_max_batch:
            self._alloc_rx(int(len(batch) * 5 // 4))
        import torch

        if self.track_late:
            self._insert_late(batch)
            return
        if self.radix_v2:
            self.k.radix_v2_window_insert(
                batch.keys,
                batch.ts.to(torch.int64),
                self.tkeys,
                self.tvals,
                self.max_ts_dev,
                self.error_flag,
                self.v2_gcur,
                self.v2_gres,
                self.v2_ev,
                self.v2_ev_res,
                self.align_ms,
                self.len_ms,
                batch.ts_base,
                self.region_bits,
            )
        elif self.radix:
            self.k.radix_window_insert(
                batch.keys,
                batch.ts,
                batch.vals,
                self.tkeys,
                self.tvals,
                self.max_ts_dev,
                self.error_flag,
                self.rx_gcursors,
                self.rx_packed,
                self.rx_vals,
                self.rx_ov_cursor,
                self.rx_ov_packed,
                self.rx_ov_vals,
                self.align_ms,
                self.len_ms,
                self.mode,
                batch.ts_base,
                self.region_bits,
                self.off_ms,
                [],
                [],
            )
        else:
            self.k.window_agg_insert(
                batch.keys,
                batch.ts,
                batch.vals,
                self.tkeys,
                self.tvals,
                self.max_ts_dev,
                self.error_flag,
                self.align_ms,
                self.len_ms,
                self.mode,
                self.dedup,
                batch.ts_base,
                self.region_bits,
                self.off_ms,
            )
        if batch.max_ts is not None and batch.max_ts > self.max_ts_host:
            self.max_ts_host = batch.max_ts

    def _insert_late(self, batch: RecordBatch) -> None:
        lt = self._late
        lt.reserve(len(batch), self.error_flag)
        cutoff = self.max_ts_host - self.wait_ms
        late_args = (cutoff, lt.keys, lt.ts, lt.vals, lt.n)
        if self.radix:
            self.k.radix_window_insert_late(
                batch.keys,
                batch.ts,
                batch.vals,
                self.tkeys,
                self.tvals,
                self.max_ts_dev,
                self.error_flag,
                self.rx_gcursors,
                self.rx_packed,
                self.rx_vals,
                self.rx_ov_cursor,
                self.rx_ov_packed,
                self.rx_ov_vals,
                self.align_ms,
                self.len_ms,
                self.mode,
                batch.ts_base,
                self.region_bits,
                self.off_ms,
                *late_args,
            )
        else:
            self.k.window_agg_insert_late(
                batch.keys,
                batch.ts,
                batch.vals,
                self.tkeys,
                self.tvals,
                self.max_ts_dev,
                self.error_flag,
                self.align_ms,
                self.len_ms,
                self.mode,
                batch.ts_base,
                self.region_bits,
                self.off_ms,
                *late_args,
            )
        lt.inserted()
        if batch.max_ts is not None:
            if batch.max_ts > self.max_ts_host:
                self.max_ts_host = batch.max_ts
        else:
            self.watermark_ms(sync=True)

    def take_late(self) -> Optional[RecordBatch]:
        if self._late is None:
            return None
        return self._late.take(None if self.cpu else self.error_flag)

    def late_drained(self) -> bool:
        return self._late is not None and bool(self._late.carry)

    def _ordered_only(self, what: str) -> None:
        if self.track_late:
            msg = f"{what} is watermark-ordered only; track_late needs insert()"
            raise ValueError(msg)

    def _ensure_pipe(self) -> None:
        import torch

        if getattr(self, "_pipe_ready", False):
            return
        self._pipe_ready = True
        self._sc_stream = torch.cuda.Stream(self.device)
        self._pipe_parity = 0
        self._ev_sc = [torch.cuda.Event(), torch.cuda.Event()]
        self._ev_ag = [torch.cuda.Event(), torch.cuda.Event()]
        self._ag_recorded = [False, False]
        if not hasattr(self, "rx_packed2"):
            self.rx_gcursors2 = torch.zeros_like(self.rx_gcursors)
            self.rx_packed2 = torch.empty_like(self.rx_packed)
            self.rx_vals2 = torch.empty_like(self.rx_vals)
            self.rx_ov_cursor2 = torch.zeros_like(self.rx_ov_cursor)
            self.rx_ov_packed2 = torch.empty_like(self.rx_ov_packed)
            self.rx_ov_vals2 = torch.empty_like(self.rx_ov_vals)

    def _pipe_bufs(self, par: int):
        if par == 0:
            return (
                self.rx_gcursors,
                self.rx_packed,
                self.rx_vals,
                self.rx_ov_cursor,
                self.rx_ov_packed,
                self.rx_ov_vals,
            )
        return (
            self.rx_gcursors2,
            self.rx_packed2,
            self.rx_vals2,
            self.rx_ov_cursor2,
            self.rx_ov_packed2,
            self.rx_ov_vals2,
        )

    def insert_pipelined(
        self,
        keys,
        ts,
        vals,
        ts_base: int,
        seg_counts,
        seg_bases,
        max_ts: Optional[int],
        works=None,
    ) -> None:
        self._ordered_only("insert_pipelined")
        import torch

        n = int(keys.numel())
        if n > self.rx_max_batch:
            if getattr(self, "_pipe_ready", False):
                torch.cuda.synchronize(self.device)
            self._alloc_rx(int(n * 5 // 4))
        self._ensure_pipe()
        par = self._pipe_parity
        self._pipe_parity ^= 1
        bufs = self._pipe_bufs(par)
        cur = torch.cuda.current_stream(self.device)
        with torch.cuda.stream(self._sc_stream):
            if works:
                for w in works:
                    w.wait()
            if self._ag_recorded[par]:
                self._sc_stream.wait_event(self._ev_ag[par])
            keys.record_stream(self._sc_stream)
            ts.record_stream(self._sc_stream)
            if vals is not None:
                vals.record_stream(self._sc_stream)
            self.k.radix_scatter_only(
                keys,
                ts,
                vals,
                self.max_ts_dev,
                self.error_flag,
                *bufs,
                self.nslots,
                self.align_ms,
                self.len_ms,
                self.mode,
                ts_base,
                self.region_bits,
                self.off_ms,
                list(seg_counts),
                [int(b) for b in seg_bases],
            )
            self._ev_sc[par].record(self._sc_stream)
        cur.wait_event(self._ev_sc[par])
        self.k.radix_agg_only(
            self.tkeys,
            self.tvals,
            self.error_flag,
            *bufs,
            self.mode,
            self.region_bits,
        )
        self._ev_ag[par].record(cur)
        self._ag_recorded[par] = True
        if max_ts is not None and max_ts > self.max_ts_host:
            self.max_ts_host = max_ts

    def insert_lazy(self, lz: "_LazyTsBatch") -> None:
        self._ordered_only("insert_lazy")
        if self.cpu or not self.radix or self.radix_v2:
            self.insert(lz.materialize())
            return
        n = len(lz)
        if n > self.rx_max_batch:
            self._alloc_rx(int(n * 5 // 4))
        self.k.radix_window_insert(
            lz.keys,
            lz.ts32,
            lz.vals,
            self.tkeys,
            self.tvals,
            self.max_ts_dev,
            self.error_flag,
            self.rx_gcursors,
            self.rx_packed,
            self.rx_vals,
            self.rx_ov_cursor,
            self.rx_ov_packed,
            self.rx_ov_vals,
            self.align_ms,
            self.len_ms,
            self.mode,
            0,
            self.region_bits,
            self.off_ms,
            lz.seg_counts,
            lz.seg_bases,
        )
        if lz.max_ts is not None and lz.max_ts > self.max_ts_host:
            self.max_ts_host = lz.max_ts

    def watermark_ms(self, sync: bool = False) -> int:
        if sync and not self.cpu:
            dev = int(self.max_ts_dev.item())
            if dev > self.max_ts_host:
                self.max_ts_host = dev
        return self.max_ts_host

    def _extract_cpu(
        self, win_lo: int, win_hi: int, delete: bool
    ) -> Optional[RecordBatch]:
        import torch

        hit = [
            (k, w, v)
            for (k, w), v in self._table.items()
            if win_lo <= w < win_hi
        ]
        if not hit:
            return None
        if delete:
            for k, w, _v in hit:
                del self._table[(k, w)]
        keys = torch.tensor([k for k, _w, _v in hit], dtype=torch.int32)
        ts = torch.tensor(
            [w * self.off_ms + self.align_ms for _k, w, _v in hit],
            dtype=torch.int64,
        )
        vals = torch.tensor([v for _k, _w, v in hit], dtype=torch.int64)
        return RecordBatch(keys, ts, vals)

    def _read_out(self) -> Optional[RecordBatch]:
        import torch

        n = int(self.out_n.item())
        if n > self.out_cap:
            msg = (
                f"window close produced {n} rows > out_cap {self.out_cap}; "
                "increase out_cap"
            )
            raise RuntimeError(msg)
        _check_error_flag(
            int(self.error_flag.item()), "keyed window state table"
        )
        if n == 0:
            return None
        return RecordBatch(
            self.out_keys[:n].clone(),
            self.out_wins[:n].to(torch.int64) * self.off_ms + self.align_ms,
            self.out_vals[:n].clone(),
        )

    def _extract_range(self, win_lo: int, win_hi: int) -> Optional[RecordBatch]:
        if self.cpu:
            return self._extract_cpu(win_lo, win_hi, delete=False)
        self.out_n.zero_()
        self.k.close_extract(
            self.tkeys,
            self.tvals,
            win_lo,
            win_hi,
            self.out_keys,
            self.out_wins,
            self.out_vals,
            self.out_n,
        )
        return self._read_out()

    def close_due(self, wait_ms: int = 0) -> Optional[RecordBatch]:
        wm = self.watermark_ms()
        horizon = (
            wm - wait_ms - self.align_ms - self.len_ms
        ) // self.off_ms + 1
        if horizon <= self.closed_horizon:
            return None
        if self.cpu:
            out = self._extract_cpu(-(1 << 40), horizon, delete=True)
            self.closed_horizon = horizon
            return out
        self.out_n.zero_()
        self.k.close_migrate(
            self.tkeys,
            self.tvals,
            self.tkeys_alt,
            self.tvals_alt,
            horizon,
            self.region_bits,
            self.out_keys,
            self.out_wins,
            self.out_vals,
            self.out_n,
            self.error_flag,
        )
        self.tkeys, self.tkeys_alt = self.tkeys_alt, self.tkeys
        self.tvals, self.tvals_alt = self.tvals_alt, self.tvals
        self.tkeys_alt.fill_(-1)
        self.tvals_alt.zero_()
        out = self._read_out()
        self.closed_horizon = horizon
        return out

    def close_launch(self, wait_ms: int = 0) -> None:
        import torch

        if self._close_pending:
            return
        wm = self.watermark_ms()
        horizon = (
            wm - wait_ms - self.align_ms - self.len_ms
        ) // self.off_ms + 1
        if horizon <= self.closed_horizon:
            return
        if self.cpu:
            self._carry_cpu = self._extract_cpu(
                -(1 << 40), horizon, delete=True
            )
            self.closed_horizon = horizon
            self._close_pending = self._carry_cpu is not None
            return
        self.out_n.zero_()
        self.k.close_migrate(
            self.tkeys,
            self.tvals,
            self.tkeys_alt,
            self.tvals_alt,
            horizon,
            self.region_bits,
            self.out_keys,
            self.out_wins,
            self.out_vals,
            self.out_n,
            self.error_flag,
        )
        self.tkeys, self.tkeys_alt = self.tkeys_alt, self.tkeys
        self.tvals, self.tvals_alt = self.tvals_alt, self.tvals
        self.tkeys_alt.fill_(-1)
        self.tvals_alt.zero_()
        self.closed_horizon = horizon
        if self._outn_pin is None:
            self._outn_pin = torch.zeros(
                2,
                dtype=torch.int32,
                pin_memory=torch.cuda.is_available(),
            )
        self._outn_pin[0:1].copy_(self.out_n, non_blocking=True)
        self._outn_pin[1:2].copy_(self.error_flag, non_blocking=True)
        self._close_ev = torch.cuda.Event()
        self._close_ev.record()
        self._close_pending = True

    def close_resolve(self) -> Optional[RecordBatch]:
        import torch

        if not self._close_pending:
            return None
        self._close_pending = False
        if self.cpu:
            out = self._carry_cpu
            self._carry_cpu = None
            return out
        self._close_ev.synchronize()
        n = int(self._outn_pin[0].item())
        _check_error_flag(
            int(self._outn_pin[1].item()), "keyed window state table"
        )
        if n > self.out_cap:
            msg = (
                f"window close produced {n} rows > out_cap "
                f"{self.out_cap}; increase out_cap"
            )
            raise RuntimeError(msg)
        if n == 0:
            return None
        return RecordBatch(
            self.out_keys[:n].clone(),
            self.out_wins[:n].to(torch.int64) * self.off_ms + self.align_ms,
            self.out_vals[:n].clone(),
        )

    def close_all(self) -> Optional[RecordBatch]:
        if self._close_pending:
            msg = "close_resolve() the pending close before close_all()"
            raise RuntimeError(msg)
        if self.cpu:
            return self._extract_cpu(self.closed_horizon, 1 << 40, delete=True)
        out = self._extract_range(self.closed_horizon, 1 << 40)
        self.closed_horizon = 1 << 40
        return out

    def snapshot_to_host(self) -> Dict[str, Any]:
        import torch

        if self.cpu:
            import numpy as np

            items = list(self._table.items())
            return {
                "keys": np.array([k for (k, _w), _v in items], dtype="int32"),
                "wins": np.array([w for (_k, w), _v in items], dtype="int32"),
                "vals": np.array([v for _kw, v in items], dtype="int64"),
                "max_ts": self.watermark_ms(),
                "closed_horizon": self.closed_horizon,
            }
        self.out_n.zero_()
        self.k.close_extract(
            self.tkeys,
            self.tvals,
            self.closed_horizon,
            1 << 40,
            self.out_keys,
            self.out_wins,
            self.out_vals,
            self.out_n,
        )
        n = int(self.out_n.item())
        if self._pin_keys is None or self._pin_keys.numel() < n:
            cap = max(n, 1)
            pin = torch.cuda.is_available()
            self._pin_keys = torch.empty(cap, dtype=torch.int32, pin_memory=pin)
            self._pin_wins = torch.empty(cap, dtype=torch.int32, pin_memory=pin)
            self._pin_vals = torch.empty(cap, dtype=torch.int64, pin_memory=pin)
        self._pin_keys[:n].copy_(self.out_keys[:n], non_blocking=True)
        self._pin_wins[:n].copy_(self.out_wins[:n], non_blocking=True)
        self._pin_vals[:n].copy_(self.out_vals[:n], non_blocking=True)
        if torch.cuda.is_available():
            torch.cuda.synchronize(self.device)
        return {
            "keys": self._pin_keys[:n].numpy().copy(),
            "wins": self._pin_wins[:n].numpy().copy(),
            "vals": self._pin_vals[:n].numpy().copy(),
            "max_ts": self.watermark_ms(),
            "closed_horizon": self.closed_horizon,
        }

    def native_run(
        self,
        key_pool,
        ts_pool,
        start_step: int,
        n_steps: int,
        sim_ms_per_batch: int,
        wait_ms: int = 0,
        pipelined: bool = True,
    ):
        self._ordered_only("native_run")
        import torch

        if self.cpu:
            msg = "native_run requires a device table"
            raise RuntimeError(msg)
        pipe = pipelined and self.radix and not self.radix_v2
        if pipe and not hasattr(self, "rx_gcursors2"):
            self.rx_gcursors2 = torch.zeros_like(self.rx_gcursors)
            self.rx_packed2 = torch.empty_like(self.rx_packed)
            self.rx_ov_cursor2 = torch.zeros_like(self.rx_ov_cursor)
            self.rx_ov_packed2 = torch.empty_like(self.rx_ov_packed)
        step_ns = torch.zeros(n_steps, dtype=torch.int64)
        state_out = torch.zeros(3, dtype=torch.int64)
        rows = self.k.native_run_window_steps(
            list(key_pool),
            list(ts_pool),
            start_step,
            n_steps,
            sim_ms_per_batch,
# ... 178 lines not shown
```

Measured before the change: 115.8 billion events/s.

## Use compact hashed scatter entries with 32-bit window division and precomputed slot

For int32-timestamp COUNT inserts through the staged2 scatter, the kernel computes the window with a 32-bit magic division. It packs each entry as key, window delta and a 13-bit precomputed LDS slot from the hash, so the aggregation kernel takes the slot directly instead of rehashing each entry. Events whose deltas fall outside range, and all spilled entries, are converted back to the classic format through the overflow path. The entry base is returned from scatter to the aggregation stage, and the overflow-agg grid now scales with CU count. The change adds encoding complexity and a slow path for out-of-range deltas.

```diff
diff --git a/bytewax_amd/_native/stream_kernels.hip b/bytewax_amd/_native/stream_kernels.hip
--- a/bytewax_amd/_native/stream_kernels.hip
+++ b/bytewax_amd/_native/stream_kernels.hip
@@ -495,6 +495,36 @@
   uint64_t e = (uint64_t)((unsigned __int128)M * (uint64_t)d - (one << p));
   *m2 = M << 4;
   *maxfast = e ? (uint64_t)((one << p) / e) : ~(uint64_t)0;
+}
+
+struct Win32 {
+  uint32_t dlo;
+  uint32_t dspan;
+  uint32_t c;
+  uint32_t wlo;
+  uint32_t qoff;
+  uint32_t dm;
+  int sh1, sh2;
+};
+
+__device__ __forceinline__ uint32_t win32_div(uint32_t y, const Win32& w) {
+  uint32_t t = __umulhi(w.dm, y);
+  return (t + ((y - t) >> w.sh1)) >> w.sh2;
+}
+
+#define ENTRY_SLOT_BITS 13
+#define ENTRY_SLOT_MASK 0x1FFFull
+#define ENTRY_DELTA_MASK 0x7FFFFu
+#define ENTRY_DELTA_LIMIT 0x7FFFFu
+#define ENTRY_W_CLASSIC INT64_MIN
+
+__device__ __forceinline__ uint32_t entry_delta(uint64_t entry) {
+  return ((uint32_t)entry >> ENTRY_SLOT_BITS) & ENTRY_DELTA_MASK;
+}
+
+__device__ __forceinline__ uint64_t entry_classic(
+    uint64_t entry, uint32_t wlo) {
+  return ((uint64_t)(wlo + entry_delta(entry)) << 32) | (entry >> 32);
 }
 
 template <int MODE, typename TS = int64_t, bool LATE = false>
@@ -907,7 +937,8 @@
          + (stage_n / SC_GRAN) * sizeof(uint32_t);
 }
 
-template <typename TS = int64_t, int U = 16, int BLK = 512>
+template <typename TS = int64_t, int U = 16, int BLK = 512,
+          bool HASHED = false>
 __global__ __launch_bounds__(BLK) void k_radix_scatter_staged2(
     const int32_t* __restrict__ keys,
     const TS* __restrict__ ts,
@@ -930,7 +961,9 @@
     unsigned long long* __restrict__ max_ts,
     int* __restrict__ error_flag,
     uint64_t win_m2,
-    uint64_t win_maxfast) {
+    uint64_t win_maxfast,
+    Win32 w32) {
+  static_assert(!HASHED || sizeof(TS) == 4, "hashed entries need deltas");
   constexpr int T = BLK * U;
   constexpr int NW = BLK / WAVE;
   static_assert(T + 7 * BLK < (1 << 14), "staging offset must fit 14 bits");
@@ -960,6 +993,10 @@
     else atomicOr(error_flag, 1);
   };
 
+  auto classic_of = [&](uint64_t entry) {
+    return HASHED ? entry_classic(entry, w32.wlo + w32.qoff) : entry;
+  };
+
   int32_t rk[U];
   TS rt[U];
   auto load_tile = [&](int64_t t0) {
@@ -974,23 +1011,64 @@
   const int64_t stride = (int64_t)gridDim.x * T;
   int64_t local_max = 0;
   int64_t t0 = (int64_t)blockIdx.x * T;
-  if (t0 < n) load_tile(t0);
+  const bool seen = t0 + tid < n;
+  if (t0 < n) {
+    load_tile(t0);
+    if (HASHED) local_max = (int64_t)rt[0];
+  }
   for (; t0 < n; t0 += stride) {
     uint64_t pk[U];
     int sr[U];
+    if (!HASHED) {
 #pragma unroll
-    for (int u = 0; u < U; ++u) {
-      int64_t i = t0 + u * BLK + tid;
-      int64_t t = (int64_t)rt[u] + ts_base;
-      int64_t win = win_of(t, align_ms, len_ms, win_m2, win_maxfast);
-      uint64_t packed =
-          ((uint64_t)(uint32_t)(int32_t)win << 32) | (uint32_t)rk[u];
-      pk[u] = packed;
-      int b = (int)region_of(mix64(packed), mask, seg_bits);
-      sr[u] = -1;
-      if (i < n) {
-        if (t > local_max) local_max = t;
-        sr[u] = (atomicAdd(&lhist[b], 1) << 13) | b;
+      for (int u = 0; u < U; ++u) {
+        int64_t i = t0 + u * BLK + tid;
+        int64_t t = (int64_t)rt[u] + ts_base;
+        int64_t win = win_of(t, align_ms, len_ms, win_m2, win_maxfast);
+        uint64_t packed =
+            ((uint64_t)(uint32_t)(int32_t)win << 32) | (uint32_t)rk[u];
+        pk[u] = packed;
+        int b = (int)region_of(mix64(packed), mask, seg_bits);
+        sr[u] = -1;
+        if (i < n) {
+          if (t > local_max) local_max = t;
+          sr[u] = (atomicAdd(&lhist[b], 1) << 13) | b;
+        }
+      }
+    } else {
+      int64_t left64 = n - t0 - tid;
+      const int left = left64 > T ? T : (left64 < 0 ? 0 : (int)left64);
+      int32_t dmax = (int32_t)local_max;
+      uint32_t rare = 0;
+#pragma unroll
+      for (int u = 0; u < U; ++u) {
+        const bool in = u * BLK < left;
+        const uint32_t d = (uint32_t)rt[u];
+        const uint32_t q = win32_div(d + w32.c, w32);
+        const uint64_t packed =
+            ((uint64_t)(w32.wlo + q) << 32) | (uint32_t)rk[u];
+        const uint64_t h64 = mix64(packed);
+        const uint32_t delta = q - w32.qoff;
+        const bool fits =
+            d - w32.dlo < w32.dspan && delta < ENTRY_DELTA_LIMIT;
+        pk[u] = ((uint64_t)(uint32_t)rk[u] << 32) |
+                (uint64_t)(delta << ENTRY_SLOT_BITS) |
+                ((h64 >> 32) & ENTRY_SLOT_MASK);
+        if (in && !fits) rare |= 1u << u;
+        if (in && (int32_t)d > dmax) dmax = (int32_t)d;
+        const bool ok = in && fits;
+        int b = (int)region_of(h64, mask, seg_bits);
+        int rank = atomicAdd(&lhist[b], ok ? 1 : 0);
+        sr[u] = ok ? ((rank << 13) | b) : -1;
+      }
+      local_max = dmax;
+      while (rare != 0) {
+        int u = __ffs(rare) - 1;
+        rare &= rare - 1;
+        int64_t i = t0 + u * BLK + tid;
+        int64_t win = win_of((int64_t)ts[i] + ts_base, align_ms, len_ms,
+                             win_m2, win_maxfast);
+        spill(((uint64_t)(uint32_t)(int32_t)win << 32) | (uint32_t)keys[i]);
       }
     }
     if (t0 + stride < n) load_tile(t0 + stride);
@@ -1049,8 +1127,8 @@
       if (d != GD_SPILL) {
         *(ulonglong2*)(ev_packed + (int64_t)d * SC_GRAN + 2 * (p & 3)) = v;
       } else {
-        if (v.x != EMPTY_SLOT) spill(v.x);
-        if (v.y != EMPTY_SLOT) spill(v.y);
+        if (v.x != EMPTY_SLOT) spill(classic_of(v.x));
+        if (v.y != EMPTY_SLOT) spill(classic_of(v.y));
       }
     }
   }
@@ -1063,10 +1141,11 @@
         uint64_t p = j < rc ? res[(size_t)tid * SC_GRAN + j] : EMPTY_SLOT;
         int64_t gp = (int64_t)gb + j;
         if (gp < cap) ev_packed[(int64_t)tid * cap + gp] = p;
-        else if (p != EMPTY_SLOT) spill(p);
-      }
-    }
-  }
+        else if (p != EMPTY_SLOT) spill(classic_of(p));
+      }
+    }
+  }
+  if (HASHED) local_max = seen ? local_max + ts_base : 0;
   for (int off = WAVE / 2; off > 0; off >>= 1) {
     int64_t other = __shfl_down((long long)local_max, off);
     if (other > local_max) local_max = other;
@@ -1226,7 +1305,7 @@
 #define AGG_DELTA_MAX 14u
 #define AGG_DELTA_MID 7u
 
-template <int BLK, int R>
+template <int BLK, int R, bool HASHED = false>
 __global__ __launch_bounds__(BLK, BLK == 1024 ? 8 : 4) void k_radix_agg_count(
     const uint64_t* __restrict__ ev_packed,
     const int* __restrict__ counts,
@@ -1236,7 +1315,8 @@
     uint64_t mask,
     int region_bits,
     int lds_bits,
-    int* __restrict__ error_flag) {
+    int* __restrict__ error_flag,
+    uint32_t wlo) {
   extern __shared__ char smem[];
   unsigned long long* cells = (unsigned long long*)smem;
   const int region = 1 << lds_bits;
@@ -1249,20 +1329,28 @@
     ((agg_u64x2*)cells)[s] = agg_u64x2{EMPTY_SLOT, EMPTY_SLOT};
   }
   const uint64_t* seg = ev_packed + (int64_t)b * cap;
-  const uint32_t wbase = (uint32_t)(seg[0] >> 32) - AGG_DELTA_MID;
+  auto win_part = [&](uint64_t packed) {
+    return HASHED ? entry_delta(packed) : (uint32_t)(packed >> 32);
+  };
+  auto key_part = [&](uint64_t packed) {
+    return HASHED ? (uint32_t)(packed >> 32) : (uint32_t)packed;
+  };
+  const uint32_t wbase = win_part(seg[0]) - AGG_DELTA_MID;
   __syncthreads();
 
   auto escape = [&](uint64_t packed) {
+    if (HASHED) packed = entry_classic(packed, wlo);
     if (!hash_add(tkeys, tvals, mask, region_bits, packed, 1ULL)) {
       atomicOr(error_flag, 1);
     }
   };
   auto slot_of = [&](uint64_t packed) {
+    if (HASHED) return (uint32_t)packed & lmask;
     return (uint32_t)(mix64(packed) >> 32) & lmask;
   };
   auto tag_of = [&](uint64_t packed) {
-    return ((unsigned long long)(uint32_t)packed << 4) |
-           (unsigned long long)((uint32_t)(packed >> 32) - wbase);
+    return ((unsigned long long)key_part(packed) << 4) |
+           (unsigned long long)(win_part(packed) - wbase);
   };
   auto drain = [&](uint32_t pend, auto entry, auto start, auto skipped) {
     uint64_t packed = 0;
@@ -1274,7 +1362,7 @@
         int e = __ffs(pend) - 1;
         pend &= pend - 1;
         packed = entry(e);
-        if ((uint32_t)(packed >> 32) - wbase > AGG_DELTA_MAX) {
+        if (win_part(packed) - wbase > AGG_DELTA_MAX) {
           escape(packed);
           continue;
         }
@@ -1337,7 +1425,7 @@
     for (int e = 0; e < E; ++e) {
       uint64_t packed = (e & 1) ? cur_p[e >> 1].y : cur_p[e >> 1].x;
       if (packed == EMPTY_SLOT) continue;
-      bool in_range = (uint32_t)(packed >> 32) - wbase <= AGG_DELTA_MAX;
+      bool in_range = win_part(packed) - wbase <= AGG_DELTA_MAX;
       if (in_range && (first[e] >> 28) == tag_of(packed)) {
         atomicAdd((unsigned int*)&cells[slot[e]], 1u);
       } else {
@@ -1377,8 +1465,8 @@
   for (int s = threadIdx.x; s < region; s += BLK) {
     unsigned long long c = cells[s];
     if (c != EMPTY_SLOT) {
-      uint64_t packed =
-          ((uint64_t)(wbase + ((uint32_t)c >> 28)) << 32) | (c >> 32);
+      uint32_t win = wbase + ((uint32_t)c >> 28) + (HASHED ? wlo : 0u);
+      uint64_t packed = ((uint64_t)win << 32) | (c >> 32);
       if (!hash_add(tkeys, tvals, mask, region_bits, packed,
                     c & 0x0FFFFFFFULL)) {
         atomicOr(error_flag, 1);
@@ -2918,6 +3006,106 @@
   return (unsigned)cus;
 }
 
+static bool agg_wide_env() {
+  const char* s = std::getenv("BYTEWAX_AGG");
+  return s != nullptr && s[0] == 'w';
+}
+
+static bool entries_classic_env() {
+  const char* s = std::getenv("BYTEWAX_ENTRIES");
+  return s != nullptr && s[0] == 'c';
+}
+
+static bool staged2_shape(int64_t nseg, int* threads, int* u, size_t* lds) {
+  int env_u = 0, env_threads = 0;
+  if (const char* e = std::getenv("BYTEWAX_SCATTER_U")) env_u = atoi(e);
+  if (const char* e = std::getenv("BYTEWAX_SCATTER_THREADS"))
+    env_threads = atoi(e);
+  *threads = env_threads == 1024 ? 1024 : 512;
+  *u = *threads == 512 && env_u != 8 ? 16 : 8;
+  *lds = staged2_lds_bytes(nseg, (int64_t)*threads * *u);
+  return nseg <= *threads && *lds <= 160 * 1024;
+}
+
+static bool count_staged2_ok(int64_t xf, const void* evp, int64_t nseg) {
+  int threads, u;
+  size_t lds;
+  return xf == 1 && scatter_staged2_env() && (((uintptr_t)evp) & 15) == 0 &&
+         staged2_shape(nseg, &threads, &u, &lds);
+}
+
+static bool count_agg_compact(int64_t cap, int seg_bits) {
+  return !agg_wide_env() && cap < ((int64_t)1 << 28) && seg_bits >= 8 &&
+         seg_bits <= 13;
+}
+
+struct CountEntries {
+  bool hashed = false;
+  int64_t W = 0;
+  uint32_t qoff = 0;
+  uint32_t dm = 0;
+  int sh1 = 0, sh2 = 0;
+  int64_t agg_w() const {
+    return hashed ? W + (int64_t)qoff : ENTRY_W_CLASSIC;
+  }
+};
+
+static CountEntries plan_count_entries(
+    bool staged_count, int64_t xf, const void* evp, int64_t nseg,
+    int64_t cap, int seg_bits, bool ts_i32, int64_t align_ms,
+    int64_t len_ms, int64_t first_base) {
+  CountEntries ce;
+  if (!staged_count || !ts_i32 || entries_classic_env() ||
+      !count_staged2_ok(xf, evp, nseg) || !count_agg_compact(cap, seg_bits))
+    return ce;
+  if (len_ms < 1 || len_ms >= ((int64_t)1 << 31)) return ce;
+  int threads, u;
+  size_t lds;
+  staged2_shape(nseg, &threads, &u, &lds);
+  if (threads != 512 || u != 16) return ce;
+  __int128 num = (__int128)first_base - align_ms - ((__int128)1 << 31);
+  __int128 w = num / len_ms;
+  if (num % len_ms < 0) w -= 1;
+  if (w < -((__int128)1 << 62) || w > ((__int128)1 << 62)) return ce;
+  ce.hashed = true;
+  ce.W = (int64_t)w;
+  int l = 0;
+  while (((int64_t)1 << l) < len_ms) ++l;
+  ce.dm = (uint32_t)((((unsigned __int128)1 << 32) *
+                      (uint64_t)(((int64_t)1 << l) - len_ms)) /
+                     (uint64_t)len_ms) + 1u;
+  ce.sh1 = l < 1 ? l : 1;
+  ce.sh2 = l > 1 ? l - 1 : 0;
+  int64_t q0 = (int64_t)((num - w * len_ms + ((__int128)1 << 31)) / len_ms);
+  ce.qoff = q0 > (1 << 18) ? (uint32_t)(q0 - (1 << 18)) : 0u;
+  return ce;
+}
+
+static Win32 make_win32(
+    const CountEntries& ce, int64_t ts_base, int64_t align_ms,
+    int64_t len_ms) {
+  Win32 w{};
+  __int128 c = (__int128)ts_base - align_ms - (__int128)ce.W * len_ms;
+  __int128 lo = -((__int128)1 << 31), hi = ((__int128)1 << 31) - 1;
+  if (-c > lo) lo = -c;
+  if ((__int128)align_ms - ts_base > lo) lo = (__int128)align_ms - ts_base;
+  __int128 top = ((__int128)1 << 32) - 1 - c;
+  if (top < hi) hi = top;
+  if (hi >= lo) {
+    __int128 span = hi - lo + 1;
+    if (span > 0xFFFFFFFFll) span = 0xFFFFFFFFll;
+    w.dlo = (uint32_t)(int32_t)(int64_t)lo;
+    w.dspan = (uint32_t)(uint64_t)span;
+  }
+  w.c = (uint32_t)(uint64_t)(c & 0xFFFFFFFFll);
+  w.wlo = (uint32_t)(uint64_t)ce.W;
+  w.qoff = ce.qoff;
+  w.dm = ce.dm;
+  w.sh1 = ce.sh1;
+  w.sh2 = ce.sh2;
+  return w;
+}
+
 template <typename TSV>
 static void launch_count_staged(
     hipStream_t stream, const int32_t* keys, const TSV* ts, int64_t n,
@@ -2925,7 +3113,7 @@
     int64_t ts_base, uint64_t mask, int seg_bits, int64_t nseg, int64_t cap,
     int* gcur, uint64_t* evp, int* ovc, uint64_t* ovp, int64_t ov_cap,
     unsigned long long* max_ts, int* err, uint64_t win_m2,
-    uint64_t win_maxfast, bool overlapped) {
+    uint64_t win_maxfast, bool overlapped, const CountEntries& ce) {
   int env_u = 0, env_threads = 0, env_blocks = 0;
   if (const char* e = std::getenv("BYTEWAX_SCATTER_U")) env_u = atoi(e);
   if (const char* e = std::getenv("BYTEWAX_SCATTER_THREADS"))
@@ -2949,20 +3137,30 @@
         extra...);
     HIP_CHECK(hipGetLastError());
   };
-  if (xf == 1 && scatter_staged2_env() && (((uintptr_t)evp) & 15) == 0) {
+  TORCH_CHECK(!ce.hashed || count_staged2_ok(xf, evp, nseg),
+              "hashed entries planned for a scatter that is not staged2");
+  if (count_staged2_ok(xf, evp, nseg)) {
     const unsigned cus = device_cu_count() * (overlapped ? 2u : 1u);
-    int threads = env_threads == 1024 ? 1024 : 512;
-    int u = threads == 512 && env_u != 8 ? 16 : 8;
-    size_t lds = staged2_lds_bytes(nseg, (int64_t)threads * u);
-    if (nseg <= threads && lds <= 160 * 1024) {
-      if (threads == 1024)
-        go((k_radix_scatter_staged2<TSV, 8, 1024>), 1024, 8, cus, lds);
-      else if (u == 16)
-        go((k_radix_scatter_staged2<TSV, 16, 512>), 512, 16, cus, lds);
-      else
-        go((k_radix_scatter_staged2<TSV, 8, 512>), 512, 8, cus, lds);
-      return;
-    }
+    int threads, u;
+    size_t lds;
+    staged2_shape(nseg, &threads, &u, &lds);
+    Win32 w32{};
+    if constexpr (sizeof(TSV) == 4) {
+      if (ce.hashed) {
+        w32 = make_win32(ce, ts_base, align_ms, len_ms);
+        go((k_radix_scatter_staged2<TSV, 16, 512, true>), 512, 16, cus, lds,
+           w32);
+        return;
+      }
+    }
+    TORCH_CHECK(!ce.hashed, "hashed entries need int32 timestamp deltas");
+    if (threads == 1024)
+      go((k_radix_scatter_staged2<TSV, 8, 1024>), 1024, 8, cus, lds, w32);
+    else if (u == 16)
+      go((k_radix_scatter_staged2<TSV, 16, 512>), 512, 16, cus, lds, w32);
+    else
+      go((k_radix_scatter_staged2<TSV, 8, 512>), 512, 8, cus, lds, w32);
+    return;
   }
   size_t lds = (size_t)nseg * SC_GRAN * 8 + 4 * (size_t)nseg * sizeof(int);
   int threads = 512;
@@ -2984,32 +3182,40 @@
        NO_LATE_ARGS);
 }
 
-static bool agg_wide_env() {
-  const char* s = std::getenv("BYTEWAX_AGG");
-  return s != nullptr && s[0] == 'w';
-}
-
 static void launch_count_agg(
     hipStream_t stream, const uint64_t* evp, const int* gcur, int64_t cap,
     uint64_t* tkeys, unsigned long long* tvals, uint64_t mask,
-    int region_bits, int seg_bits, int64_t nseg, int* err) {
-  auto go = [&](auto kern, int threads, size_t lds, auto... lead) {
-    hipLaunchKernelGGL(
-        kern, dim3((unsigned)nseg), dim3((unsigned)threads), lds, stream,
-        evp, lead..., gcur, cap, tkeys, tvals, mask, region_bits, seg_bits,
-        err);
-    HIP_CHECK(hipGetLastError());
-  };
-  if (!agg_wide_env() && cap < ((int64_t)1 << 28) && seg_bits >= 8 &&
-      seg_bits <= 13) {
-    size_t lds = (size_t)8 << seg_bits;
-    if (seg_bits >= 12) go((k_radix_agg_count<1024, 2>), 1024, lds);
-    else go((k_radix_agg_count<256, 2>), 256, lds);
+    int region_bits, int seg_bits, int64_t nseg, int* err,
+    int64_t entry_w) {
+  const bool hashed = entry_w != ENTRY_W_CLASSIC;
+  const uint32_t wlo = hashed ? (uint32_t)(uint64_t)entry_w : 0u;
+  if (count_agg_compact(cap, seg_bits)) {
+    auto go = [&](auto kern, int threads) {
+      hipLaunchKernelGGL(
+          kern, dim3((unsigned)nseg), dim3((unsigned)threads),
+          (size_t)8 << seg_bits, stream, evp, gcur, cap, tkeys, tvals, mask,
+          region_bits, seg_bits, err, wlo);
+      HIP_CHECK(hipGetLastError());
+    };
+    if (seg_bits >= 12) {
+      if (hashed) go((k_radix_agg_count<1024, 2, true>), 1024);
+      else go((k_radix_agg_count<1024, 2>), 1024);
+    } else {
+      if (hashed) go((k_radix_agg_count<256, 2, true>), 256);
+      else go((k_radix_agg_count<256, 2>), 256);
+    }
     return;
   }
-  go(k_radix_agg<AGG_COUNT>, seg_bits >= 12 ? 1024 : 256,
-     (size_t)16 << seg_bits, (const int64_t*)nullptr);
-}
+  TORCH_CHECK(!hashed, "hashed scatter entries need the compact aggregation");
+  hipLaunchKernelGGL(
+      k_radix_agg<AGG_COUNT>, dim3((unsigned)nseg),
+      dim3(seg_bits >= 12 ? 1024u : 256u), (size_t)16 << seg_bits, stream,
+      evp, (const int64_t*)nullptr, gcur, cap, tkeys, tvals, mask,
+      region_bits, seg_bits, err);
+  HIP_CHECK(hipGetLastError());
+}
+
+static dim3 overflow_agg_grid() { return dim3(device_cu_count()); }
 
 static void radix_window_insert_impl(
     torch::Tensor keys,
@@ -3140,6 +3346,10 @@
 
   uint64_t win_m2, win_maxfast;
   magic_div_u64(off_ms, &win_m2, &win_maxfast);
+  const CountEntries ce = plan_count_entries(
+      kind == SCAT_STAGED && mode == AGG_COUNT && late == nullptr, xf,
+      ev_packed.data_ptr<int64_t>(), nseg, cap, seg_bits, seg32 || ts32,
+      align_ms, len_ms, segs[0].base);
   unsigned scat_threads = 256;
   auto scat = [&](auto kern, auto tsptr, const Seg& sg, unsigned gx,
                   size_t lds, auto... extra) {
@@ -3207,7 +3417,7 @@
             (uint64_t*)ov_packed.data_ptr<int64_t>(), ov_packed.numel(),
             (unsigned long long*)max_ts.data_ptr<int64_t>(),
             error_flag.data_ptr<int32_t>(), win_m2, win_maxfast,
-            false);
+            false, ce);
       } else {
         unsigned cap_gs = env_blocks > 0 ? (unsigned)env_blocks : 1024u;
         unsigned gs = (unsigned)((sg.n * xf + 256 * 16 - 1) / (256 * 16));
@@ -3256,14 +3466,15 @@
         gcursors.data_ptr<int32_t>(), cap,
         (uint64_t*)tkeys.data_ptr<int64_t>(),
         (unsigned long long*)tvals.data_ptr<int64_t>(), mask,
-        (int)region_bits, seg_bits, nseg, error_flag.data_ptr<int32_t>());
+        (int)region_bits, seg_bits, nseg, error_flag.data_ptr<int32_t>(),
+        ce.agg_w());
   } else {
     agg(k_radix_agg<AGG_SUM>);
   }
 
   auto ov = [&](auto kern) {
     hipLaunchKernelGGL(
-        kern, dim3(64), dim3(256), 0, stream,
+        kern, overflow_agg_grid(), dim3(256), 0, stream,
         (const uint64_t*)ov_packed.data_ptr<int64_t>(),
         mode == AGG_SUM ? ov_vals.data_ptr<int64_t>() : nullptr,
         ov_cursor.data_ptr<int32_t>(), ov_packed.numel(),
@@ -3337,7 +3548,7 @@
       region_bits, off_ms, {}, {}, &sink);
 }
 
-void radix_scatter_only(
+int64_t radix_scatter_only(
     torch::Tensor keys,
     torch::Tensor ts,
     c10::optional<torch::Tensor> vals,
@@ -3430,7 +3641,7 @@
       gcursors.data_ptr<int32_t>(), 0, (size_t)nseg * sizeof(int), stream));
   HIP_CHECK(hipMemsetAsync(
       ov_cursor.data_ptr<int32_t>(), 0, sizeof(int), stream));
-  if (n == 0) return;
+  if (n == 0) return ENTRY_W_CLASSIC;
 
   struct Seg {
     int64_t off, n, base;
@@ -3445,6 +3656,11 @@
   } else {
     segs.push_back({0, n, ts_base});
   }
+  if (segs.empty()) return ENTRY_W_CLASSIC;
+  const CountEntries ce = plan_count_entries(
+      kind == SCAT_STAGED && mode == AGG_COUNT, xf,
+      ev_packed.data_ptr<int64_t>(), nseg, cap, seg_bits, seg32 || ts32,
+      align_ms, len_ms, segs[0].base);
   unsigned scat_threads = 256;
   auto scat = [&](auto kern, auto tsptr, const Seg& sg, unsigned gx,
                   size_t lds, auto... extra) {
@@ -3475,7 +3691,7 @@
             (uint64_t*)ov_packed.data_ptr<int64_t>(), ov_packed.numel(),
             (unsigned long long*)max_ts.data_ptr<int64_t>(),
             error_flag.data_ptr<int32_t>(), win_m2, win_maxfast,
-            true);
+            true, ce);
       } else {
         unsigned gs = (unsigned)((sg.n + 4095) / 4096);
         if (gs > 1024) gs = 1024;
@@ -3503,6 +3719,7 @@
     if (seg32 || ts32) scat_any(ts.data_ptr<int32_t>(), sg);
     else scat_any(ts.data_ptr<int64_t>(), sg);
   }
+  return ce.agg_w();
 }
 
 void radix_agg_only(
@@ -3516,7 +3733,8 @@
     torch::Tensor ov_packed,
     torch::Tensor ov_vals,
     int64_t mode,
-    int64_t region_bits) {
+    int64_t region_bits,
+    int64_t entry_w = ENTRY_W_CLASSIC) {
   int64_t nslots = tkeys.numel();
   int64_t nb = nslots >> region_bits;
   auto stream = at::hip::getCurrentHIPStream();
@@ -3573,13 +3791,14 @@
         gcursors.data_ptr<int32_t>(), cap,
         (uint64_t*)tkeys.data_ptr<int64_t>(),
         (unsigned long long*)tvals.data_ptr<int64_t>(), mask,
-        (int)region_bits, seg_bits, nseg, error_flag.data_ptr<int32_t>());
+        (int)region_bits, seg_bits, nseg, error_flag.data_ptr<int32_t>(),
+        mode == AGG_COUNT ? entry_w : ENTRY_W_CLASSIC);
   } else {
     agg(k_radix_agg<AGG_SUM>);
   }
   auto ov = [&](auto kern) {
     hipLaunchKernelGGL(
-        kern, dim3(64), dim3(256), 0, stream,
+        kern, overflow_agg_grid(), dim3(256), 0, stream,
         (const uint64_t*)ov_packed.data_ptr<int64_t>(),
         mode == AGG_SUM ? ov_vals.data_ptr<int64_t>() : nullptr,
         ov_cursor.data_ptr<int32_t>(), ov_packed.numel(),
@@ -5092,6 +5311,10 @@
             sc_stream));
         HIP_CHECK(hipMemsetAsync(
             ovc.data_ptr<int32_t>(), 0, sizeof(int), sc_stream));
+        const CountEntries ce = plan_count_entries(
+            kind == SCAT_STAGED, 1, evp.data_ptr<int64_t>(), nseg, cap,
+            seg_bits, ts.scalar_type() == torch::kInt32, align_ms, len_ms,
+            base);
         auto scat_step = [&](auto tsptr) {
           using TSV =
               std::remove_const_t<std::remove_pointer_t<decltype(tsptr)>>;
@@ -5103,7 +5326,7 @@
                 ovc.data_ptr<int32_t>(), (uint64_t*)ovp.data_ptr<int64_t>(),
                 ovp.numel(), (unsigned long long*)max_ts.data_ptr<int64_t>(),
                 error_flag.data_ptr<int32_t>(), win_m2, win_maxfast,
-            true);
+                true, ce);
           } else if (kind == SCAT_DIRECT) {
             hipLaunchKernelGGL(
                 (k_radix_scatter_direct<AGG_COUNT, TSV>), grid, block, 0,
@@ -5143,9 +5366,9 @@
             (uint64_t*)cur_k.data_ptr<int64_t>(),
             (unsigned long long*)cur_v.data_ptr<int64_t>(), mask,
             (int)region_bits, seg_bits, nseg,
-            error_flag.data_ptr<int32_t>());
+            error_flag.data_ptr<int32_t>(), ce.agg_w());
         hipLaunchKernelGGL(
-            k_overflow_agg<AGG_COUNT>, dim3(64), block, 0, stream,
+            k_overflow_agg<AGG_COUNT>, overflow_agg_grid(), block, 0, stream,
             (const uint64_t*)ovp.data_ptr<int64_t>(),
             (const int64_t*)nullptr, ovc.data_ptr<int32_t>(), ovp.numel(),
             (uint64_t*)cur_k.data_ptr<int64_t>(),
@@ -5621,9 +5844,17 @@
         "Experimental two-level radix with full-line LDS-staged "
         "scatter (COUNT mode)");
   m.def("radix_scatter_only", &radix_scatter_only,
-        "Scatter stage of the radix insert on the current stream");
+        "Scatter stage of the radix insert on the current stream; returns "
+        "the entry base for radix_agg_only");
   m.def("radix_agg_only", &radix_agg_only,
-        "Aggregation stage of the radix insert on the current stream");
+        "Aggregation stage of the radix insert on the current stream",
+        pybind11::arg("tkeys"), pybind11::arg("tvals"),
+        pybind11::arg("error_flag"), pybind11::arg("gcursors"),
+        pybind11::arg("ev_packed"), pybind11::arg("ev_vals"),
+        pybind11::arg("ov_cursor"), pybind11::arg("ov_packed"),
+        pybind11::arg("ov_vals"), pybind11::arg("mode"),
+        pybind11::arg("region_bits"),
+        pybind11::arg("entry_w") = (int64_t)ENTRY_W_CLASSIC);
   m.def("window_agg_insert_late", &window_agg_insert_late,
         "Single-pass window insert that diverts events below the late "
         "cutoff to a late buffer");
diff --git a/bytewax_amd/gpu/__init__.py b/bytewax_amd/gpu/__init__.py
--- a/bytewax_amd/gpu/__init__.py
+++ b/bytewax_amd/gpu/__init__.py
@@ -665,6 +665,7 @@
         self._sc_stream = torch.cuda.Stream(self.device)
         self._pipe_parity = 0
         self._ev_sc = [torch.cuda.Event(), torch.cuda.Event()]
+        self._ev_w = [None, None]
         self._ev_ag = [torch.cuda.Event(), torch.cuda.Event()]
         self._ag_recorded = [False, False]
         if not hasattr(self, "rx_packed2"):
@@ -728,7 +729,7 @@
             ts.record_stream(self._sc_stream)
             if vals is not None:
                 vals.record_stream(self._sc_stream)
-            self.k.radix_scatter_only(
+            self._ev_w[par] = self.k.radix_scatter_only(
                 keys,
                 ts,
                 vals,
@@ -754,6 +755,7 @@
             *bufs,
             self.mode,
             self.region_bits,
+            self._ev_w[par],
         )
         self._ev_ag[par].record(cur)
         self._ag_recorded[par] = True
```

Measured after the change: 122.7 billion events/s, median of 6. 6.0% higher.
